# autonomousvision/unimatch

Hardware: AMD Instinct MI355X
Metric: image_pairs_per_sec (higher is better)
Workload: dtype f16x2

## Files before the change

include/unimatch_hip.h:

```cpp
#ifndef UNIMATCH_HIP_H
#define UNIMATCH_HIP_H

#include <stddef.h>
#include <stdint.h>

#ifdef __cplusplus
extern "C" {
#endif

#define UM_VERSION 220

#define UM_MODE_EXACT 0
#define UM_MODE_FAST 1

#define UM_ERR_BAD_ARG (-1)
#define UM_ERR_BAD_GEOMETRY (-2)
#define UM_ERR_WORKSPACE (-3)
#define UM_ERR_UNSUPPORTED (-4)
#define UM_ERR_COLLECTIVE (-5)

int um_version(void);
const char* um_last_error_string(void);

#define UM_RANGE_PLANES 1u
#define UM_RANGE_ATTN_TOKENS 2u
#define UM_RANGE_ATTN_QUERY 4u
#define UM_RANGE_ATTN_OUTPUT 8u
#define UM_RANGE_FFN_TOKENS 16u
#define UM_RANGE_FFN_HIDDEN 32u
#define UM_RANGE_KV_TOKENS 64u
#define UM_RANGE_LINEAR 128u
int um_range_flags(unsigned* flags_out, int reset);

#define UM_K_WINDOW_ATTN 0
#define UM_K_GLOBAL_SOFTMAX 1
#define UM_K_SPLIT_PLANES 2
#define UM_K_LOCAL_CORR 3
#define UM_K_COST_VOLUME 4
#define UM_K_PROP_LOCAL 5
#define UM_K_DEPTH_CORR 6
#define UM_K_LINEAR 7
#define UM_K_INSTANCE_NORM 8
#define UM_K_CONVEX_UPSAMPLE 9
#define UM_K_FFN 10
#define UM_K_CONV 11
#define UM_K_COUNT 12
#define UM_V_WATTN_TILE 0
#define UM_V_WATTN_KSPLIT 1
#define UM_V_FFN_TILE 2
#define UM_V_FFN_HSPLIT 3
#define UM_V_GSV4 4
#define UM_V_GSV3 5
#define UM_V_K4_MFMA 6
#define UM_V_K4_VALU 7
#define UM_V_K3_MFMA 8
#define UM_V_K3_VALU 9
#define UM_V_CONV_PATCH 10
#define UM_V_CONV_ROWS 11
#define UM_V_CONV_GENERIC 12
#define UM_V_WATTN_W8 13
#define UM_V_CONV_PATCH_NORM 14
#define UM_V_COUNT 15
int um_census_enable(int on);
long um_census_count(int variant);
int um_window_attn_tile_census(int enable, unsigned long long* counts4);
double um_probe_mfma_flops(int iters);
int um_probe_mfma(float* sink, int iters, void* stream);
int um_probe_copy(const void* src, void* dst, size_t bytes, void* stream);
int um_probe_chase(const unsigned* ring, unsigned* out, int hops, void* stream);
int um_timing_enable(int kernel_mask);
int um_timing_collect(int kernel_id, double* total_ms, int* launches);

size_t um_window_attn_workspace_bytes(int streams, int tokens, int channels, int mode);
int um_window_attn_fwd(const float* q, const float* k, const float* v, float* out,
                       int streams, int h, int w, int channels,
                       int win_h, int win_w, int shift_h, int shift_w,
                       int mode, void* workspace, size_t workspace_bytes, void* stream);

int um_window_attn_planes_fwd(const void* q_planes, const void* k_planes, const void* v_planes, float* out,
                              int streams, int h, int w, int channels, int ldq, int ldkv,
                              long q_plane_stride, long kv_plane_stride,
                              int win_h, int win_w, int shift_h, int shift_w, int kv_rotate, int mode, void* stream);

int um_window_attn_merge_fwd(const void* q_planes, const void* k_planes, const void* v_planes, const void* wm_planes,
                             const float* gamma, const float* beta, const float* residual, float eps, int wshift, float* out,
                             int streams, int h, int w, int channels, int ldq, int ldkv, long q_plane_stride,
                             long kv_plane_stride, int win_h, int win_w, int shift_h, int shift_w, int kv_rotate, int mode,
                             void* stream);

size_t um_window_attn_ksplit_workspace_bytes(int streams, int h, int w, int win_h, int win_w);
int um_window_attn_plan(int streams, int h, int w, int win_h, int win_w, int* full_tiles, int* split_tiles, int* parts);
int um_window_attn_qproj_merge_fwd(const float* x, const void* wq_planes, const void* k_planes, const void* v_planes,
                                   const void* wm_planes, const float* gamma, const float* beta, const float* residual, float eps,
                                   int wshift, float* out, int streams, int h, int w, int channels, int ldkv,
                                   long kv_plane_stride, int win_h, int win_w, int shift_h, int shift_w, int kv_rotate, int mode,
                                   void* workspace, size_t workspace_bytes, void* stream);

#define UM_EPI_PLANES 0
#define UM_EPI_LN 1
#define UM_EPI_GELU_PLANES 2
size_t um_planes_bytes(long rows, int cols, int mode);
int um_weight_planes(const float* w, void* planes, int n, int k, int wshift, int mode, void* stream);
int um_linear_fwd(const float* a0, const float* a1, const void* a_planes, const void* w_planes,
                  int m, int n, int k, int wshift, int epilogue, void* out,
                  const float* gamma, const float* beta, const float* residual, float eps,
                  int mode, void* stream);

int um_linear_bias_fwd(const float* a0, const void* a_planes, const void* w_planes, const float* bias, int m, int n, int k,
                       int wshift, float out_mul, float bias_mul, void* out_planes, float* out_f32, int mode, void* stream);

int um_ffn_fwd(const float* x, const float* y, const void* w1_planes, const void* w2_planes, int m, int hidden,
               int wshift, const float* gamma, const float* beta, float eps, float* out, int mode, void* stream);
size_t um_ffn_split_workspace_bytes(int m, int hidden);
int um_ffn_ws_fwd(const float* x, const float* y, const void* w1_planes, const void* w2_planes, int m, int hidden,
                  int wshift, const float* gamma, const float* beta, float eps, float* out, int mode, void* workspace,
                  size_t workspace_bytes, void* stream);

int um_kv4_fwd(const float* x, const void* wc_planes, int m, int wshift, void* out_planes, int mode, void* stream);
int um_ffn_kv_fwd(const float* x, const float* y, const void* w1_planes, const void* w2_planes, int m, int hidden, int wshift,
                  const float* gamma, const float* beta, float eps, float* out, const void* wc_planes, void* kv_planes, int mode,
                  void* workspace, size_t workspace_bytes, void* stream);

int um_conv2d_fwd(const void* a_planes, const void* w_planes, const float* bias, float* out, float* stats_out, int batch,
                  int hi, int wi, int cin, int cout, int kh, int kw, int stride, int pad_h, int pad_w, int relu, int wshift,
                  int mode, void* stream);
int um_conv2d_ex(const void* a_planes, int a_ld, int a_coff, long a_rows, const void* w_planes, const float* bias, float* out,
                 int out_ld, int out_coff, void* out_planes, int outp_ld, int outp_coff, long outp_rows, float* stats_out,
                 int batch, int hi, int wi, int cin, int cout, int kh, int kw, int stride, int pad_h, int pad_w, int act,
                 int wshift, int mode, void* stream);
int um_conv2d_gru_fwd(int gate, const void* a_planes, int a_ld, int a_coff, long a_rows, const void* w_planes, const float* bias,
                      float* hidden, const float* z, int z_ld, float* z_out, int z_out_ld, void* out_planes, int outp_ld,
                      int outp_coff, long outp_rows, int batch, int hi, int wi, int cin, int channels, int kh, int kw, int pad_h,
                      int pad_w, int wshift, int mode, void* stream);
int um_conv2d_gru_add_fwd(int gate, const void* a_planes, int a_ld, int a_coff, long a_rows, const void* w_planes, const float* bias,
                          const float* addend, int addend_ld, float* hidden, const float* z, int z_ld, float* z_out, int z_out_ld,
                          void* out_planes, int outp_ld, int outp_coff, long outp_rows, int batch, int hi, int wi, int cin,
                          int channels, int kh, int kw, int pad_h, int pad_w, int wshift, int mode, void* stream);
int um_conv2d_addend_fwd(const void* a_planes, const void* w_planes, const float* bias, const float* addend, int addend_ld,
                         int addend_period, float* out, int batch, int hi, int wi, int cin, int cout, int kh, int kw, int stride,
                         int pad_h, int pad_w, int wshift, int mode, void* stream);
int um_conv_stats_parts(int hi, int wi, int cout, int kh, int kw, int stride, int pad_h, int pad_w);
size_t um_conv_stats_bytes(int batch, int parts, int channels);

size_t um_stem_planes_bytes(int batch, int h, int w);
size_t um_conv7_planes_bytes(int batch, int h, int w, int stride);
int um_conv7_fwd(const float* image, int channels, int normalize, const float* mean3, const float* std3, void* image_planes,
                 const void* w_planes, const float* bias, float* out, int out_ld, int out_coff, void* out_planes, int outp_ld,
                 int outp_coff, long outp_rows, float* stats_out, int batch, int h, int w, int cout, int stride, int act,
                 int wshift, void* stream);
int um_stem_conv_fwd(const float* image, int normalize, const float* mean3, const float* std3, void* image_planes,
                     const void* w_planes, float* out, float* stats_out, int batch, int h, int w, int cout, int wshift,
                     void* stream);

int um_stem_conv_pair_fwd(const float* image0, int batch0, const float* image1, int batch1, int normalize, const float* mean3,
                          const float* std3, void* image_planes, const void* w_planes, float* out, float* stats_out, int h, int w,
                          int cout, int wshift, void* stream);

size_t um_nhwc_norm_workspace_bytes(int batch, int pixels, int channels);
int um_nhwc_instance_norm(const float* x, const float* shortcut, const void* shortcut_planes, void* planes_out, float* f32_out,
                          int batch, int pixels, int channels, float eps, int normalize, int relu, const float* conv_stats,
                          int conv_stats_parts, void* workspace, size_t workspace_bytes, int mode, void* stream);

int um_nhwc_concat_planes(const float* map, const float* tokens, void* planes_out, int batch, int pixels, int map_channels, int channels,
                          int mode, void* stream);

size_t um_nhwc_norm_sc_workspace_bytes(int batch, int pixels, int channels);
int um_nhwc_instance_norm_sc(const float* x, const float* shortcut, const void* shortcut_planes, void* planes_out, float* f32_out,
                             int batch, int pixels, int channels, float eps, int normalize, int relu, const float* conv_stats,
                             int conv_stats_parts, void* workspace, size_t workspace_bytes, int mode, void* stream,
                             const float* sc_conv_stats, int sc_conv_stats_parts);

int um_nhwc_stats_finalize(const float* conv_stats, int conv_stats_parts, float* stats_out, int batch, int pixels, int channels,
                           float eps, void* stream);
int um_conv2d_norm_supported(int hi, int wi, int cin, int cout, int kh, int kw, int stride, int pad_h, int pad_w, int mode);
int um_conv2d_norm_fwd(const float* x, const float* norm_stats, int norm_relu, const void* w_planes, const float* bias, float* out,
                       float* stats_out, int batch, int hi, int wi, int cin, int cout, int kh, int kw, int stride, int pad_h,
                       int pad_w, int relu, int wshift, int mode, void* stream);

int um_conv2d_entry_supported(int hi, int wi, int cin, int cout, int kh, int kw, int stride, int pad_h, int pad_w, int mode);
int um_conv2d_entry_fwd(const float* u, const float* ustats, const void* s_planes, const void* w_planes, const void* w2_planes,
                        const float* bias2, float* out_t, float* out_d, float* stats_t, float* stats_d, int batch, int hi, int wi,
                        int cin, int cout, int kh, int kw, int stride, int pad_h, int pad_w, int wshift, int mode, void* stream);

int um_nhwc_gate(int mode, const float* src, int src_ld, const float* zr, float* hbuf, void* planes_out, int ld, int coff,
                 long plane_rows, long rows, int channels, void* stream);

int um_nchw_to_nhwc(const float* x, void* planes_out, float* f32_out, int batch, int channels, int pixels, int mode,
                    void* stream);

size_t um_global_corr_workspace_bytes(int batch, int tokens, int channels, int mode);
int um_global_corr_softmax_flow(const float* f0, const float* f1, float* flow,
                                int batch, int h, int w, int channels, int bidir,
                                int mode, void* workspace, size_t workspace_bytes, void* stream);

int um_global_corr_softmax_stereo(const float* f0, const float* f1, float* disp,
                                  int batch, int h, int w, int channels,
                                  int mode, void* workspace, size_t workspace_bytes, void* stream);

int um_prop_global_attn(const float* q, const float* k, const float* value, float* out,
                        int batch, int h, int w, int channels, int value_channels,
                        int mode, void* workspace, size_t workspace_bytes, void* stream);
float um_global_corr_plane_scale(int channels);
int um_prop_global_attn_planes(const void* q_planes, const void* k_planes, const float* value, float* out, int batch, int h,
                               int w, int channels, int value_channels, int mode, void* workspace, size_t workspace_bytes,
                               void* stream);

size_t um_global_match_stats_workspace_bytes(int batch, int tokens, int channels, int mode);
int um_global_match_stats(const float* f0, const float* f1, float* stats, int* best, float* mean,
                          int batch, int h, int w, int channels, int bidir, int stereo,
                          int mode, void* workspace, size_t workspace_bytes, void* stream);
int um_match_mutual(const int* best_fwd, const int* best_bwd, unsigned char* mutual, int batch, int h, int w, int radius,
                    void* stream);


int um_local_corr_softmax(const float* f0, const float* f1, float* out,
                          int batch, int h, int w, int channels, int radius, int one_d, void* stream);

int um_local_corr_with_flow(const float* f0, const float* f1, const float* flow, float* cost,
                            int batch, int h, int w, int channels, int radius, void* stream);
int um_local_corr_with_flow_dilated(const float* f0, const float* f1, const float* flow, float* cost,
                                    int batch, int h, int w, int channels, int radius, int dilation, void* stream);
int um_local_corr_with_flow_planes(const float* f0, const float* f1, const float* flow, void* planes_out, int ld, long plane_rows,
                                   int batch, int h, int w, int channels, int radius, void* stream);

size_t um_local_corr_feat_planes_bytes(int batch, int h, int w, int channels);
int um_local_corr_feat_planes(const float* f0, const float* f1, void* feat_planes, int batch, int h, int w, int channels,
                              void* stream);
int um_local_corr_with_flow_feat_supported(int h, int w, int channels, int radius);
int um_local_corr_softmax_mfma(const float* f0, const float* f1, float* out, int batch, int h, int w, int channels, int radius,
                               void* workspace, size_t workspace_bytes, void* stream);
int um_local_corr_with_flow_feat(const float* f0, const float* f1, const void* feat_planes, const float* flow, float* cost,
                                 void* planes_out, int ld, long plane_rows, int batch, int h, int w, int channels, int radius,
                                 int flags, unsigned* stats ,
                                 void* stream);

int um_prop_local_attn(const float* q, const float* k, const float* value, float* out,
                       int batch, int h, int w, int channels, int value_channels, int radius,
                       void* stream);

int um_depth_corr_softmax(const float* f0, const float* f1, const float* cam, const float* candidates,
                          float* out, int batch, int h, int w, int channels, int num_candidates,
                          int from_argmax, void* stream);

int um_convex_upsample(const float* flow, const float* mask, float* up, int batch, int channels, int h, int w,
                       int factor, int is_depth, int mask_nhwc, void* stream);

int um_flow_warp(const float* feature_tokens, const float* flow, float* out_tokens, int batch, int h, int w, int channels,
                 void* stream);

int um_fwd_bwd_occlusion(const float* fwd, const float* bwd, float* occ_fwd, float* occ_bwd, int batch, int h, int w, float alpha,
                         float beta, void* stream);
size_t um_flow_to_rgb_workspace_bytes(int batch, int h, int w);
int um_flow_to_rgb(const float* flow, unsigned char* rgb, int batch, int h, int w, void* workspace, size_t ws_bytes, void* stream);

int um_flow_chain(const float* flow, const float* occ, const float* pos_in, const unsigned char* alive_in, float* tracks,
                  unsigned char* visible, int pairs, int h, int w, int n, int grid_stride, void* stream);

#define UM_FLOW_METRICS_K 16
#define UM_DISP_METRICS_K 8
#define UM_DEPTH_METRICS_K 8
size_t um_flow_metrics_workspace_bytes(int batch, int h, int w);
int um_flow_metrics(const float* pred, const float* gt, const float* valid, const float* noc_valid, double* rows, int batch, int hp,
                    int wp, int h, int w, int top, int left, void* workspace, size_t ws_bytes, void* stream);
size_t um_disp_metrics_workspace_bytes(int batch, int h, int w);
int um_disp_metrics(const float* pred, const float* gt, double* rows, int batch, int hp, int wp, int h, int w, int top, int left,
                    float max_disp, void* workspace, size_t ws_bytes, void* stream);
size_t um_depth_metrics_workspace_bytes(int batch, int h, int w);
int um_depth_metrics(const float* pred, const float* gt, const float* valid, double* rows, int batch, int hp, int wp, int h, int w,
                     int top, int left, float lo, float hi, void* workspace, size_t ws_bytes, void* stream);

#define UM_PREPOST_MAX_DIM 262140
#define UM_IMG_F32_NCHW 0
#define UM_IMG_U8_NHWC 1
#define UM_SIZE_PAD 0
#define UM_SIZE_RESIZE 1
#define UM_PRED_FLOW 0
#define UM_PRED_DISPARITY 1
#define UM_PRED_DEPTH 2
int um_image_prepare(const void* src, int src_layout, float* dst, int batch, int h, int w, int transpose, const float* mean,
                     const float* std, int mode, int hp, int wp, int top, int left, void* stream);
int um_pred_restore(const float* pred, float* out, int batch, int channels, int hp, int wp, int mode, int top, int left, int h, int w,
                    int kind, int transpose, void* stream);
int um_image_prepare_flip(const void* src, int src_layout, float* dst, int batch, int h, int w, int transpose, const float* mean,
                          const float* std, int mode, int hp, int wp, int top, int left, int hflip, void* stream);
int um_pred_restore_flip(const float* pred, float* out, int batch, int channels, int hp, int wp, int mode, int top, int left, int h,
                         int w, int kind, int transpose, int hflip, void* stream);

#define UM_NORM_MINMAX_255 0
#define UM_NORM_MIN_P95_256 1
size_t um_scalar_to_rgb_workspace_bytes(int batch, int h, int w);
int um_scalar_to_rgb(const float* x, unsigned char* rgb, int batch, int h, int w, int inverse, int norm, const unsigned char* lut,
                     float* stats_out, void* workspace, size_t ws_bytes, void* stream);

int um_flow_upsample2x(const float* flow, float* out, int batch, int channels, int h, int w, float mult, void* stream);
int um_depth_cam_pack(const float* intrinsics, const float* pose, float* cam, int batch, float stride_div, int bidir, void* stream);
int um_rigid_flow(const float* inv_depth, const float* cam, float* flow, int batch, int h, int w, void* stream);
int um_relative_pose_pairs(const float* poses, float* rel, int frames, void* stream);

int um_disp_consistency(const float* disp_left, const float* disp_right, float* occ_left, float* occ_right, int batch, int h, int w,
                        float alpha, float beta, void* stream);
int um_depth_consistency(const float* depth_ref, const float* depth_src, const float* cam_fwd, const float* cam_inv, float* occ,
                         float* err_px, float* err_rel, int batch, int h, int w, float px_thr, float rel_thr, void* stream);
size_t um_points_workspace_bytes(int batch, int h, int w, int stride);
int um_points_pack(const float* depth, const float* cam_world, const float* keep, const unsigned char* colors, float* xyz,
                   unsigned char* rgb, int* count, int batch, int h, int w, int stride, float min_depth, float max_depth, void* workspace,
                   size_t ws_bytes, void* stream);

int um_instance_norm_fwd(const float* x, const float* shortcut, float* y, long planes, int hw, float eps,
                         int relu, void* stream);

#define UM_COMM_ID_BYTES 128
int um_comm_unique_id(void* id_out );
int um_comm_init_rank(void** comm_out, const void* id , int rank, int world);
int um_comm_init_file(void** comm_out, const char* path, int rank, int world, int timeout_seconds);
int um_comm_init_file_nonce(void** comm_out, const char* path, int rank, int world, int timeout_seconds, int nonce);
int um_comm_world(void* comm);
int um_comm_destroy(void* comm);
int um_allgather_preds(void* comm, const float* send, float* recv, size_t count_per_rank, void* stream);

int um_swin_attn_fwd(const float* q, const float* k, const float* v, float* out, int streams, int h, int w, int channels,
                     int win_h, int win_w, int shift_h, int shift_w, int mode, void* workspace, size_t workspace_bytes,
                     void* stream);
int um_attn1d_fwd(const float* q, const float* k, const float* v, float* out, int streams, int h, int w, int channels,
                  int win_w, int shift_w, int mode, void* workspace, size_t workspace_bytes, void* stream);
int um_local_corr_softmax_1d(const float* f0, const float* f1, float* out, int batch, int h, int w, int channels, int radius,
                             void* stream);
size_t um_workspace_bytes_swin_attn_fwd(int streams, int h, int w, int channels, int mode);
size_t um_workspace_bytes_attn1d_fwd(int streams, int h, int w, int channels, int mode);
size_t um_workspace_bytes_global_corr_softmax_flow(int batch, int h, int w, int channels, int mode);
size_t um_workspace_bytes_global_corr_softmax_stereo(int batch, int h, int w, int channels, int mode);
size_t um_workspace_bytes_prop_global_attn(int batch, int h, int w, int channels, int mode);
size_t um_workspace_bytes_local_corr_softmax(int batch, int h, int w, int channels, int mode);
size_t um_workspace_bytes_local_corr_softmax_1d(int batch, int h, int w, int channels, int mode);
size_t um_workspace_bytes_local_corr_with_flow(int batch, int h, int w, int channels, int mode);
size_t um_workspace_bytes_prop_local_attn(int batch, int h, int w, int channels, int mode);
size_t um_workspace_bytes_depth_corr_softmax(int batch, int h, int w, int channels, int mode);
size_t um_workspace_bytes_allgather_preds(int batch, int h, int w, int channels, int mode);

#ifdef UM_DIAGNOSTIC_BUILD
int um_debug_mfma_peak(float* sink, int iters, int random_operands, void* stream);
int um_debug_mfma_ticks(unsigned long long* ticks, float* sink, int iters, int random_operands, int waves, int chain, void* stream);
int um_debug_mfma_lds(unsigned long long* ticks, float* sink, int tiles, int mode, void* stream);
#endif

#ifdef __cplusplus
}
#endif
#endif
```

unimatch_amd/_abi.py:

```python
import ctypes
import os

_HERE = os.path.dirname(os.path.abspath(__file__))
LIB_PATH = os.environ.get('UM_LIB') or os.path.join(_HERE, 'libunimatch_hip.so')

MODE_EXACT = 0
MODE_FAST = 1

CENSUS = {'wattn_tile': 0, 'wattn_ksplit': 1, 'ffn_tile': 2, 'ffn_hsplit': 3, 'gsv4': 4, 'gsv3': 5, 'k4_mfma': 6, 'k4_valu': 7,
          'k3_mfma': 8, 'k3_valu': 9, 'conv_patch': 10, 'conv_rows': 11, 'conv_generic': 12, 'wattn_w8': 13, 'conv_patch_norm': 14}

_c_int, _c_size_t, _c_void_p = ctypes.c_int, ctypes.c_size_t, ctypes.c_void_p

SIGNATURES = {
    'um_version': (_c_int, []),
    'um_last_error_string': (ctypes.c_char_p, []),
    'um_range_flags': (_c_int, [ctypes.POINTER(ctypes.c_uint), _c_int]),
    'um_timing_enable': (_c_int, [_c_int]),
    'um_timing_collect': (_c_int, [_c_int, ctypes.POINTER(ctypes.c_double), ctypes.POINTER(_c_int)]),
    'um_window_attn_workspace_bytes': (_c_size_t, [_c_int] * 4),
    'um_window_attn_fwd': (_c_int, [_c_void_p] * 4 + [_c_int] * 9 + [_c_void_p, _c_size_t, _c_void_p]),
    'um_window_attn_planes_fwd': (_c_int, [_c_void_p] * 4 + [_c_int] * 6 + [ctypes.c_long] * 2 + [_c_int] * 6 + [_c_void_p]),
    'um_window_attn_merge_fwd': (_c_int, [_c_void_p] * 7 + [ctypes.c_float, _c_int, _c_void_p] + [_c_int] * 6 + [ctypes.c_long] * 2 +
                                 [_c_int] * 6 + [_c_void_p]),
    'um_window_attn_qproj_merge_fwd': (_c_int, [_c_void_p] * 8 + [ctypes.c_float, _c_int, _c_void_p] + [_c_int] * 5 + [ctypes.c_long] +
                                       [_c_int] * 6 + [_c_void_p, _c_size_t, _c_void_p]),
    'um_window_attn_ksplit_workspace_bytes': (_c_size_t, [_c_int] * 5),
    'um_window_attn_plan': (_c_int, [_c_int] * 5 + [ctypes.POINTER(_c_int)] * 3),
    'um_planes_bytes': (_c_size_t, [ctypes.c_long, _c_int, _c_int]),
    'um_weight_planes': (_c_int, [_c_void_p] * 2 + [_c_int] * 4 + [_c_void_p]),
    'um_linear_fwd': (_c_int, [_c_void_p] * 4 + [_c_int] * 5 + [_c_void_p] * 4 + [ctypes.c_float, _c_int, _c_void_p]),
    'um_linear_bias_fwd': (_c_int, [_c_void_p] * 4 + [_c_int] * 4 + [ctypes.c_float] * 2 + [_c_void_p] * 2 + [_c_int, _c_void_p]),
    'um_ffn_fwd': (_c_int, [_c_void_p] * 4 + [_c_int] * 3 + [_c_void_p] * 2 + [ctypes.c_float, _c_void_p, _c_int, _c_void_p]),
    'um_ffn_ws_fwd': (_c_int, [_c_void_p] * 4 + [_c_int] * 3 + [_c_void_p] * 2 + [ctypes.c_float, _c_void_p, _c_int, _c_void_p, _c_size_t,
                                _c_void_p]),
    'um_ffn_split_workspace_bytes': (_c_size_t, [_c_int] * 2),
    'um_ffn_kv_fwd': (_c_int, [_c_void_p] * 4 + [_c_int] * 3 + [_c_void_p] * 2 + [ctypes.c_float, _c_void_p, _c_void_p, _c_void_p, _c_int, _c_void_p,
                                _c_size_t, _c_void_p]),
    'um_kv4_fwd': (_c_int, [_c_void_p, _c_void_p, _c_int, _c_int, _c_void_p, _c_int, _c_void_p]),
    'um_conv2d_fwd': (_c_int, [_c_void_p] * 5 + [_c_int] * 13 + [_c_void_p]),
    'um_conv2d_addend_fwd': (_c_int, [_c_void_p] * 4 + [_c_int, _c_int, _c_void_p] + [_c_int] * 12 + [_c_void_p]),
    'um_conv2d_ex': (_c_int, [_c_void_p, _c_int, _c_int, ctypes.c_long, _c_void_p, _c_void_p, _c_void_p, _c_int, _c_int, _c_void_p,
                              _c_int, _c_int, ctypes.c_long, _c_void_p] + [_c_int] * 13 + [_c_void_p]),
    'um_nhwc_gate': (_c_int, [_c_int, _c_void_p, _c_int, _c_void_p, _c_void_p, _c_void_p, _c_int, _c_int, ctypes.c_long, ctypes.c_long,
                              _c_int, _c_void_p]),
    'um_local_corr_with_flow_planes': (_c_int, [_c_void_p] * 4 + [_c_int, ctypes.c_long] + [_c_int] * 5 + [_c_void_p]),
    'um_conv2d_gru_fwd': (_c_int, [_c_int, _c_void_p, _c_int, _c_int, ctypes.c_long, _c_void_p, _c_void_p, _c_void_p, _c_void_p, _c_int,
                                   _c_void_p, _c_int, _c_void_p, _c_int, _c_int, ctypes.c_long] + [_c_int] * 11 + [_c_void_p]),
    'um_conv2d_gru_add_fwd': (_c_int, [_c_int, _c_void_p, _c_int, _c_int, ctypes.c_long, _c_void_p, _c_void_p, _c_void_p, _c_int, _c_void_p, _c_void_p,
                                        _c_int, _c_void_p, _c_int, _c_void_p, _c_int, _c_int, ctypes.c_long] + [_c_int] * 11 + [_c_void_p]),
    'um_conv2d_norm_supported': (_c_int, [_c_int] * 10),
    'um_conv2d_norm_fwd': (_c_int, [_c_void_p, _c_void_p, _c_int] + [_c_void_p] * 4 + [_c_int] * 13 + [_c_void_p]),
    'um_conv2d_entry_supported': (_c_int, [_c_int] * 10),
    'um_conv2d_entry_fwd': (_c_int, [_c_void_p] * 10 + [_c_int] * 12 + [_c_void_p]),
    'um_nhwc_norm_sc_workspace_bytes': (_c_size_t, [_c_int] * 3),
    'um_nhwc_instance_norm_sc': (_c_int, [_c_void_p] * 5 + [_c_int] * 3 + [ctypes.c_float, _c_int, _c_int, _c_void_p, _c_int, _c_void_p,
                                          _c_size_t, _c_int, _c_void_p, _c_void_p, _c_int]),
    'um_nhwc_stats_finalize': (_c_int, [_c_void_p, _c_int, _c_void_p] + [_c_int] * 3 + [ctypes.c_float, _c_void_p]),
    'um_conv_stats_bytes': (_c_size_t, [_c_int] * 3),
    'um_conv_stats_parts': (_c_int, [_c_int] * 8),
    'um_stem_planes_bytes': (_c_size_t, [_c_int] * 3),
    'um_conv7_planes_bytes': (_c_size_t, [_c_int] * 4),
    'um_conv7_fwd': (_c_int, [_c_void_p, _c_int, _c_int] + [_c_void_p] * 6 + [_c_int, _c_int, _c_void_p, _c_int, _c_int, ctypes.c_long,
                              _c_void_p] + [_c_int] * 7 + [_c_void_p]),
    'um_stem_conv_fwd': (_c_int, [_c_void_p, _c_int] + [_c_void_p] * 6 + [_c_int] * 5 + [_c_void_p]),
    'um_stem_conv_pair_fwd': (_c_int, [_c_void_p, _c_int, _c_void_p, _c_int, _c_int] + [_c_void_p] * 6 + [_c_int] * 4 + [_c_void_p]),
    'um_nhwc_concat_planes': (_c_int, [_c_void_p] * 3 + [_c_int] * 5 + [_c_void_p]),
    'um_nhwc_norm_workspace_bytes': (_c_size_t, [_c_int] * 3),
    'um_nhwc_instance_norm': (_c_int, [_c_void_p] * 5 + [_c_int] * 3 + [ctypes.c_float, _c_int, _c_int, _c_void_p, _c_int, _c_void_p,
                                       _c_size_t, _c_int, _c_void_p]),
    'um_nchw_to_nhwc': (_c_int, [_c_void_p] * 3 + [_c_int] * 4 + [_c_void_p]),
    'um_flow_warp': (_c_int, [_c_void_p] * 3 + [_c_int] * 4 + [_c_void_p]),
    'um_fwd_bwd_occlusion': (_c_int, [_c_void_p] * 4 + [_c_int] * 3 + [ctypes.c_float] * 2 + [_c_void_p]),
    'um_flow_to_rgb_workspace_bytes': (_c_size_t, [_c_int] * 3),
    'um_flow_to_rgb': (_c_int, [_c_void_p] * 2 + [_c_int] * 3 + [_c_void_p, _c_size_t, _c_void_p]),
    'um_flow_chain': (_c_int, [_c_void_p] * 6 + [_c_int] * 5 + [_c_void_p]),
    'um_flow_metrics_workspace_bytes': (_c_size_t, [_c_int] * 3),
    'um_flow_metrics': (_c_int, [_c_void_p] * 5 + [_c_int] * 7 + [_c_void_p, _c_size_t, _c_void_p]),
    'um_disp_metrics_workspace_bytes': (_c_size_t, [_c_int] * 3),
    'um_disp_metrics': (_c_int, [_c_void_p] * 3 + [_c_int] * 7 + [ctypes.c_float, _c_void_p, _c_size_t, _c_void_p]),
    'um_depth_metrics_workspace_bytes': (_c_size_t, [_c_int] * 3),
    'um_depth_metrics': (_c_int, [_c_void_p] * 4 + [_c_int] * 7 + [ctypes.c_float] * 2 + [_c_void_p, _c_size_t, _c_void_p]),
    'um_image_prepare': (_c_int, [_c_void_p, _c_int, _c_void_p] + [_c_int] * 4 + [ctypes.POINTER(ctypes.c_float)] * 2 + [_c_int] * 5 +
                         [_c_void_p]),
    'um_pred_restore': (_c_int, [_c_void_p] * 2 + [_c_int] * 11 + [_c_void_p]),
    'um_image_prepare_flip': (_c_int, [_c_void_p, _c_int, _c_void_p] + [_c_int] * 4 + [ctypes.POINTER(ctypes.c_float)] * 2 + [_c_int] * 6 +
                              [_c_void_p]),
    'um_pred_restore_flip': (_c_int, [_c_void_p] * 2 + [_c_int] * 12 + [_c_void_p]),
    'um_scalar_to_rgb_workspace_bytes': (_c_size_t, [_c_int] * 3),
    'um_scalar_to_rgb': (_c_int, [_c_void_p] * 2 + [_c_int] * 5 + [_c_void_p] * 3 + [_c_size_t, _c_void_p]),
    'um_convex_upsample': (_c_int, [_c_void_p] * 3 + [_c_int] * 7 + [_c_void_p]),
    'um_flow_upsample2x': (_c_int, [_c_void_p] * 2 + [_c_int] * 4 + [ctypes.c_float, _c_void_p]),
    'um_depth_cam_pack': (_c_int, [_c_void_p] * 3 + [_c_int, ctypes.c_float, _c_int, _c_void_p]),
    'um_rigid_flow': (_c_int, [_c_void_p] * 3 + [_c_int] * 3 + [_c_void_p]),
    'um_relative_pose_pairs': (_c_int, [_c_void_p] * 2 + [_c_int, _c_void_p]),
    'um_disp_consistency': (_c_int, [_c_void_p] * 4 + [_c_int] * 3 + [ctypes.c_float] * 2 + [_c_void_p]),
    'um_depth_consistency': (_c_int, [_c_void_p] * 7 + [_c_int] * 3 + [ctypes.c_float] * 2 + [_c_void_p]),
    'um_points_workspace_bytes': (_c_size_t, [_c_int] * 4),
    'um_points_pack': (_c_int, [_c_void_p] * 7 + [_c_int] * 4 + [ctypes.c_float] * 2 + [_c_void_p, _c_size_t, _c_void_p]),
    'um_instance_norm_fwd': (_c_int, [_c_void_p] * 3 + [ctypes.c_long, _c_int, ctypes.c_float, _c_int, _c_void_p]),
    'um_global_corr_workspace_bytes': (_c_size_t, [_c_int] * 4),
    'um_global_corr_softmax_flow': (_c_int, [_c_void_p] * 3 + [_c_int] * 6 + [_c_void_p, _c_size_t, _c_void_p]),
    'um_global_corr_softmax_stereo': (_c_int, [_c_void_p] * 3 + [_c_int] * 5 + [_c_void_p, _c_size_t, _c_void_p]),
    'um_prop_global_attn': (_c_int, [_c_void_p] * 4 + [_c_int] * 6 + [_c_void_p, _c_size_t, _c_void_p]),
    'um_global_corr_plane_scale': (ctypes.c_float, [_c_int]),
    'um_prop_global_attn_planes': (_c_int, [_c_void_p] * 4 + [_c_int] * 6 + [_c_void_p, _c_size_t, _c_void_p]),
    'um_global_match_stats_workspace_bytes': (_c_size_t, [_c_int] * 4),
    'um_global_match_stats': (_c_int, [_c_void_p] * 5 + [_c_int] * 7 + [_c_void_p, _c_size_t, _c_void_p]),
    'um_match_mutual': (_c_int, [_c_void_p] * 3 + [_c_int] * 4 + [_c_void_p]),
    'um_local_corr_softmax': (_c_int, [_c_void_p] * 3 + [_c_int] * 6 + [_c_void_p]),
    'um_local_corr_with_flow': (_c_int, [_c_void_p] * 4 + [_c_int] * 5 + [_c_void_p]),
    'um_local_corr_with_flow_dilated': (_c_int, [_c_void_p] * 4 + [_c_int] * 6 + [_c_void_p]),
    'um_local_corr_feat_planes_bytes': (ctypes.c_size_t, [_c_int] * 4),
    'um_local_corr_feat_planes': (_c_int, [_c_void_p] * 3 + [_c_int] * 4 + [_c_void_p]),
    'um_local_corr_with_flow_feat_supported': (_c_int, [_c_int] * 4),
    'um_local_corr_softmax_mfma': (_c_int, [_c_void_p] * 3 + [_c_int] * 5 + [_c_void_p, ctypes.c_size_t, _c_void_p]),
    'um_local_corr_with_flow_feat': (_c_int, [_c_void_p] * 6 + [_c_int, ctypes.c_long] + [_c_int] * 6 + [_c_void_p, _c_void_p]),
    'um_prop_local_attn': (_c_int, [_c_void_p] * 4 + [_c_int] * 6 + [_c_void_p]),
    'um_depth_corr_softmax': (_c_int, [_c_void_p] * 5 + [_c_int] * 6 + [_c_void_p]),
    'um_census_enable': (_c_int, [_c_int]),
    'um_census_count': (ctypes.c_long, [_c_int]),
    'um_window_attn_tile_census': (_c_int, [_c_int, ctypes.POINTER(ctypes.c_ulonglong)]),
    'um_probe_mfma_flops': (ctypes.c_double, [_c_int]),
    'um_probe_mfma': (_c_int, [_c_void_p, _c_int, _c_void_p]),
    'um_probe_copy': (_c_int, [_c_void_p, _c_void_p, _c_size_t, _c_void_p]),
    'um_probe_chase': (_c_int, [_c_void_p, _c_void_p, _c_int, _c_void_p]),
    'um_swin_attn_fwd': (_c_int, [_c_void_p] * 4 + [_c_int] * 9 + [_c_void_p, _c_size_t, _c_void_p]),
    'um_attn1d_fwd': (_c_int, [_c_void_p] * 4 + [_c_int] * 7 + [_c_void_p, _c_size_t, _c_void_p]),
    'um_local_corr_softmax_1d': (_c_int, [_c_void_p] * 3 + [_c_int] * 5 + [_c_void_p]),
    **{f'um_workspace_bytes_{op}': (_c_size_t, [_c_int] * 5) for op in (
        'swin_attn_fwd', 'attn1d_fwd', 'global_corr_softmax_flow', 'global_corr_softmax_stereo', 'prop_global_attn',
        'local_corr_softmax', 'local_corr_softmax_1d', 'local_corr_with_flow', 'prop_local_attn', 'depth_corr_softmax',
        'allgather_preds')},
    'um_comm_unique_id': (_c_int, [_c_void_p]),
    'um_comm_init_rank': (_c_int, [ctypes.POINTER(_c_void_p), _c_void_p, _c_int, _c_int]),
    'um_comm_init_file': (_c_int, [ctypes.POINTER(_c_void_p), ctypes.c_char_p, _c_int, _c_int, _c_int]),
    'um_comm_init_file_nonce': (_c_int, [ctypes.POINTER(_c_void_p), ctypes.c_char_p, _c_int, _c_int, _c_int, _c_int]),
    'um_comm_world': (_c_int, [_c_void_p]),
    'um_comm_destroy': (_c_int, [_c_void_p]),
    'um_allgather_preds': (_c_int, [_c_void_p, _c_void_p, _c_void_p, _c_size_t, _c_void_p]),
}
COMM_ID_BYTES = 128
DIAG_SIGNATURES = {
    'um_debug_mfma_peak': (_c_int, [_c_void_p, _c_int, _c_int, _c_void_p]),
    'um_debug_mfma_lds': (_c_int, [_c_void_p, _c_void_p, _c_int, _c_int, _c_void_p]),
    'um_debug_mfma_ticks': (_c_int, [_c_void_p, _c_void_p, _c_int, _c_int, _c_int, _c_int, _c_void_p]),
}

RANGE_ROLES = {1: 'a tensor converted to operand planes (q / k / v / features)', 2: 'attention source tokens', 4: 'projected queries',
               8: 'attention output (input of the merge Linear)', 16: 'FFN input [x | y]', 32: 'FFN hidden activations',
               64: 'tokens / projected keys and values of the k | v projection', 128: 'inputs / plane outputs of a Linear'}

_lib = None


class HipExtensionError(RuntimeError):
    pass


def load():
    global _lib
    if _lib is not None:
        return _lib
    if not os.path.exists(LIB_PATH):
        raise HipExtensionError(
            f'{LIB_PATH} is missing: build it with `python -m unimatch_amd.build` '
            '(hipcc --offload-arch=gfx950).  There is no CPU / PyTorch fallback for the hot path.')
    try:
        lib = ctypes.CDLL(LIB_PATH)
    except OSError as exc:
        raise HipExtensionError(f'cannot load {LIB_PATH}: {exc}') from exc
    for name, (res, args) in SIGNATURES.items():
        try:
            fn = getattr(lib, name)
        except AttributeError as exc:
            raise HipExtensionError(f'{LIB_PATH} does not export {name}') from exc
        fn.restype = res
        fn.argtypes = args
    for name, (res, args) in DIAG_SIGNATURES.items():
        fn = getattr(lib, name, None)
        if fn is not None:
            fn.restype = res
            fn.argtypes = args
    _lib = lib
    return lib


def load_diagnostic():
    lib = load()
    if not hasattr(lib, 'um_debug_mfma_peak'):
        raise HipExtensionError('the shipped library carries no um_debug_* symbol: build a diagnostic variant '
                                '(`python -m unimatch_amd.build --variant diag`) and set UM_LIB=unimatch_amd/_variants/libdiag.so')
    return lib


def census(lib=None):
    lib = lib or load()
    return {k: int(lib.um_census_count(v)) for k, v in CENSUS.items()}


def attn_tile_census(enable):
    out = (ctypes.c_ulonglong * 4)()
    check(load().um_window_attn_tile_census(1 if enable else 0, out), 'um_window_attn_tile_census')
    return dict(zip(('full', 'probed', 'probed_then_computed', 'workgroups'), (int(v) for v in out)))


def check(code, what):
    if code == 0:
        return
    msg = load().um_last_error_string().decode('utf-8', 'replace')
    if code < 0:
        raise ValueError(f'{what}: {msg} (code {code})')
    raise RuntimeError(f'{what}: HIP error {code}')


class OperandRangeError(FloatingPointError):
    """An activation reached fp16's largest finite value (65504) on its way into an exact-mode MFMA operand."""


def range_flags(reset=False):
    out = ctypes.c_uint(0)
    check(load().um_range_flags(ctypes.byref(out), 1 if reset else 0), 'um_range_flags')
    return out.value


def check_operand_range(where=''):
    flags = range_flags(reset=True)
    if flags:
        roles = '; '.join(v for k, v in RANGE_ROLES.items() if flags & k)
        raise OperandRangeError(
            f'{where}exact mode splits fp32 values into fp16 hi | lo operands, and an element of magnitude >= 65504 reached: {roles} '
            '(the hi plane is inf there and NaN follows downstream; the fp32 reference has no such limit).  Scale the inputs / '
            "weights by a power of two, or run precision='fast' (bf16 operands: fp32's exponent range).")
```

unimatch_amd/build.py:

```python
import os
import re
import shutil
import subprocess
import sys

HERE = os.path.dirname(os.path.abspath(__file__))
CSRC = os.path.join(HERE, 'csrc')
LIB = os.path.join(HERE, 'libunimatch_hip.so')
SOURCES = ['capi.hip', 'global_match.hip', 'window_attn.hip', 'local_ops.hip', 'linear.hip', 'ffn.hip', 'conv.hip', 'nhwc_ops.hip', 'norm_ops.hip', 'upsample.hip',
           'rccl_gather.hip', 'local_corr_mfma.hip', 'aliases.hip', 'probe.hip', 'video.hip', 'metrics.hip', 'prepost.hip', 'visualize.hip', 'geometry.hip', 'match_stats.hip']
DIAG_SOURCES = ['microbench.hip']
HEADERS = ['common.h', 'planes.h', 'timing.h', os.path.join('..', '..', 'include', 'unimatch_hip.h')]
EXTRA_FLAGS = {'ffn.hip': ['-fno-slp-vectorize'], 'global_match.hip': ['-fno-slp-vectorize', '-mllvm', '-amdgpu-mfma-vgpr-form', '-Wno-inline-asm'], 'window_attn.hip': ['-fno-slp-vectorize'],
               'linear.hip': ['-fno-slp-vectorize'],
               'video.hip': ['-ffp-contract=off'],
               'metrics.hip': ['-ffp-contract=off', '-fhip-fp32-correctly-rounded-divide-sqrt'],
               'prepost.hip': ['-ffp-contract=off', '-fhip-fp32-correctly-rounded-divide-sqrt'],
               'visualize.hip': ['-ffp-contract=off', '-fhip-fp32-correctly-rounded-divide-sqrt'],
               'geometry.hip': ['-ffp-contract=off', '-fhip-fp32-correctly-rounded-divide-sqrt'],
               'match_stats.hip': ['-fno-slp-vectorize', '-fhip-fp32-correctly-rounded-divide-sqrt', '-Wno-inline-asm']}
RESOURCE_GUARDS = {'conv.hip': {'conv_entry_kernel': 2},
                   'geometry.hip': {'disp_consistency_kernel': 4, 'depth_consistency_kernel': 4, 'points_count_kernel': 4,
                                    'points_scan_kernel': 4, 'points_scatter_kernel': 4},
                   'match_stats.hip': {'match_stats_kernel': 2, 'match_mutual_kernel': 4}}
FLAGS = ['--offload-arch=gfx950', '-O3', '-std=c++17', '-fPIC', '-fno-gpu-rdc', '-Wno-unused-result']


def find_hipcc():
    for cand in (os.environ.get('HIPCC'), shutil.which('hipcc'), '/opt/rocm/bin/hipcc'):
        if cand and os.path.exists(cand):
            return cand
    raise RuntimeError('hipcc not found: the HIP extension cannot be built')


def parse_resource_report(text):
    out, cur = {}, None
    for line in text.splitlines():
        m = re.search(r'remark: .*?Function Name: (\S+)', line)
        if m:
            cur = out.setdefault(m.group(1), {})
            continue
        m = re.search(r'remark: .*?\s{2,}([A-Za-z ]+?)(?: \[[^\]]*\])?: (\d+)', line)
        if m and cur is not None:
            cur[m.group(1).strip()] = int(m.group(2))
    return out


def check_resources(src, report):
    for key, min_occ in RESOURCE_GUARDS.get(src, {}).items():
        hits = {k: v for k, v in report.items() if key in k}
        if not hits:
            raise RuntimeError(f'{src}: no resource report for {key}: the guard of unimatch_amd/build.py has nothing to check')
        for name, r in hits.items():
            if r.get('ScratchSize', -1) != 0 or r.get('Occupancy', 0) < min_occ:
                raise RuntimeError(f'{src}: {name} needs scratch {r.get("ScratchSize")} B/lane at occupancy {r.get("Occupancy")} '
                                   f'({r.get("VGPRs")} VGPRs): it was written for no scratch at {min_occ} waves per SIMD')


def _stale(target, deps):
    if not os.path.exists(target):
        return True
    t = os.path.getmtime(target)
    return any(os.path.getmtime(d) > t for d in deps)


def build(force=False, verbose=False):
    hipcc = find_hipcc()
    objdir = os.path.join(HERE, '_obj')
    os.makedirs(objdir, exist_ok=True)
    hdrs = [os.path.normpath(os.path.join(CSRC, h)) for h in HEADERS] + [os.path.abspath(__file__)]
    objs = []
    for src in SOURCES:
        s = os.path.join(CSRC, src)
        o = os.path.join(objdir, src.replace('.hip', '.o'))
        if force or _stale(o, [s] + hdrs) or (src in RESOURCE_GUARDS and not os.path.exists(o[:-2] + '.resources.txt')):
            cmd = [hipcc] + FLAGS + EXTRA_FLAGS.get(src, []) + ['-c', s, '-o', o]
            if verbose:
                print(' '.join(cmd))
            if src in RESOURCE_GUARDS:
                done = subprocess.run(cmd + ['-Rpass-analysis=kernel-resource-usage', '-fno-caret-diagnostics'], cwd=CSRC, stderr=subprocess.PIPE, text=True)
                remarks = [ln for ln in done.stderr.splitlines() if 'kernel-resource-usage' in ln]
                sys.stderr.write('\n'.join(ln for ln in done.stderr.splitlines() if 'kernel-resource-usage' not in ln))
                if done.returncode != 0:
                    raise subprocess.CalledProcessError(done.returncode, cmd)
                try:
                    check_resources(src, parse_resource_report('\n'.join(remarks)))
                except RuntimeError:
                    os.remove(o)
                    raise
                with open(o[:-2] + '.resources.txt', 'w') as f:
                    f.write('\n'.join(remarks) + '\n')
            else:
                subprocess.run(cmd, check=True, cwd=CSRC)
        objs.append(o)
    if force or _stale(LIB, objs):
        cmd = [hipcc, '--offload-arch=gfx950', '-shared', '-fPIC', '-o', LIB] + objs + ['-ldl']
        if verbose:
            print(' '.join(cmd))
        subprocess.run(cmd, check=True)
    return LIB


def build_variant(name, defines, verbose=False, only=None):
    hipcc = find_hipcc()
    objdir = os.path.join(HERE, '_variants', '_obj_' + name)
    os.makedirs(objdir, exist_ok=True)
    objs = []
    defines = list(defines) + ['-DUM_DIAGNOSTIC_BUILD']
    if only:
        build(verbose=verbose)
    for src in SOURCES + DIAG_SOURCES:
        if only and src not in only and src not in DIAG_SOURCES:
            objs.append(os.path.join(HERE, '_obj', src.replace('.hip', '.o')))
            continue
        o = os.path.join(objdir, src.replace('.hip', '.o'))
        cmd = [hipcc] + FLAGS + EXTRA_FLAGS.get(src, []) + list(defines) + ['-c', os.path.join(CSRC, src), '-o', o]
        if verbose:
            print(' '.join(cmd))
        subprocess.run(cmd, check=True, cwd=CSRC)
        objs.append(o)
    lib = os.path.join(HERE, '_variants', f'lib{name}.so')
    subprocess.run([hipcc, '--offload-arch=gfx950', '-shared', '-fPIC', '-o', lib] + objs + ['-ldl'], check=True)
    shutil.rmtree(objdir, ignore_errors=True)
    return lib


if __name__ == '__main__':
    if '--variant' in sys.argv:
        i = sys.argv.index('--variant')
        only = sys.argv[sys.argv.index('--only') + 1].split(',') if '--only' in sys.argv else None
        print(build_variant(sys.argv[i + 1], [a for a in sys.argv[i + 2:] if a.startswith('-D')], verbose=True, only=only))
    else:
        print(build(force='--force' in sys.argv, verbose=True))
```

unimatch_amd/csrc/ffn.hip:

```cpp
#include <type_traits>
#include <stdlib.h>
#ifndef UM_FFN_H1
#define UM_FFN_H1 0
#endif
#include "common.h"
#include "planes.h"

#ifdef UM_FFN_TRACE
__device__ unsigned long long* g_um_ffn_trace = nullptr;
#define UM_FSTAMP(slot) do { if (tracing && i < 24) trace_buf[(i) * 8 + (slot)] = __builtin_amdgcn_s_memtime(); } while (0)
#else
#define UM_FSTAMP(slot) do { } while (0)
#endif

struct Kv4Args {
    const float* x;
    const unsigned short* w;
    long w_plane_stride;
    unsigned short* out;
    long out_plane_stride;
    int M;
    float out_scale;
    unsigned* range_flag;
};

struct FfnArgs {
    const float* x;
    const float* y;
    const unsigned short* w1;
    long w1_plane_stride;
    const unsigned short* w2;
    long w2_plane_stride;
    const float* gamma;
    const float* beta;
    float* out;
    int M, hid;
    float out_scale;
    float eps;
    int split;
    float* hs_part;
    unsigned* hs_flag;
    Kv4Args kv;
    unsigned* range_flag;
};

__device__ __forceinline__ void ffn_dma16_at(const void* base, unsigned byte_off, unsigned lds_addr) {
    lds_addr = __builtin_amdgcn_readfirstlane(lds_addr);
    unsigned keep;
    asm volatile("s_mov_b32 %0, m0\n\ts_mov_b32 m0, %3\n\ts_nop 0\n\tglobal_load_lds_dwordx4 %1, %2\n\ts_mov_b32 m0, %0"
                 : "=&s"(keep)
                 : "v"(byte_off), "s"(base), "s"(lds_addr)
                 : "memory");
}
__device__ __forceinline__ void ffn_dma16(const void* base, unsigned byte_off, const unsigned char* lds_dst) {
    const unsigned dst = __builtin_amdgcn_readfirstlane(
        (unsigned)(unsigned long)(const __attribute__((address_space(3))) unsigned char*)lds_dst);
    unsigned keep;
    asm volatile("s_mov_b32 %0, m0\n\ts_mov_b32 m0, %3\n\ts_nop 0\n\tglobal_load_lds_dwordx4 %1, %2\n\ts_mov_b32 m0, %0"
                 : "=&s"(keep)
                 : "v"(byte_off), "s"(base), "s"(dst)
                 : "memory");
}

#ifndef UM_FFN_ORDER
#define UM_FFN_ORDER 1
#endif
#ifndef UM_FFN_PRIO
#define UM_FFN_PRIO 0
#endif
#ifndef UM_FFN_DMA_ASYM
#define UM_FFN_DMA_ASYM 0
#endif
#ifndef UM_FFN_NT
#define UM_FFN_NT 0
#endif
#if UM_FFN_NT >= 1
#define UM_FFN_LD(p) __builtin_nontemporal_load(p)
#else
#define UM_FFN_LD(p) (*(p))
#endif
#if UM_FFN_NT >= 2
#define UM_FFN_ST(p, v) __builtin_nontemporal_store(v, p)
#else
#define UM_FFN_ST(p, v) (*(p) = (v))
#endif
#ifndef UM_FFN_ROWSTORE
#define UM_FFN_ROWSTORE 1
#endif
#ifndef UM_FFN_ABL
#define UM_FFN_ABL 0
#endif
struct Gelu2 {
    float x[2], r[2];
};
#define UM_GELU_STAGES 4
__device__ __forceinline__ void ffn_gelu_stage(Gelu2& g, int stage) {
#pragma unroll
    for (int i = 0; i < 2; ++i) {
        if (UM_FFN_ABL & 1) {
            if (stage == UM_GELU_STAGES - 1) g.x[i] = g.x[i] * 0.5f;
            continue;
        }
        const float u = __builtin_fabsf(g.x[i]);
        switch (stage) {
        case 0:
            g.r[i] = __builtin_fmaf(-2.572117637100746e-06f, u, 3.6567180359270424e-05f);
            g.r[i] = __builtin_fmaf(g.r[i], u, -1.7448408470954746e-04f);
            g.r[i] = __builtin_fmaf(g.r[i], u, -1.6111040895339102e-04f);
            break;
        case 1:
            g.r[i] = __builtin_fmaf(g.r[i], u, 7.089670747518539e-03f);
            g.r[i] = __builtin_fmaf(g.r[i], u, -5.2510716021060944e-02f);
            g.r[i] = __builtin_fmaf(g.r[i], u, -4.592045545578003e-01f);
            break;
        case 2:
            g.r[i] = __builtin_fmaf(g.r[i], u, -1.151105523109436f);
            g.r[i] = g.r[i] * u;
            g.r[i] = fast_exp2(g.r[i]);
            break;
        default: {
            const float hx = g.x[i] * 0.5f;
            const float sum = hx + __builtin_fabsf(hx);
            g.x[i] = __builtin_fmaf(-__builtin_fabsf(hx), g.r[i], sum);
            break;
        }
        }
    }
}

template <int NS>
struct FfnLds {
    static constexpr int W1P = 32 * 512;
    static constexpr int W1S = NS * W1P;
    static constexpr int W2P = 128 * 64;
    static constexpr int W2S = NS * W2P;
    static constexpr int W1_OFF = 0, W2_OFF = 2 * W1S, XB_OFF = W2_OFF + 2 * W2S;
    static constexpr int XB = 2048;
    static constexpr int RING = XB_OFF + 2 * 8 * XB;
    static constexpr int TOTAL = RING > 65536 ? RING : 65536;
};


template <int NS>
struct Kv4Lds {
    static constexpr int RING = 2 * FfnLds<NS>::W1S;
    static constexpr int SCRP = 2048;
    static constexpr int SCRW = 2 * NS * SCRP;
    static constexpr int SCR_BYTES = 8 * SCRW;
};

template <typename T, int NS, bool CHUNK0_ISSUED>
__device__ __forceinline__ void kv4_project(unsigned char* ring, unsigned char* scr, const Kv4Args& k, const i16x8 (&yf)[NS][8],
                                            int m0, int wave, int lane, const int (&aoff)[8], float neg1) {
    using L = FfnLds<NS>;
    const int pair = wave & 3, role = wave >> 2;
    const int half = lane >> 5, tl = lane & 31;
    auto dma = [&](int c, int slot) {
#pragma unroll
        for (int i = 0; i < 2; ++i) {
            const int blk = 8 * i + wave;
            const int r = 2 * blk + half, cc = tl ^ r;
            const unsigned off = (unsigned)((((long)(32 * c + r)) * 256 + 8 * cc) * 2);
#pragma unroll
            for (int pl = 0; pl < NS; ++pl)
                ffn_dma16(k.w + pl * k.w_plane_stride, off, ring + slot * L::W1S + pl * L::W1P + blk * 1024);
        }
    };
    unsigned char* myscr = scr + wave * Kv4Lds<NS>::SCRW;
    const int sw = (tl >> 2) & 3;
    auto store_chunk = [&](int c) {
        const unsigned char* sp = myscr + (c & 1) * (NS * Kv4Lds<NS>::SCRP);
        const int j = 2 * role + (c >> 2);
#pragma unroll
        for (int pl = 0; pl < NS; ++pl)
#pragma unroll
            for (int it = 0; it < 2; ++it) {
                const int row = 16 * it + (lane >> 2), q = lane & 3;
                const u32x4 d = *reinterpret_cast<const u32x4*>(sp + pl * Kv4Lds<NS>::SCRP + row * 64 + ((q ^ ((row >> 2) & 3)) << 4));
                const long tok = (long)m0 + 32 * pair + row;
                if (tok < k.M)
                    *reinterpret_cast<u32x4*>(k.out + pl * k.out_plane_stride + ((long)j * k.M + tok) * 128 + 32 * (c & 3) + 8 * q) = d;
            }
    };
    if (!CHUNK0_ISSUED) dma(0, 0);
    float kmx = 0.f;
#pragma unroll 1
    for (int c = 0; c < 8; ++c) {
        const int slot = c & 1;
        asm volatile("s_waitcnt vmcnt(0)" ::: "memory");
        __syncthreads();
        if (c + 1 < 8) dma(c + 1, slot ^ 1);
        if (c > 0) store_chunk(c - 1);
        const unsigned char* w1s = ring + slot * L::W1S;
        f32x16 acc;
#pragma unroll
        for (int r = 0; r < 16; ++r) acc[r] = 0.f;
        {
            i16x8 fh[3], fl[3];
            __builtin_amdgcn_s_setprio(1);
#pragma unroll
            for (int ks = 0; ks < 2; ++ks) {
                fh[ks] = *reinterpret_cast<const i16x8*>(w1s + aoff[ks]);
                if (NS == 2) fl[ks] = *reinterpret_cast<const i16x8*>(w1s + L::W1P + aoff[ks]);
            }
#pragma unroll
            for (int ks = 0; ks < 8; ++ks) {
                if (ks + 2 < 8) {
                    fh[(ks + 2) % 3] = *reinterpret_cast<const i16x8*>(w1s + aoff[ks + 2]);
                    if (NS == 2) fl[(ks + 2) % 3] = *reinterpret_cast<const i16x8*>(w1s + L::W1P + aoff[ks + 2]);
                }
                if (NS == 2) {
                    acc = T::mfma(fl[ks % 3], yf[0][ks], acc);
                    acc = T::mfma(fh[ks % 3], yf[NS - 1][ks], acc);
                }
                acc = T::mfma(fh[ks % 3], yf[0][ks], acc);
            }
            constexpr int RD = NS, MF = (NS == 2) ? 3 : 1;
            __builtin_amdgcn_sched_group_barrier(0x100, 2 * RD, 0);
#pragma unroll
            for (int ks = 0; ks < 6; ++ks) {
                __builtin_amdgcn_sched_group_barrier(0x008, MF, 0);
                __builtin_amdgcn_sched_group_barrier(0x100, RD, 0);
            }
            __builtin_amdgcn_sched_group_barrier(0x008, 2 * MF, 0);
            __builtin_amdgcn_s_setprio(0);
        }
        unsigned char* dp = myscr + slot * (NS * Kv4Lds<NS>::SCRP) + tl * 64 + 8 * half;
#pragma unroll
        for (int g = 0; g < 4; ++g) {
            const float v0 = acc[4 * g] * k.out_scale, v1 = acc[4 * g + 1] * k.out_scale, v2 = acc[4 * g + 2] * k.out_scale,
                        v3 = acc[4 * g + 3] * k.out_scale;
            kmx = fmaxf(fmaxf(kmx, fmaxf(__builtin_fabsf(v0), __builtin_fabsf(v1))), fmaxf(__builtin_fabsf(v2), __builtin_fabsf(v3)));
            const unsigned h0 = T::pack2(v0, v1), h1 = T::pack2(v2, v3);
            *reinterpret_cast<u32x2*>(dp + ((g ^ sw) << 4)) = u32x2{h0, h1};
            if (NS == 2) {
                const unsigned l0 = T::lo2(v0, v1, h0, neg1), l1 = T::lo2(v2, v3, h1, neg1);
                *reinterpret_cast<u32x2*>(dp + Kv4Lds<NS>::SCRP + ((g ^ sw) << 4)) = u32x2{l0, l1};
            }
        }
    }
    store_chunk(7);
    um_range_note<T>(k.range_flag, kmx, UM_RANGE_KV_TOKENS);
}

template <typename T, int NS>
__global__ __launch_bounds__(512, 2) void kv4_kernel(Kv4Args k) {
    extern __shared__ __attribute__((aligned(16))) unsigned char lds[];
    const int tid = threadIdx.x, lane = tid & 63;
    const float neg1 = um_opaque_neg1();
    const int wave = __builtin_amdgcn_readfirstlane(tid >> 6);
    const int pair = wave & 3, role = wave >> 2;
    const int half = lane >> 5, tl = lane & 31;
    const int m0 = (int)blockIdx.x * 128;
    const int tok = m0 + 32 * pair + tl;
    i16x8 yf[NS][8];
    {
        const float* src = k.x + (long)min(tok, k.M - 1) * 128 + 8 * half;
        float xmx = 0.f;
#pragma unroll
        for (int ks = 0; ks < 8; ++ks) {
            const f32x4 v0 = *reinterpret_cast<const f32x4*>(src + 16 * ks);
            const f32x4 v1 = *reinterpret_cast<const f32x4*>(src + 16 * ks + 4);
#pragma unroll
            for (int j = 0; j < 4; ++j) xmx = fmaxf(xmx, fmaxf(__builtin_fabsf(v0[j]), __builtin_fabsf(v1[j])));
            const u32x4 h = {T::pack2(v0[0], v0[1]), T::pack2(v0[2], v0[3]), T::pack2(v1[0], v1[1]), T::pack2(v1[2], v1[3])};
            yf[0][ks] = __builtin_bit_cast(i16x8, h);
            if (NS == 2) {
                const u32x4 l = {T::lo2(v0[0], v0[1], h[0], neg1), T::lo2(v0[2], v0[3], h[1], neg1),
                                 T::lo2(v1[0], v1[1], h[2], neg1), T::lo2(v1[2], v1[3], h[3], neg1)};
                yf[NS - 1][ks] = __builtin_bit_cast(i16x8, l);
            }
        }
        um_range_note<T>(k.range_flag, xmx, UM_RANGE_KV_TOKENS);
    }
    const int arow = tl ^ (16 * role);
    int aoff[8];
#pragma unroll
    for (int ks = 0; ks < 8; ++ks) aoff[ks] = arow * 512 + (((16 * role + 2 * ks + half) ^ arow) << 4);
    kv4_project<T, NS, false>(lds, lds + Kv4Lds<NS>::RING, k, yf, m0, wave, lane, aoff, neg1);
}

template <typename T, int NS, bool HSPLIT = false, bool KV4 = false>
__global__ __launch_bounds__(512, 2) void ffn_kernel(FfnArgs a) {
    using L = FfnLds<NS>;
    extern __shared__ __attribute__((aligned(16))) unsigned char lds[];

    const int tid = threadIdx.x, lane = tid & 63;
    const float neg1 = um_opaque_neg1();
    const int wave = __builtin_amdgcn_readfirstlane(tid >> 6);
    const int pair = wave & 3, role = wave >> 2;
    const int half = lane >> 5, tl = lane & 31;
    const int nsplit = HSPLIT ? a.split : 1;
    const int tile_id = HSPLIT ? (int)blockIdx.x / nsplit : (int)blockIdx.x;
    const int part = HSPLIT ? (int)blockIdx.x - tile_id * nsplit : 0;
    const int m0 = tile_id * 128;
    const int tok = m0 + 32 * pair + tl;
    const int nslice = (a.hid >> 5) / nsplit;
    const int sbase = part * nslice;

    auto dma_w1 = [&](int j, int slot) {
#pragma unroll
        for (int i = 0; i < 2; ++i) {
            const int blk = 8 * i + wave;
            const int r = 2 * blk + half, c = tl ^ r;
            const unsigned off = (unsigned)((((long)(32 * (sbase + j) + r)) * 256 + 8 * c) * 2);
#pragma unroll
            for (int pl = 0; pl < NS; ++pl)
                ffn_dma16(a.w1 + pl * a.w1_plane_stride, off, lds + L::W1_OFF + slot * L::W1S + pl * L::W1P + blk * 1024);
        }
    };
    auto dma_w2 = [&](int j, int slot) {
        const int r = 16 * wave + (lane >> 2), c = (lane & 3) ^ ((r >> 2) & 3);
        const unsigned off = (unsigned)((((long)r) * a.hid + 32 * (sbase + j) + 8 * c) * 2);
#pragma unroll
        for (int pl = 0; pl < NS; ++pl)
            ffn_dma16(a.w2 + pl * a.w2_plane_stride, off, lds + L::W2_OFF + slot * L::W2S + pl * L::W2P + wave * 1024);
    };

#ifdef UM_FFN_TRACE
    const bool tracing = g_um_ffn_trace != nullptr && (blockIdx.x % 37) == 0 && lane == 0 && pair == 0;
    unsigned long long* trace_buf = g_um_ffn_trace + ((size_t)(blockIdx.x / 37) * 2 + role) * (24 * 8 + 8);
    if (tracing) trace_buf[24 * 8] = __builtin_amdgcn_s_memtime();
#endif
    const unsigned lds_wave = __builtin_amdgcn_readfirstlane(
        (unsigned)(unsigned long)(const __attribute__((address_space(3))) unsigned char*)lds) + (unsigned)wave * 1024u;
    auto dma_piece = [&](int k, int jw1, int jw2, int slot) {
        if (k < 4) {
            const int i = k >> 1, pl = k & 1;
            if (pl >= NS) return;
            const int blk = 8 * i + wave;
            const int r = 2 * blk + half, c = tl ^ r;
            const unsigned off = (unsigned)((((long)(32 * (sbase + jw1) + r)) * 256 + 8 * c) * 2);
            ffn_dma16_at(a.w1 + pl * a.w1_plane_stride, off, lds_wave + (unsigned)(L::W1_OFF + slot * L::W1S + pl * L::W1P + 8 * i * 1024));
        } else {
            const int pl = k - 4;
            if (pl >= NS) return;
            const int r = 16 * wave + (lane >> 2), c = (lane & 3) ^ ((r >> 2) & 3);
            const unsigned off = (unsigned)((((long)r) * a.hid + 32 * (sbase + jw2) + 8 * c) * 2);
            ffn_dma16_at(a.w2 + pl * a.w2_plane_stride, off, lds_wave + (unsigned)(L::W2_OFF + slot * L::W2S + pl * L::W2P));
        }
    };

    auto dma_piece_asym = [&](int k, int jw1, int jw2, int slot) {
        const int pl = k & 1;
        if (pl >= NS) return;
        if (k < 8) {
            const int blk = 4 * (k >> 1) + pair;
            const int r = 2 * blk + half, c = tl ^ r;
            const unsigned off = (unsigned)((((long)(32 * (sbase + jw1) + r)) * 256 + 8 * c) * 2);
            ffn_dma16(a.w1 + pl * a.w1_plane_stride, off, lds + L::W1_OFF + slot * L::W1S + pl * L::W1P + blk * 1024);
        } else {
            const int blk = 2 * pair + ((k - 8) >> 1);
            const int r = 16 * blk + (lane >> 2), c = (lane & 3) ^ ((r >> 2) & 3);
            const unsigned off = (unsigned)((((long)r) * a.hid + 32 * (sbase + jw2) + 8 * c) * 2);
            ffn_dma16(a.w2 + pl * a.w2_plane_stride, off, lds + L::W2_OFF + slot * L::W2S + pl * L::W2P + blk * 1024);
        }
    };

    dma_w1(0, 0);

    i16x8 xf[NS][8];
    {
        const float* src = (role ? a.y : a.x) + (long)min(tok, a.M - 1) * 128 + 8 * half;
        float xmx = 0.f;
#pragma unroll
        for (int ks = 0; ks < 8; ++ks) {
            const f32x4 v0 = UM_FFN_LD(reinterpret_cast<const f32x4*>(src + 16 * ks));
            const f32x4 v1 = UM_FFN_LD(reinterpret_cast<const f32x4*>(src + 16 * ks + 4));
#pragma unroll
            for (int j = 0; j < 4; ++j) xmx = fmaxf(xmx, fmaxf(__builtin_fabsf(v0[j]), __builtin_fabsf(v1[j])));
            const u32x4 h = {T::pack2(v0[0], v0[1]), T::pack2(v0[2], v0[3]), T::pack2(v1[0], v1[1]), T::pack2(v1[2], v1[3])};
            xf[0][ks] = __builtin_bit_cast(i16x8, h);
            if (NS == 2) {
                const u32x4 l = {T::lo2(v0[0], v0[1], h[0], neg1), T::lo2(v0[2], v0[3], h[1], neg1),
                                 T::lo2(v1[0], v1[1], h[2], neg1), T::lo2(v1[2], v1[3], h[3], neg1)};
                xf[NS - 1][ks] = __builtin_bit_cast(i16x8, l);
            }
        }
        um_range_note<T>(a.range_flag, xmx, UM_RANGE_FFN_TOKENS);
    }

    f32x16 o[4];
#pragma unroll
    for (int ot = 0; ot < 4; ++ot)
#pragma unroll
        for (int r = 0; r < 16; ++r) o[ot][r] = 0.f;

    const int arow = tl ^ (16 * role);
    int aoff[8];
#pragma unroll
    for (int ks = 0; ks < 8; ++ks) aoff[ks] = arow * 512 + (((16 * role + 2 * ks + half) ^ arow) << 4);
    int boff[4];
#pragma unroll
    for (int ot = 0; ot < 4; ++ot) {
        const int r = 32 * ot + tl;
        boff[ot] = L::W2_OFF + r * 64 + (((2 * role + half) ^ ((r >> 2) & 3)) << 4);
    }
    unsigned char* xb_out = lds + L::XB_OFF + wave * L::XB + lane * 16;
    const unsigned char* xb_in = lds + L::XB_OFF + (wave ^ 4) * L::XB + lane * 16;

    auto phase_a = [&](const unsigned char* w1s, f32x16& sc) {
#pragma unroll
        for (int r = 0; r < 16; ++r) sc[r] = 0.f;
        if (UM_FFN_ABL & 4) return;
        i16x8 fh[3], fl[3];
#pragma unroll
        for (int ks = 0; ks < 2; ++ks) {
            fh[ks] = *reinterpret_cast<const i16x8*>(w1s + aoff[ks]);
            if (NS == 2) fl[ks] = *reinterpret_cast<const i16x8*>(w1s + L::W1P + aoff[ks]);
        }
#pragma unroll
        for (int ks = 0; ks < 8; ++ks) {
            if (ks + 2 < 8) {
                fh[(ks + 2) % 3] = *reinterpret_cast<const i16x8*>(w1s + aoff[ks + 2]);
                if (NS == 2) fl[(ks + 2) % 3] = *reinterpret_cast<const i16x8*>(w1s + L::W1P + aoff[ks + 2]);
            }
            if (NS == 2) {
                sc = T::mfma(fl[ks % 3], xf[0][ks], sc);
                sc = T::mfma(fh[ks % 3], xf[NS - 1][ks], sc);
            }
            sc = T::mfma(fh[ks % 3], xf[0][ks], sc);
        }
    };
    auto send = [&](const f32x16& sc, int parity) {
        if (UM_FFN_ABL & 16) return;
        unsigned char* p = xb_out + parity * (8 * L::XB);
        *reinterpret_cast<f32x4*>(p) = f32x4{sc[8], sc[9], sc[10], sc[11]};
        *reinterpret_cast<f32x4*>(p + 1024) = f32x4{sc[12], sc[13], sc[14], sc[15]};
    };

    asm volatile("s_waitcnt vmcnt(0)" ::: "memory");
    __syncthreads();
    if (nslice > 1) dma_w1(1, 1);

    f32x16 sc;
    __builtin_amdgcn_s_setprio(1);
    phase_a(lds + L::W1_OFF, sc);
    {
        constexpr int RD = NS, MF = (NS == 2) ? 3 : 1;
        __builtin_amdgcn_sched_group_barrier(0x100, 2 * RD, 0);
#pragma unroll
        for (int ks = 0; ks < 6; ++ks) {
            __builtin_amdgcn_sched_group_barrier(0x008, MF, 0);
            __builtin_amdgcn_sched_group_barrier(0x100, RD, 0);
        }
        __builtin_amdgcn_sched_group_barrier(0x008, 2 * MF, 0);
    }
    __builtin_amdgcn_s_setprio(0);
    send(sc, 0);

    struct Frag {
        unsigned wh[4], wl[4];
    };
    float hmx = 0.f;
    auto frag_stage = [&](Frag& f, const Gelu2* g, i16x8* pf, int stage) {
        switch (stage) {
        case 0:
#pragma unroll
            for (int q = 0; q < 4; ++q) {
                hmx = fmaxf(hmx, fmaxf(__builtin_fabsf(g[q].x[0]), __builtin_fabsf(g[q].x[1])));
                f.wh[q] = T::pack2(g[q].x[0], g[q].x[1]);
            }
            break;
        case 1:
            if (NS == 2 && !UM_FFN_H1) {
#pragma unroll
                for (int q = 0; q < 2; ++q) f.wl[q] = T::lo2(g[q].x[0], g[q].x[1], f.wh[q], neg1);
            }
            break;
        case 2:
            if (NS == 2 && !UM_FFN_H1) {
#pragma unroll
                for (int q = 2; q < 4; ++q) f.wl[q] = T::lo2(g[q].x[0], g[q].x[1], f.wh[q], neg1);
            }
            break;
        default: {
            const auto sx = __builtin_amdgcn_permlane32_swap(f.wh[0], f.wh[2], false, false);
            const auto sy = __builtin_amdgcn_permlane32_swap(f.wh[1], f.wh[3], false, false);
            const u32x4 fh = {sx[0], sy[0], sx[1], sy[1]};
            pf[0] = __builtin_bit_cast(i16x8, fh);
            if (NS == 2 && !UM_FFN_H1) {
                const auto tx = __builtin_amdgcn_permlane32_swap(f.wl[0], f.wl[2], false, false);
                const auto ty = __builtin_amdgcn_permlane32_swap(f.wl[1], f.wl[3], false, false);
                const u32x4 fl = {tx[0], ty[0], tx[1], ty[1]};
                pf[NS - 1] = __builtin_bit_cast(i16x8, fl);
            }
            break;
        }
        }
    };

    i16x8 pf[NS];
    auto iteration = [&](auto has_a_tag, auto has_b_tag, int i) {
        constexpr bool HAS_A = decltype(has_a_tag)::value && !(UM_FFN_ABL & 4);
        constexpr bool HAS_B = decltype(has_b_tag)::value && !(UM_FFN_ABL & 8);
        constexpr int MF = (NS == 2) ? 3 : 1;
        constexpr int MFB = (NS == 2 && UM_FFN_H1) ? 2 : MF;
        constexpr int NMFMA = (HAS_A ? 8 * MF : 0) + (HAS_B ? 4 * MFB : 0);
        constexpr int NGELU = 4 * UM_GELU_STAGES, NSTAGE = NGELU + 4;
        const int slot = i & 1;
        const unsigned char* w1s = lds + L::W1_OFF + (slot ^ 1) * L::W1S;
        const unsigned char* w2s = lds + (slot ^ 1) * L::W2S;
        UM_FSTAMP(0);
        asm volatile("s_waitcnt vmcnt(0)" ::: "memory");
        UM_FSTAMP(1);
        __syncthreads();
        UM_FSTAMP(2);
        if (!(UM_FFN_ABL & 2)) {
            if (i + 2 < nslice) dma_w1(i + 2, slot);
            dma_w2(i, slot);
        }
        f32x4 r0 = {0.f, 0.f, 0.f, 0.f}, r1 = r0;
        if (!(UM_FFN_ABL & 16)) {
            const unsigned char* p = xb_in + slot * (8 * L::XB);
            r0 = *reinterpret_cast<const f32x4*>(p);
            r1 = *reinterpret_cast<const f32x4*>(p + 1024);
        }
        Gelu2 g[4];
#pragma unroll
        for (int q = 0; q < 2; ++q) {
#pragma unroll
            for (int i = 0; i < 2; ++i) {
                g[q].x[i] = (sc[2 * q + i] + r0[2 * q + i]) * a.out_scale;
                g[2 + q].x[i] = (sc[4 + 2 * q + i] + r1[2 * q + i]) * a.out_scale;
            }
        }
        Frag fr;
        i16x8 pfn[NS];
        int done = 0;
        auto valu_share = [&](int slot_idx) {
            const int upto = (slot_idx + 1) * NSTAGE / (NMFMA > 0 ? NMFMA : 1);
            for (; done < upto; ++done) {
                if (done < NGELU) ffn_gelu_stage(g[done / UM_GELU_STAGES], done % UM_GELU_STAGES);
                else frag_stage(fr, g, pfn, done - NGELU);
            }
        };
        f32x16 scn, scm;
#pragma unroll
        for (int r = 0; r < 16; ++r) scn[r] = scm[r] = 0.f;
        UM_FSTAMP(3);
        __builtin_amdgcn_s_setprio(1);
        int mslot = 0;
        i16x8 fh[3], fl[3];
        if (HAS_A) {
#pragma unroll
            for (int ks = 0; ks < 2; ++ks) {
                fh[ks] = *reinterpret_cast<const i16x8*>(w1s + aoff[ks]);
                if (NS == 2) fl[ks] = *reinterpret_cast<const i16x8*>(w1s + L::W1P + aoff[ks]);
            }
        }
        if (HAS_B) {
            i16x8 vh[4], vl[4];
#pragma unroll
            for (int ot = 0; ot < 4; ++ot) {
                vh[ot] = *reinterpret_cast<const i16x8*>(w2s + boff[ot]);
                if (NS == 2) vl[ot] = *reinterpret_cast<const i16x8*>(w2s + L::W2P + boff[ot]);
            }
#pragma unroll
            for (int m = 0; m < MFB; ++m)
#pragma unroll
                for (int ot = 0; ot < 4; ++ot) {
                    const i16x8 wa = (NS == 2 && m == 0) ? vl[ot] : vh[ot];
                    const i16x8 hb = (NS == 2 && MFB == 3 && m == 1) ? pf[NS - 1] : pf[0];
                    o[ot] = T::mfma(wa, hb, o[ot]);
                    valu_share(mslot++);
                    __builtin_amdgcn_sched_group_barrier(0x008, 1, 1);
                    __builtin_amdgcn_sched_group_barrier(0x402, 16, 1);
                    __builtin_amdgcn_sched_barrier(0);
                }
        }
        if (HAS_A) {
#pragma unroll
            for (int ks = 0; ks < 8; ++ks) {
                if (ks + 2 < 8) {
                    fh[(ks + 2) % 3] = *reinterpret_cast<const i16x8*>(w1s + aoff[ks + 2]);
                    if (NS == 2) fl[(ks + 2) % 3] = *reinterpret_cast<const i16x8*>(w1s + L::W1P + aoff[ks + 2]);
                }
#pragma unroll
                for (int m = 0; m < MF; ++m) {
                    const i16x8 wa = (NS == 2 && m == 0) ? fl[ks % 3] : fh[ks % 3];
                    const i16x8 xb = (NS == 2 && m == 1) ? xf[NS - 1][ks] : xf[0][ks];
                    if ((ks * MF + m) & 1) scm = T::mfma(wa, xb, scm);
                    else scn = T::mfma(wa, xb, scn);
                    valu_share(mslot++);
                    if (m == 0 && ks + 2 < 8) __builtin_amdgcn_sched_group_barrier(0x100, NS, 1);
                    __builtin_amdgcn_sched_group_barrier(0x008, 1, 1);
                    __builtin_amdgcn_sched_group_barrier(0x402, 16, 1);
                    __builtin_amdgcn_sched_barrier(0);
                }
            }
        }
        __builtin_amdgcn_s_setprio(0);
        UM_FSTAMP(4);
        for (; done < NSTAGE; ++done) {
            if (done < NGELU) ffn_gelu_stage(g[done / UM_GELU_STAGES], done % UM_GELU_STAGES);
            else frag_stage(fr, g, pfn, done - NGELU);
        }
        __builtin_amdgcn_sched_barrier(0);
        if (decltype(has_a_tag)::value) {
#pragma unroll
            for (int r = 0; r < 16; ++r) scn[r] += scm[r];
            send(scn, slot ^ 1);
#pragma unroll
            for (int r = 0; r < 8; ++r) sc[r] = scn[r];
        }
#pragma unroll
        for (int pl = 0; pl < NS; ++pl) pf[pl] = pfn[pl];
        UM_FSTAMP(5);
    };

    auto iteration1 = [&](auto has_a_tag, auto has_b_tag, auto dma1_tag, auto slot_tag, int i) {
        constexpr bool HAS_A = decltype(has_a_tag)::value && !(UM_FFN_ABL & 4);
        constexpr bool HAS_B = decltype(has_b_tag)::value && !(UM_FFN_ABL & 8);
        constexpr bool DMA1 = decltype(dma1_tag)::value;
        constexpr int MF = (NS == 2) ? 3 : 1;
        constexpr int MFB = (NS == 2 && UM_FFN_H1) ? 2 : MF;
        constexpr int NA = HAS_A ? 8 * MF : 0, NB = HAS_B ? 4 * MFB : 0, NMFMA = NA + NB;
        constexpr int NGELU = 4 * UM_GELU_STAGES, NSTAGE = NGELU + 4;
        const int slot = slot_tag;
        const unsigned char* w1s = lds + L::W1_OFF + (slot ^ 1) * L::W1S;
        const unsigned char* w2s = lds + (slot ^ 1) * L::W2S;
        UM_FSTAMP(0);
        asm volatile("s_waitcnt vmcnt(0)" ::: "memory");
        UM_FSTAMP(1);
        __syncthreads();
        UM_FSTAMP(2);
        f32x4 r0 = {0.f, 0.f, 0.f, 0.f}, r1 = r0;
        if (!(UM_FFN_ABL & 16)) {
            const unsigned char* p = xb_in + slot * (8 * L::XB);
            r0 = *reinterpret_cast<const f32x4*>(p);
            r1 = *reinterpret_cast<const f32x4*>(p + 1024);
        }
        i16x8 fh[3], fl[3];
        if (HAS_A) {
#pragma unroll
            for (int ks = 0; ks < 2; ++ks) {
                fh[ks] = *reinterpret_cast<const i16x8*>(w1s + aoff[ks]);
                if (NS == 2) fl[ks] = *reinterpret_cast<const i16x8*>(w1s + L::W1P + aoff[ks]);
            }
        }
        Gelu2 g[4];
#pragma unroll
        for (int q = 0; q < 2; ++q) {
#pragma unroll
            for (int e = 0; e < 2; ++e) {
                g[q].x[e] = (sc[2 * q + e] + r0[2 * q + e]) * a.out_scale;
                g[2 + q].x[e] = (sc[4 + 2 * q + e] + r1[2 * q + e]) * a.out_scale;
            }
        }
        Frag fr;
        i16x8 pfn[NS];
        int done = 0;
        auto valu_share = [&](int slot_idx) {
            const int upto = (slot_idx + 1) * NSTAGE / (NMFMA > 0 ? NMFMA : 1);
            for (; done < upto; ++done) {
                if (done < NGELU) ffn_gelu_stage(g[done / UM_GELU_STAGES], done % UM_GELU_STAGES);
                else frag_stage(fr, g, pfn, done - NGELU);
            }
        };
        int piece = UM_FFN_DMA_ASYM ? (DMA1 ? 0 : 8) : (DMA1 ? 0 : 4);
        constexpr int NPIECE = UM_FFN_DMA_ASYM ? 12 : 6;
        auto dma_share = [&](int slot_idx) {
            if (UM_FFN_ABL & 2) return;
            if (slot_idx >= 1 && piece < NPIECE) {
                if (UM_FFN_DMA_ASYM) {
                    if (role == 0) dma_piece_asym(piece, i + 2, i, slot);
                    piece += (NS == 1) ? 2 : 1;
                } else {
                    dma_piece(piece, i + 2, i, slot);
                    ++piece;
                    if (NS == 1 && (piece == 1 || piece == 3)) ++piece;
                }
            }
        };
        f32x16 scn, scm;
#pragma unroll
        for (int r = 0; r < 16; ++r) scn[r] = scm[r] = 0.f;
        UM_FSTAMP(3);
        __builtin_amdgcn_s_setprio(1);
        auto prio = [&](int ms) {
            int fav = -1;
            if (UM_FFN_PRIO == 1 && (ms == 0 || ms == NMFMA / 2)) fav = ms == 0 ? 0 : 1;
            if (UM_FFN_PRIO == 2 && ms % 6 == 0) fav = (ms / 6) & 1;
            if (UM_FFN_PRIO == 4 && ms % 3 == 0) fav = (ms / 3) & 1;
            if (UM_FFN_PRIO == 5 && ms % 12 == 0) fav = (ms / 12) & 1;
            if (UM_FFN_PRIO == 3 && ms == 0) fav = 1;
            if (fav < 0) return;
            if (role == fav) __builtin_amdgcn_s_setprio(2);
            else __builtin_amdgcn_s_setprio(1);
        };
        int mslot = 0;
        i16x8 vh[4], vl[4];
        if (HAS_A) {
#pragma unroll
            for (int ks = 0; ks < 8; ++ks) {
                if (ks + 2 < 8) {
                    fh[(ks + 2) % 3] = *reinterpret_cast<const i16x8*>(w1s + aoff[ks + 2]);
                    if (NS == 2) fl[(ks + 2) % 3] = *reinterpret_cast<const i16x8*>(w1s + L::W1P + aoff[ks + 2]);
                }
#pragma unroll
                for (int m = 0; m < MF; ++m) {
                    const i16x8 wa = (NS == 2 && m == 0) ? fl[ks % 3] : fh[ks % 3];
                    const i16x8 xb = (NS == 2 && m == 1) ? xf[NS - 1][ks] : xf[0][ks];
                    prio(mslot);
                    if ((ks * MF + m) & 1) scm = T::mfma(wa, xb, scm);
                    else scn = T::mfma(wa, xb, scn);
                    const int left = NA - 1 - (ks * MF + m);
                    const bool vread = HAS_B && left < 4;
                    if (vread) {
                        vh[3 - left] = *reinterpret_cast<const i16x8*>(w2s + boff[3 - left]);
                        if (NS == 2) vl[3 - left] = *reinterpret_cast<const i16x8*>(w2s + L::W2P + boff[3 - left]);
                    }
                    dma_share(mslot);
                    valu_share(mslot++);
                    if ((m == 0 && ks + 2 < 8) || vread) __builtin_amdgcn_sched_group_barrier(0x100, NS, 1);
                    __builtin_amdgcn_sched_group_barrier(0x008, 1, 1);
                    __builtin_amdgcn_sched_group_barrier(0x402, 16, 1);
                    __builtin_amdgcn_sched_barrier(0);
                }
            }
        }
        if (HAS_B) {
            if (!HAS_A) {
#pragma unroll
                for (int ot = 0; ot < 4; ++ot) {
                    vh[ot] = *reinterpret_cast<const i16x8*>(w2s + boff[ot]);
                    if (NS == 2) vl[ot] = *reinterpret_cast<const i16x8*>(w2s + L::W2P + boff[ot]);
                }
            }
#pragma unroll
            for (int m = 0; m < MFB; ++m)
#pragma unroll
                for (int ot = 0; ot < 4; ++ot) {
                    const i16x8 wa = (NS == 2 && m == 0) ? vl[ot] : vh[ot];
                    const i16x8 hb = (NS == 2 && MFB == 3 && m == 1) ? pf[NS - 1] : pf[0];
                    prio(mslot);
                    o[ot] = T::mfma(wa, hb, o[ot]);
                    const int bslot = m * 4 + ot;
                    dma_share(mslot);
                    if (decltype(has_a_tag)::value) {
                        constexpr int H0 = NB >= 6 ? 2 : NB - 3;
                        static_assert(NB == 0 || H0 >= 0, "phase B too short for the hand-over");
                        if (bslot == H0) {
#pragma unroll
                            for (int r = 0; r < 8; ++r) scn[r] += scm[r];
                        }
                        if (bslot == H0 + 1) {
#pragma unroll
                            for (int r = 8; r < 16; ++r) scn[r] += scm[r];
                        }
                        if (bslot == H0 + 2) send(scn, slot ^ 1);
                    }
                    valu_share(mslot++);
                    __builtin_amdgcn_sched_group_barrier(0x008, 1, 1);
                    __builtin_amdgcn_sched_group_barrier(0x602, 24, 1);
                    __builtin_amdgcn_sched_barrier(0);
                }
        }
        __builtin_amdgcn_s_setprio(0);
        UM_FSTAMP(4);
        for (; done < NSTAGE; ++done) {
            if (done < NGELU) ffn_gelu_stage(g[done / UM_GELU_STAGES], done % UM_GELU_STAGES);
            else frag_stage(fr, g, pfn, done - NGELU);
        }
        if (!(UM_FFN_ABL & 2)) {
            while (piece < NPIECE) {
                if (UM_FFN_DMA_ASYM) {
                    if (role == 0) dma_piece_asym(piece, i + 2, i, slot);
                    piece += (NS == 1) ? 2 : 1;
                } else {
                    dma_piece(piece, i + 2, i, slot);
                    ++piece;
                    if (NS == 1 && (piece == 1 || piece == 3)) ++piece;
                }
            }
        }
        __builtin_amdgcn_sched_barrier(0);
        if (decltype(has_a_tag)::value) {
            if (!HAS_B) {
#pragma unroll
                for (int r = 0; r < 16; ++r) scn[r] += scm[r];
                send(scn, slot ^ 1);
            }
#pragma unroll
            for (int r = 0; r < 8; ++r) sc[r] = scn[r];
        }
#pragma unroll
        for (int pl = 0; pl < NS; ++pl) pf[pl] = pfn[pl];
        UM_FSTAMP(5);
    };

    if (UM_FFN_ORDER == 1) {
        using Y = std::true_type;
        using N = std::false_type;
        using S0 = std::integral_constant<int, 0>;
        using S1 = std::integral_constant<int, 1>;
        if ((nslice & 1) == 0 && nslice >= 4) {
            iteration1(Y{}, N{}, Y{}, S0{}, 0);
            int i = 1;
            for (; i + 4 < nslice; i += 2) {
                iteration1(Y{}, Y{}, Y{}, S1{}, i);
                iteration1(Y{}, Y{}, Y{}, S0{}, i + 1);
            }
            iteration1(Y{}, Y{}, Y{}, S1{}, nslice - 3);
            iteration1(Y{}, Y{}, N{}, S0{}, nslice - 2);
            iteration1(N{}, Y{}, N{}, S1{}, nslice - 1);
        } else {
            if (2 < nslice) iteration1(Y{}, N{}, Y{}, 0, 0);
            else iteration1(Y{}, N{}, N{}, 0, 0);
            int i = 1;
            for (; i + 2 < nslice; ++i) iteration1(Y{}, Y{}, Y{}, i & 1, i);
            for (; i + 1 < nslice; ++i) iteration1(Y{}, Y{}, N{}, i & 1, i);
            iteration1(N{}, Y{}, N{}, (nslice - 1) & 1, nslice - 1);
        }
    } else {
        iteration(std::true_type{}, std::false_type{}, 0);
        for (int i = 1; i + 1 < nslice; ++i) iteration(std::true_type{}, std::true_type{}, i);
        iteration(std::false_type{}, std::true_type{}, nslice - 1);
    }
    f32x4 rr[16];
    {
        const unsigned char* w2s = lds + ((nslice - 1) & 1) * L::W2S;
        asm volatile("s_waitcnt vmcnt(0)" ::: "memory");
        __syncthreads();
        if (role == 0) {
            const float* res = a.x + (long)min(tok, a.M - 1) * 128 + 4 * half;
#pragma unroll
            for (int q = 0; q < 16; ++q)
                rr[q] = (UM_FFN_ABL & 32) ? f32x4{0.f, 0.f, 0.f, 0.f} : UM_FFN_LD(reinterpret_cast<const f32x4*>(res + 8 * q));
        }
        if (!(UM_FFN_ABL & 8)) {
#pragma unroll
            for (int ot = 0; ot < 4; ++ot) {
                const i16x8 vh = *reinterpret_cast<const i16x8*>(w2s + boff[ot]);
                if (NS == 2) {
                    const i16x8 vl = *reinterpret_cast<const i16x8*>(w2s + L::W2P + boff[ot]);
                    o[ot] = T::mfma(vl, pf[0], o[ot]);
                    if (!UM_FFN_H1) o[ot] = T::mfma(vh, pf[NS - 1], o[ot]);
                }
                o[ot] = T::mfma(vh, pf[0], o[ot]);
            }
        }
    }

#ifdef UM_FFN_TRACE
    if (tracing) trace_buf[24 * 8 + 1] = __builtin_amdgcn_s_memtime();
#endif
    um_range_note<T>(a.range_flag, hmx, UM_RANGE_FFN_HIDDEN);
    __syncthreads();
    static_assert(!(KV4 && HSPLIT), "the k | v epilogue runs on whole tiles only");
    if constexpr (KV4) {
#pragma unroll
        for (int i = 0; i < 2; ++i) {
            const int blk = 8 * i + wave;
            const int r = 2 * blk + half, cc = tl ^ r;
            const unsigned off = (unsigned)((((long)r) * 256 + 8 * cc) * 2);
#pragma unroll
            for (int pl = 0; pl < NS; ++pl)
                ffn_dma16(a.kv.w + pl * a.kv.w_plane_stride, off, lds + pl * L::W1P + blk * 1024);
        }
    }
    unsigned char* ob = lds + (KV4 ? 65536 : 0) + pair * 16384 + lane * 16;
    if (role == 1) {
#pragma unroll
        for (int ot = 0; ot < 4; ++ot)
#pragma unroll
            for (int g = 0; g < 4; ++g)
                *reinterpret_cast<f32x4*>(ob + (4 * ot + g) * 1024) =
                    f32x4{o[ot][4 * g], o[ot][4 * g + 1], o[ot][4 * g + 2], o[ot][4 * g + 3]};
    }
    __syncthreads();
    if (!HSPLIT && !KV4 && role == 1) return;
    if (role == 0) {
#pragma unroll
        for (int ot = 0; ot < 4; ++ot)
#pragma unroll
            for (int g = 0; g < 4; ++g) {
                const f32x4 r = *reinterpret_cast<const f32x4*>(ob + (4 * ot + g) * 1024);
#pragma unroll
                for (int i = 0; i < 4; ++i) o[ot][4 * g + i] = (o[ot][4 * g + i] + r[i]) * a.out_scale;
            }
    }
    if constexpr (HSPLIT) {
        const int t4 = 64 * pair + lane;
        constexpr int HS_SLOT = 16 * 256 * 4;
        if (role == 0) {
            float* mine = a.hs_part + ((long)tile_id * nsplit + part) * HS_SLOT + 4 * t4;
#pragma unroll
            for (int ot = 0; ot < 4; ++ot)
#pragma unroll
                for (int g = 0; g < 4; ++g) {
                    const f32x4 v = {o[ot][4 * g], o[ot][4 * g + 1], o[ot][4 * g + 2], o[ot][4 * g + 3]};
                    st_agent_16B(mine + (ot * 4 + g) * 1024, v);
                }
        }
        asm volatile("s_waitcnt vmcnt(0)" ::: "memory");
        __syncthreads();
        unsigned* ticket = reinterpret_cast<unsigned*>(lds);
        if (tid == 0) *ticket = __hip_atomic_fetch_add(a.hs_flag + tile_id, 1u, __ATOMIC_RELAXED, __HIP_MEMORY_SCOPE_AGENT);
        __syncthreads();
        const unsigned my_ticket = *ticket;
        __syncthreads();
        if (my_ticket != (unsigned)(nsplit - 1)) return;
        asm volatile("buffer_inv sc1" ::: "memory");
        if (tid == 0) __hip_atomic_store(a.hs_flag + tile_id, 0u, __ATOMIC_RELAXED, __HIP_MEMORY_SCOPE_AGENT);
        if (role == 1) return;
        for (int p = 0; p < nsplit; ++p) {
            const float* pr = a.hs_part + ((long)tile_id * nsplit + p) * HS_SLOT + 4 * t4;
#pragma unroll
            for (int ot = 0; ot < 4; ++ot) {
                f32x4 w[4];
                const float* q = pr + ot * 4 * 1024;
                ld_agent_16Bx4(q, q + 1024, q + 2048, q + 3072, w[0], w[1], w[2], w[3]);
#pragma unroll
                for (int g = 0; g < 4; ++g)
#pragma unroll
                    for (int i = 0; i < 4; ++i) o[ot][4 * g + i] = (p == 0 ? 0.f : o[ot][4 * g + i]) + w[g][i];
            }
        }
    }
    float s1 = 0.f;
#pragma unroll
    for (int ot = 0; ot < 4; ++ot)
#pragma unroll
        for (int r = 0; r < 16; ++r) s1 += o[ot][r];
    float u, v2;
    half_wave_pair(s1, u, v2);
    const float mean = (u + v2) * (1.0f / 128.0f);
    float s2 = 0.f;
#pragma unroll
    for (int ot = 0; ot < 4; ++ot)
#pragma unroll
        for (int r = 0; r < 16; ++r) {
            const float d = o[ot][r] - mean;
            s2 = __builtin_fmaf(d, d, s2);
        }
    half_wave_pair(s2, u, v2);
    const float rstd = 1.0f / sqrtf((u + v2) * (1.0f / 128.0f) + a.eps);
#if UM_FFN_ROWSTORE
    if (role == 0) {
        unsigned char* stg = lds + (KV4 ? 65536 : 0) + pair * 16384;
#pragma unroll
        for (int ot = 0; ot < 4; ++ot)
#pragma unroll
            for (int g = 0; g < 4; ++g) {
                const int n = 32 * ot + 8 * g;
                const f32x4 gm = *reinterpret_cast<const f32x4*>(a.gamma + n + 4 * half);
                const f32x4 bt = *reinterpret_cast<const f32x4*>(a.beta + n + 4 * half);
                f32x4 yv;
#pragma unroll
                for (int i = 0; i < 4; ++i) yv[i] = (o[ot][4 * g + i] - mean) * rstd * gm[i] + bt[i] + rr[4 * ot + g][i];
                *reinterpret_cast<f32x4*>(stg + tl * 512 + (((8 * ot + 2 * g + half) ^ tl) << 4)) = yv;
                if constexpr (KV4) {
#pragma unroll
                    for (int i = 0; i < 4; ++i) o[ot][4 * g + i] = yv[i];
                }
            }
        __builtin_amdgcn_wave_barrier();
        const int cc = lane & 31;
#pragma unroll
        for (int j = 0; j < 16; ++j) {
            const int r = 2 * j + half;
            const f32x4 v = *reinterpret_cast<const f32x4*>(stg + r * 512 + ((cc ^ r) << 4));
            const int trow = m0 + 32 * pair + r;
            if (trow < a.M) UM_FFN_ST(reinterpret_cast<f32x4*>(a.out + (long)trow * 128 + 4 * cc), v);
        }
    }
#else
    if (KV4 ? role == 0 : tok < a.M) {
        const int tokc = min(tok, a.M - 1);
        float* dst = a.out + (long)tokc * 128 + 4 * half;
#pragma unroll
        for (int ot = 0; ot < 4; ++ot)
#pragma unroll
            for (int g = 0; g < 4; ++g) {
                const int n = 32 * ot + 8 * g;
                const f32x4 gm = *reinterpret_cast<const f32x4*>(a.gamma + n + 4 * half);
                const f32x4 bt = *reinterpret_cast<const f32x4*>(a.beta + n + 4 * half);
                f32x4 yv;
#pragma unroll
                for (int i = 0; i < 4; ++i) yv[i] = (o[ot][4 * g + i] - mean) * rstd * gm[i] + bt[i] + rr[4 * ot + g][i];
                if (tok < a.M) UM_FFN_ST(reinterpret_cast<f32x4*>(dst + n), yv);
                if constexpr (KV4) {
#pragma unroll
                    for (int i = 0; i < 4; ++i) o[ot][4 * g + i] = yv[i];
                }
            }
    }
#endif
#ifdef UM_FFN_TRACE
    if (tracing) trace_buf[24 * 8 + 2] = __builtin_amdgcn_s_memtime();
#endif
    if constexpr (KV4) {
        i16x8 yf[NS][8];
        unsigned char* xch = lds + 65536 + pair * 16384 + lane * 16;
        if (role == 0) {
#pragma unroll
            for (int ot = 0; ot < 4; ++ot)
#pragma unroll
                for (int kk = 0; kk < 2; ++kk) {
                    unsigned wh[4], wl[4];
#pragma unroll
                    for (int j = 0; j < 4; ++j) {
                        const float p0 = o[ot][8 * kk + 2 * j], p1 = o[ot][8 * kk + 2 * j + 1];
                        wh[j] = T::pack2(p0, p1);
                        if (NS == 2) wl[j] = T::lo2(p0, p1, wh[j], neg1);
                    }
                    {
                        const auto xx = __builtin_amdgcn_permlane32_swap(wh[0], wh[2], false, false);
                        const auto yy = __builtin_amdgcn_permlane32_swap(wh[1], wh[3], false, false);
                        const u32x4 f = {xx[0], yy[0], xx[1], yy[1]};
                        yf[0][2 * ot + kk] = __builtin_bit_cast(i16x8, f);
                    }
                    if (NS == 2) {
                        const auto xx = __builtin_amdgcn_permlane32_swap(wl[0], wl[2], false, false);
                        const auto yy = __builtin_amdgcn_permlane32_swap(wl[1], wl[3], false, false);
                        const u32x4 f = {xx[0], yy[0], xx[1], yy[1]};
                        yf[NS - 1][2 * ot + kk] = __builtin_bit_cast(i16x8, f);
                    }
                }
#pragma unroll
            for (int pl = 0; pl < NS; ++pl)
#pragma unroll
                for (int ks = 0; ks < 8; ++ks) *reinterpret_cast<i16x8*>(xch + (pl * 8 + ks) * 1024) = yf[pl][ks];
        }
        __syncthreads();
        if (role == 1) {
#pragma unroll
            for (int pl = 0; pl < NS; ++pl)
#pragma unroll
                for (int ks = 0; ks < 8; ++ks) yf[pl][ks] = *reinterpret_cast<const i16x8*>(xch + (pl * 8 + ks) * 1024);
        }
        kv4_project<T, NS, true>(lds, lds + 65536, a.kv, yf, m0, wave, lane, aoff, neg1);
#ifdef UM_FFN_TRACE
        if (tracing) trace_buf[24 * 8 + 3] = __builtin_amdgcn_s_memtime();
#endif
    }
}

extern void um_set_error(const char* fmt, ...);
#ifdef UM_FFN_TRACE
extern "C" int um_debug_set_ffn_trace(void* ptr) {
    return (int)hipMemcpyToSymbol(HIP_SYMBOL(g_um_ffn_trace), &ptr, sizeof(ptr));
}
#endif

template <typename T, int NS, bool HSPLIT, bool KV4 = false>
static hipError_t launch_ffn_impl(const FfnArgs& a, hipStream_t stream) {
    constexpr int LDS = FfnLds<NS>::TOTAL > 131072 ? FfnLds<NS>::TOTAL : (KV4 ? 131072 : FfnLds<NS>::TOTAL);
    static bool configured = false;
    if (!configured) {
        hipError_t e = hipFuncSetAttribute(reinterpret_cast<const void*>(&ffn_kernel<T, NS, HSPLIT, KV4>),
                                           hipFuncAttributeMaxDynamicSharedMemorySize, LDS);
        if (e != hipSuccess) return e;
        configured = true;
    }
    ScopedKernelTimer timer(UM_K_FFN, stream);
    um_census_hit(HSPLIT ? UM_V_FFN_HSPLIT : UM_V_FFN_TILE);
    hipLaunchKernelGGL((ffn_kernel<T, NS, HSPLIT, KV4>), dim3(((a.M + 127) / 128) * a.split), dim3(512), LDS, stream, a);
    return hipGetLastError();
}

template <typename T, int NS>
static hipError_t launch_ffn(const FfnArgs& a, hipStream_t stream) {
    if (a.kv.w) return launch_ffn_impl<T, NS, false, true>(a, stream);
    return a.split > 1 ? launch_ffn_impl<T, NS, true>(a, stream) : launch_ffn_impl<T, NS, false>(a, stream);
}

static int ffn_num_cus() { return um_num_cus(); }

static int ffn_hidden_split(int m, int hidden) {
    static const bool off = um_debug_env("UM_FFN_NO_HSPLIT") != nullptr;
    if (off) return 1;
    const int tiles = (m + 127) / 128, nslice = hidden / 32, cus = ffn_num_cus();
    int split = 1;
    while (split < 4 && tiles * (2 * split) <= cus && nslice % (2 * split) == 0 && nslice / (2 * split) >= 4) split *= 2;
    return split;
}

static size_t ffn_hs_bytes(int m, int split) {
    const size_t tiles = (size_t)((m + 127) / 128);
    return ((tiles * sizeof(unsigned) + 255) & ~(size_t)255) + tiles * split * (64 * 256 * sizeof(float));
}

extern "C" size_t um_ffn_split_workspace_bytes(int m, int hidden) {
    if (m <= 0 || hidden < 64 || hidden % 32 != 0) return 0;
    const int split = ffn_hidden_split(m, hidden);
    return split > 1 ? ffn_hs_bytes(m, split) : 0;
}

extern "C" int um_ffn_ws_fwd(const float* x, const float* y, const void* w1_planes, const void* w2_planes, int m, int hidden,
                             int wshift, const float* gamma, const float* beta, float eps, float* out, int mode, void* workspace,
                             size_t workspace_bytes, void* stream_);

extern "C" int um_ffn_fwd(const float* x, const float* y, const void* w1_planes, const void* w2_planes, int m, int hidden,
                          int wshift, const float* gamma, const float* beta, float eps, float* out, int mode,
                          void* stream_) {
    return um_ffn_ws_fwd(x, y, w1_planes, w2_planes, m, hidden, wshift, gamma, beta, eps, out, mode, nullptr, 0, stream_);
}

extern "C" int um_kv4_fwd(const float* x, const void* wc_planes, int m, int wshift, void* out_planes, int mode, void* stream_);
static int ffn_impl(const float* x, const float* y, const void* w1_planes, const void* w2_planes, int m, int hidden,
                    int wshift, const float* gamma, const float* beta, float eps, float* out, int mode, void* workspace,
                    size_t workspace_bytes, const void* wc_planes, void* kv_planes, void* stream_);

extern "C" int um_ffn_ws_fwd(const float* x, const float* y, const void* w1_planes, const void* w2_planes, int m, int hidden,
                             int wshift, const float* gamma, const float* beta, float eps, float* out, int mode, void* workspace,
                             size_t workspace_bytes, void* stream_) {
    return ffn_impl(x, y, w1_planes, w2_planes, m, hidden, wshift, gamma, beta, eps, out, mode, workspace, workspace_bytes, nullptr,
                    nullptr, stream_);
}

extern "C" int um_ffn_kv_fwd(const float* x, const float* y, const void* w1_planes, const void* w2_planes, int m, int hidden,
                             int wshift, const float* gamma, const float* beta, float eps, float* out, const void* wc_planes,
                             void* kv_planes, int mode, void* workspace, size_t workspace_bytes, void* stream_) {
    if (!wc_planes || !kv_planes) {
        um_set_error("um_ffn_kv_fwd: null k | v weight planes or output planes");
        return -1;
    }
    return ffn_impl(x, y, w1_planes, w2_planes, m, hidden, wshift, gamma, beta, eps, out, mode, workspace, workspace_bytes, wc_planes,
                    kv_planes, stream_);
}

static int ffn_impl(const float* x, const float* y, const void* w1_planes, const void* w2_planes, int m, int hidden,
                    int wshift, const float* gamma, const float* beta, float eps, float* out, int mode, void* workspace,
                    size_t workspace_bytes, const void* wc_planes, void* kv_planes, void* stream_) {
    if (!x || !y || !w1_planes || !w2_planes || !gamma || !beta || !out || m <= 0 || hidden < 64 || hidden % 32 != 0 ||
        (mode != 0 && mode != 1) || wshift < 0 || wshift > 14) {
        um_set_error("um_ffn_fwd: bad argument (m=%d hidden=%d wshift=%d mode=%d; hidden must be a multiple of 32, >= 64)",
                     m, hidden, wshift, mode);
        return -1;
    }
    if ((long)hidden * 256 * 2 >= (1L << 32)) {
        um_set_error("um_ffn_fwd: weight planes beyond 4 GiB are not addressable by this kernel");
        return -4;
    }
    FfnArgs a;
    a.x = x;
    a.y = y;
    a.w1 = (const unsigned short*)w1_planes;
    a.w1_plane_stride = (long)hidden * 256;
    a.w2 = (const unsigned short*)w2_planes;
    a.w2_plane_stride = (long)128 * hidden;
    a.gamma = gamma;
    a.beta = beta;
    a.out = out;
    a.M = m;
    a.hid = hidden;
    a.out_scale = ldexpf(1.f, -wshift);
    a.eps = eps;
    a.split = 1;
    a.hs_part = nullptr;
    a.hs_flag = nullptr;
    a.kv = Kv4Args{};
    a.range_flag = a.kv.range_flag = (mode == 0) ? um_range_flag_dev() : nullptr;
    if (workspace) {
        const int split = ffn_hidden_split(m, hidden);
        if (split > 1 && workspace_bytes >= ffn_hs_bytes(m, split)) {
            const size_t slots = (size_t)((m + 127) / 128);
            a.split = split;
            a.hs_flag = (unsigned*)workspace;
            a.hs_part = (float*)((unsigned char*)workspace + ((slots * sizeof(unsigned) + 255) & ~(size_t)255));
        }
    }
    static const bool no_fuse = um_debug_env("UM_FFN_NO_KV4") != nullptr;
    const bool fuse = wc_planes && a.split == 1 && !no_fuse;
    if (fuse) {
        a.kv.x = nullptr;
        a.kv.w = (const unsigned short*)wc_planes;
        a.kv.w_plane_stride = 256L * 256;
        a.kv.out = (unsigned short*)kv_planes;
        a.kv.out_plane_stride = 4L * m * 128;
        a.kv.M = m;
        a.kv.out_scale = a.out_scale;
    }
    const hipError_t e = mode == 0 ? launch_ffn<Fp16, 2>(a, (hipStream_t)stream_) : launch_ffn<Bf16, 1>(a, (hipStream_t)stream_);
    if (e != hipSuccess) {
        um_set_error("um_ffn_fwd: launch failed: %s", hipGetErrorString(e));
        return (int)e;
    }
    if (wc_planes && !fuse) return um_kv4_fwd(out, wc_planes, m, wshift, kv_planes, mode, stream_);
    return 0;
}

extern "C" int um_kv4_fwd(const float* x, const void* wc_planes, int m, int wshift, void* out_planes, int mode, void* stream_) {
    if (!x || !wc_planes || !out_planes || m <= 0 || (mode != 0 && mode != 1) || wshift < 0 || wshift > 14) {
        um_set_error("um_kv4_fwd: bad argument (m=%d wshift=%d mode=%d)", m, wshift, mode);
        return -1;
    }
    Kv4Args k;
    k.x = x;
    k.w = (const unsigned short*)wc_planes;
    k.w_plane_stride = 256L * 256;
    k.out = (unsigned short*)out_planes;
    k.out_plane_stride = 4L * m * 128;
    k.M = m;
    k.out_scale = ldexpf(1.f, -wshift);
    k.range_flag = (mode == 0) ? um_range_flag_dev() : nullptr;
    hipStream_t stream = (hipStream_t)stream_;
    hipError_t e = hipSuccess;
    ScopedKernelTimer timer(UM_K_LINEAR, stream);
    if (mode == 0) {
        constexpr int LDS = Kv4Lds<2>::RING + Kv4Lds<2>::SCR_BYTES;
        static bool configured = false;
        if (!configured) {
            e = hipFuncSetAttribute(reinterpret_cast<const void*>(&kv4_kernel<Fp16, 2>), hipFuncAttributeMaxDynamicSharedMemorySize, LDS);
            if (e != hipSuccess) return (int)e;
            configured = true;
        }
        hipLaunchKernelGGL((kv4_kernel<Fp16, 2>), dim3((m + 127) / 128), dim3(512), LDS, stream, k);
    } else {
        constexpr int LDS = Kv4Lds<1>::RING + Kv4Lds<1>::SCR_BYTES;
        static bool configured = false;
        if (!configured) {
            e = hipFuncSetAttribute(reinterpret_cast<const void*>(&kv4_kernel<Bf16, 1>), hipFuncAttributeMaxDynamicSharedMemorySize, LDS);
            if (e != hipSuccess) return (int)e;
            configured = true;
        }
        hipLaunchKernelGGL((kv4_kernel<Bf16, 1>), dim3((m + 127) / 128), dim3(512), LDS, stream, k);
    }
    e = hipGetLastError();
    if (e != hipSuccess) {
        um_set_error("um_kv4_fwd: launch failed: %s", hipGetErrorString(e));
        return (int)e;
    }
    return 0;
}
```

unimatch_amd/ops.py:

```python
import contextlib
import ctypes
import threading
import weakref
from collections import namedtuple

import torch

from . import _abi

PRECISIONS = {'exact': _abi.MODE_EXACT, 'fast': _abi.MODE_FAST}


class KernelTimer:

    def __init__(self):
        self.records = []

    def summary(self):
        torch.cuda.synchronize()
        out = {}
        for name, s, e, meta in self.records:
            d = out.setdefault(name, {'calls': 0, 'ms': 0.0, 'meta': meta})
            d['calls'] += 1
            d['ms'] += s.elapsed_time(e)
        return out


def _ptr(t):
    return t.data_ptr()


def _stream():
    return torch.cuda.current_stream().cuda_stream


def _check_tokens(name, t, n=None, tokens=None):
    if not (t.is_cuda and t.dtype == torch.float32 and t.dim() == 3 and t.is_contiguous()):
        raise ValueError(f'{name}: expected a contiguous CUDA float32 [N, L, C] tensor, got '
                         f'{tuple(t.shape)} {t.dtype} {t.device} contiguous={t.is_contiguous()}')
    if n is not None and t.shape[0] != n or tokens is not None and t.shape[1] != tokens:
        raise ValueError(f'{name}: shape {tuple(t.shape)} does not match N={n}, L={tokens}')


def _check_map(name, t, n, h, w):
    if not (t.is_cuda and t.dtype == torch.float32 and t.dim() == 4 and t.is_contiguous()
            and t.shape[0] == n and t.shape[2] == h and t.shape[3] == w):
        raise ValueError(f'{name}: expected a contiguous CUDA float32 [{n}, V, {h}, {w}] tensor, got '
                         f'{tuple(t.shape)} {t.dtype}')


def pack_kv4_weights(weights):
    w4 = torch.cat([w.detach().float() for w in weights], 0)
    perm = torch.arange(32, device=w4.device) ^ 16
    cross = w4[256:].view(8, 32, 128)[:, perm].reshape(256, 128)
    return torch.cat([w4[:256], cross], 1).contiguous()


WorkspaceKey = namedtuple('WorkspaceKey', 'kind geometry device owner')


class _Scope(threading.local):
    token = None
    lane = 0


class WorkspaceRegistry:

    GEOMETRIES = 8

    def __init__(self, stream=None, capturing=None):
        self._entries = {}
        self._scope = _Scope()
        self._stream_handle = stream or _stream
        self._capturing = capturing or torch.cuda.is_current_stream_capturing

    @contextlib.contextmanager
    def graph_scope(self, token):
        prev, self._scope.token = self._scope.token, token
        owned = {}
        try:
            yield owned
        finally:
            self._scope.token = prev
            for k in [k for k in self._entries if isinstance(k.owner, tuple) and k.owner[0] is token]:
                owned[k] = self._entries.pop(k)

    @contextlib.contextmanager
    def part_scope(self, lane):
        prev, self._scope.lane = self._scope.lane, lane
        try:
            yield
        finally:
            self._scope.lane = prev

    def workspace_scope(self):
        return self._scope.token, self._scope.lane

    def workspace_entries(self):
        return list(self._entries.items())

    def _workspace(self, kind, geometry, nbytes, device, keep):
        scope = self._scope
        owner = self._stream_handle() if scope.token is None else (scope.token, scope.lane)
        buf = self._entries.get((kind, geometry, device, owner))
        if buf is None:
            if self._capturing():
                return torch.zeros(nbytes, dtype=torch.uint8, device=device)
            group = [k for k in self._entries if (k.kind, k.device, k.owner) == (kind, device, owner)]
            for k in group[:max(0, len(group) + 1 - keep)]:
                del self._entries[k]
            buf = self._entries[WorkspaceKey(kind, geometry, device, owner)] = torch.zeros(nbytes, dtype=torch.uint8, device=device)
        return buf

    def release_cached_planes(self):
        for k in [k for k in self._entries if isinstance(k.kind, tuple)]:
            del self._entries[k]


class HipOps(WorkspaceRegistry):

    fused_tail = True
    fused_ffn = True
    fused_merge = True
    fused_qproj = True
    block_kv = True
    refine_hoist = True
    fused_kv = True
    fused_conv = True
    norm_on_load = True
    fused_entry = True
    fused_glue = True
    CONV_MODE = 0
    WSHIFT = 10

    def __init__(self, precision='exact'):
        if precision not in PRECISIONS:
            raise ValueError(f'precision must be one of {sorted(PRECISIONS)}')
        self.lib = _abi.load()
        if not torch.cuda.is_available():
            raise _abi.HipExtensionError('no GPU visible: the UniMatch hot path only runs on the HIP extension')
        self.precision = precision
        self.mode = PRECISIONS[precision]
        self.timer = None
        self.nplanes = 2 if precision == 'exact' else 1
        self._wcache = {}
        self.cache_generation = 0
        WorkspaceRegistry.__init__(self)

    def _ws(self, nbytes, device):
        return torch.empty(max(int(nbytes), 256), dtype=torch.uint8, device=device)

    def _launch(self, name, fn, meta=None):
        if self.timer is None:
            return fn()
        s, e = torch.cuda.Event(enable_timing=True), torch.cuda.Event(enable_timing=True)
        s.record()
        r = fn()
        e.record()
        self.timer.records.append((name, s, e, meta))
        return r

    def window_attention(self, q, k, v, h, w, win_h, win_w, shift_h=0, shift_w=0):
        s, l, c = q.shape
        _check_tokens('q', q, tokens=h * w)
        _check_tokens('k', k, s, l)
        _check_tokens('v', v, s, l)
        out = torch.empty_like(q)
        nbytes = self.lib.um_window_attn_workspace_bytes(s, l, c, self.mode)
        ws = self._ws(nbytes, q.device)
        n = win_h * win_w
        meta = {'flops': 4.0 * s * l * n * c, 'bytes': 4.0 * 4 * s * l * c}
        code = self._launch('window_attn', lambda: self.lib.um_window_attn_fwd(
            _ptr(q), _ptr(k), _ptr(v), _ptr(out), s, h, w, c, win_h, win_w, shift_h, shift_w,
            self.mode, _ptr(ws), ws.numel(), _stream()), meta)
        _abi.check(code, 'um_window_attn_fwd')
        return out

    def _cache_get(self, tag, tensors):
        key = (tag,) + tuple((id(t), t._version, t.data_ptr(), str(t.device), t.dtype) for t in tensors)
        hit = self._wcache.get(key)
        if hit is not None and all(r() is t for r, t in zip(hit[0], tensors)):
            return key, hit[1]
        return key, None

    def invalidate_weights(self):
        self._wcache.clear()
        self._entries.clear()
        self.cache_generation += 1

    def _cache_put(self, key, tensors, value):
        if len(self._wcache) > 256:
            self._wcache = {k: v for k, v in self._wcache.items() if all(r() is not None for r in v[0])}
            if len(self._wcache) > 256:
                self._wcache.clear()
        self._wcache[key] = (tuple(weakref.ref(t) for t in tensors), value)
        self.cache_generation += 1
        return value

    def weight_planes(self, weights):
        key, hit = self._cache_get('lin', weights)
        if hit is not None:
            return hit
        w = (weights[0] if len(weights) == 1 else torch.cat(list(weights), 0)).detach().float().contiguous()
        n, k = w.shape
        self._check_weight_range(w, self.WSHIFT if self.mode == 0 else 0, 'Linear weight')
        planes = torch.empty(self.lib.um_planes_bytes(n, k, self.mode), dtype=torch.uint8, device=w.device)
        _abi.check(self.lib.um_weight_planes(_ptr(w), _ptr(planes), n, k, self.WSHIFT, self.mode, _stream()),
                   'um_weight_planes')
        return self._cache_put(key, weights, (planes, n, k))

    @staticmethod
    def _check_weight_range(w, shift, what):
        limit = 65504.0 / float(1 << shift)
        amax = float(w.abs().max()) if w.numel() else 0.0
        if not amax < limit:
            raise ValueError(f'{what}: max |w| = {amax:.4g} does not fit the fp16 operand planes (|w| < {limit:.4g} at the '
                             f'2^{shift} pre-scale; see include/unimatch_hip.h, "Operand range")')

    def _check_rows(self, name, t, k):
        if not (t.is_cuda and t.dtype == torch.float32 and t.dim() == 2 and t.is_contiguous() and t.shape[1] == k):
            raise ValueError(f'{name}: expected a contiguous CUDA float32 [M, {k}] tensor, got {tuple(t.shape)} {t.dtype}')

    def linear_planes(self, a, weights, a1=None, gelu=False, a_planes_k=None):
        wp, n, k = self.weight_planes(weights)
        if a_planes_k is not None:
            m = a.numel() // (2 * self.nplanes * a_planes_k)
            args = (None, None, _ptr(a))
        else:
            m = a.shape[0]
            self._check_rows('a', a, k // 2 if a1 is not None else k)
            if a1 is not None:
                self._check_rows('a1', a1, k // 2)
            args = (_ptr(a), _ptr(a1) if a1 is not None else None, None)
        out = torch.empty(self.lib.um_planes_bytes(m, n, self.mode), dtype=torch.uint8, device=a.device)
        meta = {'flops': 2.0 * m * n * k}
        code = self._launch('linear', lambda: self.lib.um_linear_fwd(
            args[0], args[1], args[2], _ptr(wp), m, n, k, self.WSHIFT, 2 if gelu else 0, _ptr(out),
            None, None, None, 0.0, self.mode, _stream()), meta)
        _abi.check(code, 'um_linear_fwd')
        return out, m, n

    def linear_ln(self, a, weights, norm, residual=None, a_planes_k=None):
        wp, n, k = self.weight_planes(weights)
        if a_planes_k is not None:
            m = a.numel() // (2 * self.nplanes * a_planes_k)
            args = (None, None, _ptr(a))
        else:
            m = a.shape[0]
            self._check_rows('a', a, k)
            args = (_ptr(a), None, None)
        if residual is not None:
            self._check_rows('residual', residual, n)
        out = torch.empty((m, n), dtype=torch.float32, device=a.device)
        code = self._launch('linear', lambda: self.lib.um_linear_fwd(
            args[0], args[1], args[2], _ptr(wp), m, n, k, self.WSHIFT, 1, _ptr(out),
            _ptr(norm.weight), _ptr(norm.bias), _ptr(residual) if residual is not None else None,
            float(norm.eps), self.mode, _stream()), {'flops': 2.0 * m * n * k})
        _abi.check(code, 'um_linear_fwd')
        return out

    def ffn_ln(self, x, y, w1, w2, norm):
        w1p, hid, k1 = self.weight_planes((w1,))
        w2p, n2, k2 = self.weight_planes((w2,))
        if (k1, n2, k2) != (256, 128, hid):
            raise ValueError(f'ffn_ln: expected W1 [hidden, 256] and W2 [128, hidden], got {tuple(w1.shape)} {tuple(w2.shape)}')
        self._check_rows('x', x, 128)
        self._check_rows('y', y, 128)
        m = x.shape[0]
        if y.shape[0] != m:
            raise ValueError('ffn_ln: x and y must have the same number of rows')
        out = torch.empty((m, 128), dtype=torch.float32, device=x.device)
        ws = self._split_workspace('ffn_hsplit', (m, hid), x.device)
        code = self._launch('ffn', lambda: self.lib.um_ffn_ws_fwd(
            _ptr(x), _ptr(y), _ptr(w1p), _ptr(w2p), m, hid, self.WSHIFT, _ptr(norm.weight), _ptr(norm.bias),
            float(norm.eps), _ptr(out), self.mode, _ptr(ws) if ws is not None else None, ws.numel() if ws is not None else 0,
            _stream()), {'flops': 2.0 * m * hid * (256 + 128)})
        _abi.check(code, 'um_ffn_ws_fwd')
        return out

    def ffn_ln_kv(self, x, y, w1, w2, norm, kv_weights):
        w1p, hid, k1 = self.weight_planes((w1,))
        w2p, n2, k2 = self.weight_planes((w2,))
        if (k1, n2, k2) != (256, 128, hid):
            raise ValueError(f'ffn_ln_kv: expected W1 [hidden, 256] and W2 [128, hidden], got {tuple(w1.shape)} {tuple(w2.shape)}')
        self._check_rows('x', x, 128)
        self._check_rows('y', y, 128)
        m = x.shape[0]
        if y.shape[0] != m:
            raise ValueError('ffn_ln_kv: x and y must have the same number of rows')
        wc = self.kv4_weight_planes(kv_weights)
        out = torch.empty((m, 128), dtype=torch.float32, device=x.device)
        kv = torch.empty(self.lib.um_planes_bytes(4 * m, 128, self.mode), dtype=torch.uint8, device=x.device)
        ws = self._split_workspace('ffn_hsplit', (m, hid), x.device)
        code = self._launch('ffn', lambda: self.lib.um_ffn_kv_fwd(
            _ptr(x), _ptr(y), _ptr(w1p), _ptr(w2p), m, hid, self.WSHIFT, _ptr(norm.weight), _ptr(norm.bias),
            float(norm.eps), _ptr(out), _ptr(wc), _ptr(kv), self.mode, _ptr(ws) if ws is not None else None,
            ws.numel() if ws is not None else 0, _stream()), {'flops': 2.0 * m * hid * (256 + 128) + 2.0 * m * 512 * 128})
        _abi.check(code, 'um_ffn_kv_fwd')
        return out, kv

    def window_attention_planes(self, q, k, v, streams, h, w, win_h, win_w, shift_h=0, shift_w=0, kv_rotate=0):
        (qt, qrows, qcols, qoff), (kt, krows, kcols, koff), (vt, vrows, vcols, voff) = q, k, v
        if (krows, kcols) != (vrows, vcols) or qrows != streams * h * w or krows != qrows:
            raise ValueError('inconsistent plane shapes')
        out = torch.empty((streams, h * w, 128), dtype=torch.float32, device=qt.device)
        n = win_h * win_w
        meta = {'flops': 4.0 * streams * h * w * n * 128}
        code = self._launch('window_attn', lambda: self.lib.um_window_attn_planes_fwd(
            _ptr(qt) + 2 * qoff, _ptr(kt) + 2 * koff, _ptr(vt) + 2 * voff, _ptr(out), streams, h, w, 128,
            qcols, kcols, qrows * qcols, krows * kcols, win_h, win_w, shift_h, shift_w, kv_rotate, self.mode, _stream()), meta)
        _abi.check(code, 'um_window_attn_planes_fwd')
        return out

    def window_attention_merge(self, q, k, v, streams, h, w, win_h, win_w, shift_h, shift_w, kv_rotate, merge_weight, norm,
                               residual=None):
        (qt, qrows, qcols, qoff), (kt, krows, kcols, koff), (vt, vrows, vcols, voff) = q, k, v
        if (krows, kcols) != (vrows, vcols) or qrows != streams * h * w or krows != qrows:
            raise ValueError('inconsistent plane shapes')
        wp, n, kk = self.weight_planes((merge_weight,))
        if (n, kk) != (128, 128):
            raise ValueError('window_attention_merge: the merge weight must be [128, 128]')
        if residual is not None:
            self._check_rows('residual', residual, 128)
        out = torch.empty((streams, h * w, 128), dtype=torch.float32, device=qt.device)
        meta = {'flops': 4.0 * streams * h * w * win_h * win_w * 128}
        code = self._launch('window_attn', lambda: self.lib.um_window_attn_merge_fwd(
            _ptr(qt) + 2 * qoff, _ptr(kt) + 2 * koff, _ptr(vt) + 2 * voff, _ptr(wp), _ptr(norm.weight), _ptr(norm.bias),
            _ptr(residual) if residual is not None else None, float(norm.eps), self.WSHIFT, _ptr(out), streams, h, w, 128,
            qcols, kcols, qrows * qcols, krows * kcols, win_h, win_w, shift_h, shift_w, kv_rotate, self.mode, _stream()), meta)
        _abi.check(code, 'um_window_attn_merge_fwd')
        return out

    def _split_workspace(self, kind, geometry, device):
        size = self.lib.um_window_attn_ksplit_workspace_bytes if kind == 'attn_ksplit' else self.lib.um_ffn_split_workspace_bytes
        nbytes = size(*geometry)
        return self._workspace(kind, geometry, nbytes, device, self.GEOMETRIES) if nbytes else None

    def window_attention_qproj_merge(self, x, q_weight, k, v, streams, h, w, win_h, win_w, shift_h, shift_w, kv_rotate,
                                     merge_weight, norm, residual=None):
        (kt, krows, kcols, koff), (vt, vrows, vcols, voff) = k[:4], v[:4]
        kps = k[4] if len(k) > 4 else krows * kcols
        if (v[4] if len(v) > 4 else vrows * vcols) != kps:
            raise ValueError('k and v must share their plane stride')
        self._check_rows('x', x, 128)
        if (krows, kcols) != (vrows, vcols) or x.shape[0] != streams * h * w or krows != x.shape[0]:
            raise ValueError('inconsistent plane shapes')
        wqp, nq, kq = self.weight_planes((q_weight,))
        wp, n, kk = self.weight_planes((merge_weight,))
        if (n, kk, nq, kq) != (128, 128, 128, 128):
            raise ValueError('window_attention_qproj_merge: the query and merge weights must be [128, 128]')
        if residual is not None:
            self._check_rows('residual', residual, 128)
        out = torch.empty((streams, h * w, 128), dtype=torch.float32, device=x.device)
        meta = {'flops': 4.0 * streams * h * w * win_h * win_w * 128}
        ks = self._split_workspace('attn_ksplit', (streams, h, w, win_h, win_w), x.device)
        code = self._launch('window_attn', lambda: self.lib.um_window_attn_qproj_merge_fwd(
            _ptr(x), _ptr(wqp), _ptr(kt) + 2 * koff, _ptr(vt) + 2 * voff, _ptr(wp), _ptr(norm.weight), _ptr(norm.bias),
            _ptr(residual) if residual is not None else None, float(norm.eps), self.WSHIFT, _ptr(out), streams, h, w, 128,
            kcols, kps, win_h, win_w, shift_h, shift_w, kv_rotate, self.mode,
            _ptr(ks) if ks is not None else None, ks.numel() if ks is not None else 0, _stream()), meta)
        _abi.check(code, 'um_window_attn_qproj_merge_fwd')
        return out

    def kv4_weight_planes(self, weights):
        key, hit = self._cache_get('kv4', weights)
        if hit is not None:
            return hit
        if len(weights) != 4 or any(tuple(w.shape) != (128, 128) for w in weights):
            raise ValueError('kv4_weight_planes: expected four [128, 128] weights (k_self, v_self, k_cross, v_cross)')
        wc = pack_kv4_weights(weights)
        self._check_weight_range(wc, self.WSHIFT if self.mode == 0 else 0, 'Linear weight')
        planes = torch.empty(self.lib.um_planes_bytes(256, 256, self.mode), dtype=torch.uint8, device=wc.device)
        _abi.check(self.lib.um_weight_planes(_ptr(wc), _ptr(planes), 256, 256, self.WSHIFT, self.mode, _stream()), 'um_weight_planes')
        return self._cache_put(key, weights, planes)

    @staticmethod
    def kv4_slices(kv, m):
        part = lambda j: (kv, m, 128, j * m * 128, 4 * m * 128)
        return (part(0), part(1)), (part(2), part(3))

    def kv4_planes(self, x, weights):
        self._check_rows('x', x, 128)
        wc = self.kv4_weight_planes(weights)
        m = x.shape[0]
        out = torch.empty(self.lib.um_planes_bytes(4 * m, 128, self.mode), dtype=torch.uint8, device=x.device)
        code = self._launch('linear', lambda: self.lib.um_kv4_fwd(_ptr(x), _ptr(wc), m, self.WSHIFT, _ptr(out), self.mode, _stream()),
                            {'flops': 2.0 * m * 512 * 128})
        _abi.check(code, 'um_kv4_fwd')
        return out

    def convex_upsample(self, flow, mask, factor, is_depth=False, mask_nhwc=False, out=None):
        b, v, h, w = flow.shape
        want = (b * h * w, 9 * factor * factor) if mask_nhwc else (b, 9 * factor * factor, h, w)
        if not (flow.is_cuda and flow.dtype == torch.float32 and mask.dtype == torch.float32 and tuple(mask.shape) == want):
            raise ValueError(f'convex_upsample: bad shapes flow {tuple(flow.shape)} mask {tuple(mask.shape)}')
        flow, mask = flow.contiguous(), mask.contiguous()
        up = out
        if up is None:
            up = torch.empty((b, v, factor * h, factor * w), dtype=torch.float32, device=flow.device)
        elif not (tuple(up.shape) == (b, v, factor * h, factor * w) and up.dtype == torch.float32 and up.device == flow.device
                  and up.is_contiguous()):
            raise ValueError(f'convex_upsample: out must be a contiguous float32 [{b}, {v}, {factor * h}, {factor * w}] tensor on '
                             f'{flow.device}, got {tuple(up.shape)} {up.dtype} {up.device}')
        code = self._launch('convex_upsample', lambda: self.lib.um_convex_upsample(
            _ptr(flow), _ptr(mask), _ptr(up), b, v, h, w, factor, int(bool(is_depth)), int(bool(mask_nhwc)), _stream()))
        _abi.check(code, 'um_convex_upsample')
        return up

    def flow_warp(self, tokens, flow, h, w):
        b, l, c = tokens.shape
        if not (tokens.is_cuda and tokens.dtype == torch.float32 and tokens.is_contiguous() and l == h * w
                and tuple(flow.shape) == (b, 2, h, w) and flow.dtype == torch.float32):
            raise ValueError(f'flow_warp: bad shapes tokens {tuple(tokens.shape)} flow {tuple(flow.shape)}')
        flow = flow.contiguous()
        out = torch.empty_like(tokens)
        code = self._launch('convex_upsample', lambda: self.lib.um_flow_warp(
            _ptr(tokens), _ptr(flow), _ptr(out), b, h, w, c, _stream()))
        _abi.check(code, 'um_flow_warp')
        return out

    def fwd_bwd_occlusion(self, fwd, bwd, alpha=0.01, beta=0.5):
        if not (fwd.is_cuda and fwd.dtype == torch.float32 and fwd.dim() == 4 and fwd.shape[1] == 2
                and bwd.shape == fwd.shape and bwd.dtype == torch.float32 and bwd.device == fwd.device):
            raise ValueError(f'fwd_bwd_occlusion: expected two CUDA float32 [B, 2, H, W] flows of one shape, got '
                             f'{tuple(fwd.shape)} {fwd.dtype} and {tuple(bwd.shape)} {bwd.dtype}')
        fwd, bwd = fwd.contiguous(), bwd.contiguous()
        b, _, h, w = fwd.shape
        occ_f = torch.empty((b, h, w), dtype=torch.float32, device=fwd.device)
        occ_b = torch.empty_like(occ_f)
        code = self._launch('fwd_bwd_occlusion', lambda: self.lib.um_fwd_bwd_occlusion(
            _ptr(fwd), _ptr(bwd), _ptr(occ_f), _ptr(occ_b), b, h, w, float(alpha), float(beta), _stream()))
        _abi.check(code, 'um_fwd_bwd_occlusion')
        return occ_f, occ_b

    def flow_to_rgb(self, flow):
        if not (flow.is_cuda and flow.dtype == torch.float32 and flow.dim() == 4 and flow.shape[1] == 2):
            raise ValueError(f'flow_to_rgb: expected a CUDA float32 [B, 2, H, W] flow, got {tuple(flow.shape)} {flow.dtype}')
        flow = flow.contiguous()
        b, _, h, w = flow.shape
        rgb = torch.empty((b, h, w, 3), dtype=torch.uint8, device=flow.device)
        ws = self._ws(self.lib.um_flow_to_rgb_workspace_bytes(b, h, w), flow.device)
        code = self._launch('flow_to_rgb', lambda: self.lib.um_flow_to_rgb(
            _ptr(flow), _ptr(rgb), b, h, w, _ptr(ws), ws.numel(), _stream()))
        _abi.check(code, 'um_flow_to_rgb')
        return rgb

    def flow_chain(self, flow, occ=None, points=None, alive=None, stride=1):
        if not (flow.is_cuda and flow.dtype == torch.float32 and flow.dim() == 4 and flow.shape[1] == 2):
            raise ValueError(f'flow_chain: flow: expected a CUDA float32 [P, 2, H, W] tensor, got {tuple(flow.shape)} {flow.dtype}')
        p, _, h, w = flow.shape
        if occ is not None and not (occ.dtype == torch.float32 and occ.device == flow.device and tuple(occ.shape) == (p, h, w)):
            raise ValueError(f'flow_chain: occ: expected float32 {(p, h, w)} on {flow.device}, got {tuple(occ.shape)} {occ.dtype} '
                             f'on {occ.device}')
        if points is not None:
            if not (points.dtype == torch.float32 and points.device == flow.device and points.dim() == 2 and points.shape[1] == 2):
                raise ValueError(f'flow_chain: points: expected float32 [N, 2] on {flow.device}, got {tuple(points.shape)} '
                                 f'{points.dtype} on {points.device}')
            n = points.shape[0]
            points = points.contiguous()
        else:
            if int(stride) < 1:
                raise ValueError(f'flow_chain: stride must be >= 1, got {stride}')
            n = -(-h // int(stride)) * -(-w // int(stride))
        if alive is not None:
            if not (alive.dtype == torch.bool and alive.device == flow.device and tuple(alive.shape) == (n,)):
                raise ValueError(f'flow_chain: alive: expected bool {(n,)} on {flow.device}, got {tuple(alive.shape)} {alive.dtype} '
                                 f'on {alive.device}')
            alive = alive.contiguous().view(torch.uint8)
        flow = flow.contiguous()
        occ = None if occ is None else occ.contiguous()
        tracks = torch.empty((p, n, 2), dtype=torch.float32, device=flow.device)
        visible = torch.empty((p, n), dtype=torch.uint8, device=flow.device)
        opt = lambda t: None if t is None else _ptr(t)
        code = self._launch('flow_chain', lambda: self.lib.um_flow_chain(
            _ptr(flow), opt(occ), opt(points), opt(alive), _ptr(tracks), _ptr(visible), p, h, w, n, int(stride), _stream()),
            {'bytes': 21.0 * p * n})
        _abi.check(code, 'um_flow_chain')
        return tracks, visible.view(torch.bool)

    @staticmethod
    def _check_sizing(name, mode, size, crop):
        if mode not in ('pad', 'resize'):
            raise ValueError(f"{name}: mode must be 'pad' or 'resize', got {mode!r}")
        (hp, wp), (top, left) = (int(s) for s in size), (int(c) for c in crop)
        if hp < 1 or wp < 1:
            raise ValueError(f'{name}: the inference size {hp}x{wp} is empty')
        return (1 if mode == 'resize' else 0), hp, wp, top, left

    def image_prepare(self, images, size, mode='pad', crop=(0, 0), transpose=False, mean=None, std=None, hflip=False, out=None):
        u8 = images.dtype == torch.uint8
        ok = images.is_cuda and images.dim() == 4 and (u8 or images.dtype == torch.float32) and images.shape[3 if u8 else 1] == 3
        if not ok:
            raise ValueError(f'image_prepare: expected a CUDA float32 [B, 3, H, W] or uint8 [B, H, W, 3] tensor, got '
                             f'{tuple(images.shape)} {images.dtype} {images.device}')
        if (mean is None) != (std is None) or (mean is not None and (len(mean) != 3 or len(std) != 3)):
            raise ValueError('image_prepare: mean and std are three floats each, given together')
        m, hp, wp, top, left = self._check_sizing('image_prepare', mode, size, crop)
        images = images.contiguous()
        b = images.shape[0]
        h, w = (images.shape[1:3] if u8 else images.shape[2:])
        ih, iw = (w, h) if transpose else (h, w)
        if m == 0 and (top < 0 or left < 0 or top + ih > hp or left + iw > wp):
            raise ValueError(f'image_prepare: the image {ih}x{iw} at ({top}, {left}) leaves the padded size {hp}x{wp}')
        if out is None:
            out = torch.empty((b, 3, hp, wp), dtype=torch.float32, device=images.device)
        elif not (out.is_cuda and out.device == images.device and out.dtype == torch.float32 and tuple(out.shape) == (b, 3, hp, wp)
                  and out.is_contiguous()):
            raise ValueError(f'image_prepare: out must be a contiguous CUDA float32 [{b}, 3, {hp}, {wp}] tensor on {images.device}, got '
                             f'{tuple(out.shape)} {out.dtype} {out.device}')
        fmean = (ctypes.c_float * 3)(*mean) if mean is not None else None
        fstd = (ctypes.c_float * 3)(*std) if std is not None else None
        code = self._launch('image_prepare', lambda: self.lib.um_image_prepare_flip(
            _ptr(images), 1 if u8 else 0, _ptr(out), b, h, w, int(bool(transpose)), fmean, fstd, m, hp, wp, top, left, int(bool(hflip)),
            _stream()))
        _abi.check(code, 'um_image_prepare_flip')
        return out

    def pred_restore(self, pred, size, mode='pad', crop=(0, 0), kind='flow', transpose=False, hflip=False, out=None):
        kinds = {'flow': 0, 'disparity': 1, 'depth': 2}
        if kind not in kinds:
            raise ValueError(f'pred_restore: kind must be one of {sorted(kinds)}, got {kind!r}')
        if not (pred.is_cuda and pred.dtype == torch.float32 and pred.dim() == 4 and pred.shape[1] == (2 if kind == 'flow' else 1)):
            raise ValueError(f"pred_restore: expected a CUDA float32 [B, {2 if kind == 'flow' else 1}, hp, wp] {kind}, got "
                             f'{tuple(pred.shape)} {pred.dtype} {pred.device}')
        m, h, w, top, left = self._check_sizing('pred_restore', mode, size, crop)
        pred = pred.contiguous()
        b, c, hp, wp = pred.shape
        ih, iw = (w, h) if transpose else (h, w)
        if m == 0 and (top < 0 or left < 0 or top + ih > hp or left + iw > wp):
            raise ValueError(f'pred_restore: the crop {ih}x{iw} at ({top}, {left}) leaves the prediction {hp}x{wp}')
        if out is None:
            out = torch.empty((b, c, h, w), dtype=torch.float32, device=pred.device)
        elif not (out.is_cuda and out.device == pred.device and out.dtype == torch.float32 and tuple(out.shape) == (b, c, h, w)
                  and out.is_contiguous()):
            raise ValueError(f'pred_restore: out must be a contiguous CUDA float32 [{b}, {c}, {h}, {w}] tensor on {pred.device}, got '
                             f'{tuple(out.shape)} {out.dtype} {out.device}')
        code = self._launch('pred_restore', lambda: self.lib.um_pred_restore_flip(
            _ptr(pred), _ptr(out), b, c, hp, wp, m, top, left, h, w, kinds[kind], int(bool(transpose)), int(bool(hflip)), _stream()))
        _abi.check(code, 'um_pred_restore_flip')
        return out

    NORMS = {'minmax_255': 0, 'min_p95_256': 1}

    def scalar_to_rgb(self, x, lut, inverse=False, norm='minmax_255', return_stats=False):
        if norm not in self.NORMS:
            raise ValueError(f'scalar_to_rgb: norm must be one of {sorted(self.NORMS)}, got {norm!r}')
        if not (x.is_cuda and x.dtype == torch.float32 and x.dim() == 3):
            raise ValueError(f'scalar_to_rgb: expected a CUDA float32 [B, H, W] tensor, got {tuple(x.shape)} {x.dtype} {x.device}')
        if not (lut.is_cuda and lut.device == x.device and lut.dtype == torch.uint8 and tuple(lut.shape) == (256, 3) and lut.is_contiguous()):
            raise ValueError(f'scalar_to_rgb: expected a contiguous uint8 [256, 3] table on {x.device}, got {tuple(lut.shape)} {lut.dtype} '
                             f'{lut.device}')
        x = x.contiguous()
        b, h, w = x.shape
        rgb = torch.empty((b, h, w, 3), dtype=torch.uint8, device=x.device)
        stats = torch.empty((b, 2), dtype=torch.float32, device=x.device) if return_stats else None
        ws = self._ws(self.lib.um_scalar_to_rgb_workspace_bytes(b, h, w), x.device)
        code = self._launch('scalar_to_rgb', lambda: self.lib.um_scalar_to_rgb(
            _ptr(x), _ptr(rgb), b, h, w, int(bool(inverse)), self.NORMS[norm], _ptr(lut), _ptr(stats) if return_stats else None,
            _ptr(ws), ws.numel(), _stream()))
        _abi.check(code, 'um_scalar_to_rgb')
        return (rgb, stats) if return_stats else rgb

    @staticmethod
    def _metric_args(name, pred, gt, channels, crop, masks):
        want = 4 if channels else 3
        ok = (pred.is_cuda and pred.dtype == torch.float32 and gt.dtype == torch.float32 and gt.device == pred.device
              and pred.dim() == want and gt.dim() == want and gt.shape[0] == pred.shape[0]
              and (not channels or (pred.shape[1] == channels and gt.shape[1] == channels)))
        if not ok:
            raise ValueError(f'{name}: expected CUDA float32 pred / gt of {want} dimensions and one batch, got {tuple(pred.shape)} '
                             f'{pred.dtype} and {tuple(gt.shape)} {gt.dtype}')
        b, (hp, wp), (h, w) = pred.shape[0], pred.shape[-2:], gt.shape[-2:]
        top, left = (int(crop[0]), int(crop[1])) if crop is not None else (0, 0)
        if top < 0 or left < 0 or top + h > hp or left + w > wp:
            raise ValueError(f'{name}: the crop {h}x{w} at ({top}, {left}) leaves the prediction {hp}x{wp}')
        out = []
        for m in masks:
            if m is not None:
                if not (m.is_cuda and m.device == pred.device and tuple(m.shape) == (b, h, w)):
                    raise ValueError(f'{name}: expected a CUDA mask [{b}, {h}, {w}], got {tuple(m.shape)} on {m.device}')
                m = m.float().contiguous()
            out.append(m)
        return pred.contiguous(), gt.contiguous(), out, (b, hp, wp, h, w, top, left)

    def flow_metrics(self, pred, gt, valid=None, noc_valid=None, crop=None):
        pred, gt, (valid, noc_valid), (b, hp, wp, h, w, top, left) = self._metric_args('flow_metrics', pred, gt, 2, crop, (valid, noc_valid))
        rows = torch.empty((b, 16), dtype=torch.float64, device=pred.device)
        ws = self._ws(self.lib.um_flow_metrics_workspace_bytes(b, h, w), pred.device)
        code = self._launch('flow_metrics', lambda: self.lib.um_flow_metrics(
            _ptr(pred), _ptr(gt), _ptr(valid) if valid is not None else None, _ptr(noc_valid) if noc_valid is not None else None,
            _ptr(rows), b, hp, wp, h, w, top, left, _ptr(ws), ws.numel(), _stream()))
        _abi.check(code, 'um_flow_metrics')
        return rows

    def disp_metrics(self, pred, gt, max_disp=0.0, crop=None):
        pred, gt, _, (b, hp, wp, h, w, top, left) = self._metric_args('disp_metrics', pred, gt, 0, crop, ())
        rows = torch.empty((b, 8), dtype=torch.float64, device=pred.device)
        ws = self._ws(self.lib.um_disp_metrics_workspace_bytes(b, h, w), pred.device)
        code = self._launch('disp_metrics', lambda: self.lib.um_disp_metrics(
            _ptr(pred), _ptr(gt), _ptr(rows), b, hp, wp, h, w, top, left, float(max_disp), _ptr(ws), ws.numel(), _stream()))
        _abi.check(code, 'um_disp_metrics')
# ... 668 lines not shown
```

Baseline: 961.2.

## Make FFN kernel persistent with a per-workgroup tile loop and overlapped next-tile loads

Restructures the FFN kernel so each workgroup loops over several 128-row tiles with stride gridDim.x, instead of launching one workgroup per tile. The grid is sized to about the CU count with balanced tiles per workgroup. The next tile's rows and first W1 chunk are prefetched while the current tile finishes, and in the KV4 path the ring slot is released early. This targets launch, tail and prologue costs, but adds register pressure, which the new resource guards try to bound, and more complex synchronisation.

```diff
diff --git a/include/unimatch_hip.h b/include/unimatch_hip.h
--- a/include/unimatch_hip.h
+++ b/include/unimatch_hip.h
@@ -120,6 +120,13 @@
 int um_ffn_kv_fwd(const float* x, const float* y, const void* w1_planes, const void* w2_planes, int m, int hidden, int wshift,
                   const float* gamma, const float* beta, float eps, float* out, const void* wc_planes, void* kv_planes, int mode,
                   void* workspace, size_t workspace_bytes, void* stream);
+int um_ffn_plan(int m, int* workgroups, int* tiles_per_wg_max);
+int um_ffn_ws_fwd_ex(const float* x, const float* y, const void* w1_planes, const void* w2_planes, int m, int hidden,
+                     int wshift, const float* gamma, const float* beta, float eps, float* out, int mode, void* workspace,
+                     size_t workspace_bytes, int grid_limit, void* stream);
+int um_ffn_kv_fwd_ex(const float* x, const float* y, const void* w1_planes, const void* w2_planes, int m, int hidden, int wshift,
+                     const float* gamma, const float* beta, float eps, float* out, const void* wc_planes, void* kv_planes, int mode,
+                     void* workspace, size_t workspace_bytes, int grid_limit, void* stream);
 
 int um_conv2d_fwd(const void* a_planes, const void* w_planes, const float* bias, float* out, float* stats_out, int batch,
                   int hi, int wi, int cin, int cout, int kh, int kw, int stride, int pad_h, int pad_w, int relu, int wshift,
diff --git a/unimatch_amd/_abi.py b/unimatch_amd/_abi.py
--- a/unimatch_amd/_abi.py
+++ b/unimatch_amd/_abi.py
@@ -38,6 +38,11 @@
     'um_ffn_kv_fwd': (_c_int, [_c_void_p] * 4 + [_c_int] * 3 + [_c_void_p] * 2 + [ctypes.c_float, _c_void_p, _c_void_p, _c_void_p, _c_int, _c_void_p,
                                 _c_size_t, _c_void_p]),
     'um_kv4_fwd': (_c_int, [_c_void_p, _c_void_p, _c_int, _c_int, _c_void_p, _c_int, _c_void_p]),
+    'um_ffn_plan': (_c_int, [_c_int] + [ctypes.POINTER(_c_int)] * 2),
+    'um_ffn_ws_fwd_ex': (_c_int, [_c_void_p] * 4 + [_c_int] * 3 + [_c_void_p] * 2 + [ctypes.c_float, _c_void_p, _c_int, _c_void_p, _c_size_t,
+                                   _c_int, _c_void_p]),
+    'um_ffn_kv_fwd_ex': (_c_int, [_c_void_p] * 4 + [_c_int] * 3 + [_c_void_p] * 2 + [ctypes.c_float, _c_void_p, _c_void_p, _c_void_p, _c_int,
+                                   _c_void_p, _c_size_t, _c_int, _c_void_p]),
     'um_conv2d_fwd': (_c_int, [_c_void_p] * 5 + [_c_int] * 13 + [_c_void_p]),
     'um_conv2d_addend_fwd': (_c_int, [_c_void_p] * 4 + [_c_int, _c_int, _c_void_p] + [_c_int] * 12 + [_c_void_p]),
     'um_conv2d_ex': (_c_int, [_c_void_p, _c_int, _c_int, ctypes.c_long, _c_void_p, _c_void_p, _c_void_p, _c_int, _c_int, _c_void_p,
diff --git a/unimatch_amd/build.py b/unimatch_amd/build.py
--- a/unimatch_amd/build.py
+++ b/unimatch_amd/build.py
@@ -20,6 +20,7 @@
                'geometry.hip': ['-ffp-contract=off', '-fhip-fp32-correctly-rounded-divide-sqrt'],
                'match_stats.hip': ['-fno-slp-vectorize', '-fhip-fp32-correctly-rounded-divide-sqrt', '-Wno-inline-asm']}
 RESOURCE_GUARDS = {'conv.hip': {'conv_entry_kernel': 2},
+                   'ffn.hip': {'ffn_kernel': 2, 'kv4_kernelI4Fp16': 3, 'kv4_kernelI4Bf16': 5},
                    'geometry.hip': {'disp_consistency_kernel': 4, 'depth_consistency_kernel': 4, 'points_count_kernel': 4,
                                     'points_scan_kernel': 4, 'points_scatter_kernel': 4},
                    'match_stats.hip': {'match_stats_kernel': 2, 'match_mutual_kernel': 4}}
diff --git a/unimatch_amd/csrc/ffn.hip b/unimatch_amd/csrc/ffn.hip
--- a/unimatch_amd/csrc/ffn.hip
+++ b/unimatch_amd/csrc/ffn.hip
@@ -8,7 +8,8 @@
 
 #ifdef UM_FFN_TRACE
 __device__ unsigned long long* g_um_ffn_trace = nullptr;
-#define UM_FSTAMP(slot) do { if (tracing && i < 24) trace_buf[(i) * 8 + (slot)] = __builtin_amdgcn_s_memtime(); } while (0)
+#define UM_FSTAMP(slot) do { if (tracing && trip == 0 && i < 24) trace_buf[(i) * 8 + (slot)] = __builtin_amdgcn_s_memtime(); \
+                             if (tracing && trip == 1 && i == 0 && (slot) == 0) trace_buf[24 * 8 + 4] = __builtin_amdgcn_s_memtime(); } while (0)
 #else
 #define UM_FSTAMP(slot) do { } while (0)
 #endif
@@ -149,9 +150,9 @@
     static constexpr int SCR_BYTES = 8 * SCRW;
 };
 
-template <typename T, int NS, bool CHUNK0_ISSUED>
+template <typename T, int NS, bool CHUNK0_ISSUED, class F>
 __device__ __forceinline__ void kv4_project(unsigned char* ring, unsigned char* scr, const Kv4Args& k, const i16x8 (&yf)[NS][8],
-                                            int m0, int wave, int lane, const int (&aoff)[8], float neg1) {
+                                            int m0, int wave, int lane, const int (&aoff)[8], float neg1, F ring_slot0_free) {
     using L = FfnLds<NS>;
     const int pair = wave & 3, role = wave >> 2;
     const int half = lane >> 5, tl = lane & 31;
@@ -190,6 +191,7 @@
         asm volatile("s_waitcnt vmcnt(0)" ::: "memory");
         __syncthreads();
         if (c + 1 < 8) dma(c + 1, slot ^ 1);
+        else ring_slot0_free();
         if (c > 0) store_chunk(c - 1);
         const unsigned char* w1s = ring + slot * L::W1S;
         f32x16 acc;
@@ -277,7 +279,13 @@
     int aoff[8];
 #pragma unroll
     for (int ks = 0; ks < 8; ++ks) aoff[ks] = arow * 512 + (((16 * role + 2 * ks + half) ^ arow) << 4);
-    kv4_project<T, NS, false>(lds, lds + Kv4Lds<NS>::RING, k, yf, m0, wave, lane, aoff, neg1);
+    kv4_project<T, NS, false>(lds, lds + Kv4Lds<NS>::RING, k, yf, m0, wave, lane, aoff, neg1, [] {});
+}
+
+template <class V, int N>
+__device__ __forceinline__ void um_fresh(V (&v)[N]) {
+#pragma unroll
+    for (int i = 0; i < N; ++i) asm volatile("" : "=v"(v[i]));
 }
 
 template <typename T, int NS, bool HSPLIT = false, bool KV4 = false>
@@ -285,16 +293,35 @@
     using L = FfnLds<NS>;
     extern __shared__ __attribute__((aligned(16))) unsigned char lds[];
 
-    const int tid = threadIdx.x, lane = tid & 63;
+    const int tid = threadIdx.x;
     const float neg1 = um_opaque_neg1();
     const int wave = __builtin_amdgcn_readfirstlane(tid >> 6);
     const int pair = wave & 3, role = wave >> 2;
-    const int half = lane >> 5, tl = lane & 31;
+    int lane = tid & 63, half, tl, arow;
+    int aoff[8], boff[4];
+    unsigned char* xb_out;
+    const unsigned char* xb_in;
+    auto lane_setup = [&]() {
+        asm volatile("" : "+v"(lane));
+        half = lane >> 5;
+        tl = lane & 31;
+        arow = tl ^ (16 * role);
+#pragma unroll
+        for (int ks = 0; ks < 8; ++ks) aoff[ks] = arow * 512 + (((16 * role + 2 * ks + half) ^ arow) << 4);
+#pragma unroll
+        for (int ot = 0; ot < 4; ++ot) {
+            const int r = 32 * ot + tl;
+            boff[ot] = L::W2_OFF + r * 64 + (((2 * role + half) ^ ((r >> 2) & 3)) << 4);
+        }
+        xb_out = lds + L::XB_OFF + wave * L::XB + lane * 16;
+        xb_in = lds + L::XB_OFF + (wave ^ 4) * L::XB + lane * 16;
+    };
+    lane_setup();
     const int nsplit = HSPLIT ? a.split : 1;
-    const int tile_id = HSPLIT ? (int)blockIdx.x / nsplit : (int)blockIdx.x;
+    int tile_id = HSPLIT ? (int)blockIdx.x / nsplit : (int)blockIdx.x;
     const int part = HSPLIT ? (int)blockIdx.x - tile_id * nsplit : 0;
-    const int m0 = tile_id * 128;
-    const int tok = m0 + 32 * pair + tl;
+    const int ntiles = (a.M + 127) >> 7;
+    int m0 = tile_id * 128;
     const int nslice = (a.hid >> 5) / nsplit;
     const int sbase = part * nslice;
 
@@ -321,6 +348,7 @@
     const bool tracing = g_um_ffn_trace != nullptr && (blockIdx.x % 37) == 0 && lane == 0 && pair == 0;
     unsigned long long* trace_buf = g_um_ffn_trace + ((size_t)(blockIdx.x / 37) * 2 + role) * (24 * 8 + 8);
     if (tracing) trace_buf[24 * 8] = __builtin_amdgcn_s_memtime();
+    int trip = 0;
 #endif
     const unsigned lds_wave = __builtin_amdgcn_readfirstlane(
         (unsigned)(unsigned long)(const __attribute__((address_space(3))) unsigned char*)lds) + (unsigned)wave * 1024u;
@@ -359,14 +387,22 @@
 
     dma_w1(0, 0);
 
+    f32x4 xraw[16];
+    auto load_rows = [&](int t) {
+        const float* src = (role ? a.y : a.x) + (long)min(t, a.M - 1) * 128 + 8 * half;
+#pragma unroll
+        for (int ks = 0; ks < 8; ++ks) {
+            xraw[2 * ks] = UM_FFN_LD(reinterpret_cast<const f32x4*>(src + 16 * ks));
+            xraw[2 * ks + 1] = UM_FFN_LD(reinterpret_cast<const f32x4*>(src + 16 * ks + 4));
+        }
+    };
+    load_rows(m0 + 32 * pair + tl);
     i16x8 xf[NS][8];
-    {
-        const float* src = (role ? a.y : a.x) + (long)min(tok, a.M - 1) * 128 + 8 * half;
+    auto split_rows = [&]() {
         float xmx = 0.f;
 #pragma unroll
         for (int ks = 0; ks < 8; ++ks) {
-            const f32x4 v0 = UM_FFN_LD(reinterpret_cast<const f32x4*>(src + 16 * ks));
-            const f32x4 v1 = UM_FFN_LD(reinterpret_cast<const f32x4*>(src + 16 * ks + 4));
+            const f32x4 v0 = xraw[2 * ks], v1 = xraw[2 * ks + 1];
 #pragma unroll
             for (int j = 0; j < 4; ++j) xmx = fmaxf(xmx, fmaxf(__builtin_fabsf(v0[j]), __builtin_fabsf(v1[j])));
             const u32x4 h = {T::pack2(v0[0], v0[1]), T::pack2(v0[2], v0[3]), T::pack2(v1[0], v1[1]), T::pack2(v1[2], v1[3])};
@@ -378,26 +414,9 @@
             }
         }
         um_range_note<T>(a.range_flag, xmx, UM_RANGE_FFN_TOKENS);
-    }
+    };
 
     f32x16 o[4];
-#pragma unroll
-    for (int ot = 0; ot < 4; ++ot)
-#pragma unroll
-        for (int r = 0; r < 16; ++r) o[ot][r] = 0.f;
-
-    const int arow = tl ^ (16 * role);
-    int aoff[8];
-#pragma unroll
-    for (int ks = 0; ks < 8; ++ks) aoff[ks] = arow * 512 + (((16 * role + 2 * ks + half) ^ arow) << 4);
-    int boff[4];
-#pragma unroll
-    for (int ot = 0; ot < 4; ++ot) {
-        const int r = 32 * ot + tl;
-        boff[ot] = L::W2_OFF + r * 64 + (((2 * role + half) ^ ((r >> 2) & 3)) << 4);
-    }
-    unsigned char* xb_out = lds + L::XB_OFF + wave * L::XB + lane * 16;
-    const unsigned char* xb_in = lds + L::XB_OFF + (wave ^ 4) * L::XB + lane * 16;
 
     auto phase_a = [&](const unsigned char* w1s, f32x16& sc) {
 #pragma unroll
@@ -429,25 +448,7 @@
         *reinterpret_cast<f32x4*>(p + 1024) = f32x4{sc[12], sc[13], sc[14], sc[15]};
     };
 
-    asm volatile("s_waitcnt vmcnt(0)" ::: "memory");
-    __syncthreads();
-    if (nslice > 1) dma_w1(1, 1);
-
     f32x16 sc;
-    __builtin_amdgcn_s_setprio(1);
-    phase_a(lds + L::W1_OFF, sc);
-    {
-        constexpr int RD = NS, MF = (NS == 2) ? 3 : 1;
-        __builtin_amdgcn_sched_group_barrier(0x100, 2 * RD, 0);
-#pragma unroll
-        for (int ks = 0; ks < 6; ++ks) {
-            __builtin_amdgcn_sched_group_barrier(0x008, MF, 0);
-            __builtin_amdgcn_sched_group_barrier(0x100, RD, 0);
-        }
-        __builtin_amdgcn_sched_group_barrier(0x008, 2 * MF, 0);
-    }
-    __builtin_amdgcn_s_setprio(0);
-    send(sc, 0);
 
     struct Frag {
         unsigned wh[4], wl[4];
@@ -790,251 +791,328 @@
         UM_FSTAMP(5);
     };
 
-    if (UM_FFN_ORDER == 1) {
-        using Y = std::true_type;
-        using N = std::false_type;
-        using S0 = std::integral_constant<int, 0>;
-        using S1 = std::integral_constant<int, 1>;
-        if ((nslice & 1) == 0 && nslice >= 4) {
-            iteration1(Y{}, N{}, Y{}, S0{}, 0);
-            int i = 1;
-            for (; i + 4 < nslice; i += 2) {
-                iteration1(Y{}, Y{}, Y{}, S1{}, i);
-                iteration1(Y{}, Y{}, Y{}, S0{}, i + 1);
-            }
-            iteration1(Y{}, Y{}, Y{}, S1{}, nslice - 3);
-            iteration1(Y{}, Y{}, N{}, S0{}, nslice - 2);
-            iteration1(N{}, Y{}, N{}, S1{}, nslice - 1);
-        } else {
-            if (2 < nslice) iteration1(Y{}, N{}, Y{}, 0, 0);
-            else iteration1(Y{}, N{}, N{}, 0, 0);
-            int i = 1;
-            for (; i + 2 < nslice; ++i) iteration1(Y{}, Y{}, Y{}, i & 1, i);
-            for (; i + 1 < nslice; ++i) iteration1(Y{}, Y{}, N{}, i & 1, i);
-            iteration1(N{}, Y{}, N{}, (nslice - 1) & 1, nslice - 1);
-        }
-    } else {
-        iteration(std::true_type{}, std::false_type{}, 0);
-        for (int i = 1; i + 1 < nslice; ++i) iteration(std::true_type{}, std::true_type{}, i);
-        iteration(std::false_type{}, std::true_type{}, nslice - 1);
-    }
-    f32x4 rr[16];
-    {
-        const unsigned char* w2s = lds + ((nslice - 1) & 1) * L::W2S;
+    int next_tile = 0;
+    bool has_next = false;
+    auto next_tile_w1 = [&]() {
+        lane_setup();
+        if constexpr (!KV4) {
+            __syncthreads();
+            dma_w1(0, 0);
+        }
+#ifdef UM_FFN_TRACE
+        ++trip;
+#endif
+        tile_id = next_tile;
+        m0 = tile_id * 128;
+    };
+#pragma unroll 1
+    for (;; next_tile_w1()) {
+        split_rows();
+#pragma unroll
+        for (int ot = 0; ot < 4; ++ot)
+#pragma unroll
+            for (int r = 0; r < 16; ++r) o[ot][r] = 0.f;
+        hmx = 0.f;
+        next_tile = tile_id + (int)gridDim.x;
+        has_next = !HSPLIT && next_tile < ntiles;
+
         asm volatile("s_waitcnt vmcnt(0)" ::: "memory");
         __syncthreads();
+        if (nslice > 1) dma_w1(1, 1);
+
+        __builtin_amdgcn_s_setprio(1);
+        phase_a(lds + L::W1_OFF, sc);
+        {
+            constexpr int RD = NS, MF = (NS == 2) ? 3 : 1;
+            __builtin_amdgcn_sched_group_barrier(0x100, 2 * RD, 0);
+#pragma unroll
+            for (int ks = 0; ks < 6; ++ks) {
+                __builtin_amdgcn_sched_group_barrier(0x008, MF, 0);
+                __builtin_amdgcn_sched_group_barrier(0x100, RD, 0);
+            }
+            __builtin_amdgcn_sched_group_barrier(0x008, 2 * MF, 0);
+        }
+        __builtin_amdgcn_s_setprio(0);
+        send(sc, 0);
+
+        if (UM_FFN_ORDER == 1) {
+            using Y = std::true_type;
+            using N = std::false_type;
+            using S0 = std::integral_constant<int, 0>;
+            using S1 = std::integral_constant<int, 1>;
+            if ((nslice & 1) == 0 && nslice >= 4) {
+                iteration1(Y{}, N{}, Y{}, S0{}, 0);
+                int i = 1;
+                for (; i + 4 < nslice; i += 2) {
+                    iteration1(Y{}, Y{}, Y{}, S1{}, i);
+                    iteration1(Y{}, Y{}, Y{}, S0{}, i + 1);
+                }
+                iteration1(Y{}, Y{}, Y{}, S1{}, nslice - 3);
+                iteration1(Y{}, Y{}, N{}, S0{}, nslice - 2);
+                iteration1(N{}, Y{}, N{}, S1{}, nslice - 1);
+            } else {
+                if (2 < nslice) iteration1(Y{}, N{}, Y{}, 0, 0);
+                else iteration1(Y{}, N{}, N{}, 0, 0);
+                int i = 1;
+                for (; i + 2 < nslice; ++i) iteration1(Y{}, Y{}, Y{}, i & 1, i);
+                for (; i + 1 < nslice; ++i) iteration1(Y{}, Y{}, N{}, i & 1, i);
+                iteration1(N{}, Y{}, N{}, (nslice - 1) & 1, nslice - 1);
+            }
+        } else {
+            iteration(std::true_type{}, std::false_type{}, 0);
+            for (int i = 1; i + 1 < nslice; ++i) iteration(std::true_type{}, std::true_type{}, i);
+            iteration(std::false_type{}, std::true_type{}, nslice - 1);
+        }
+        f32x4 rr[16];
+        um_fresh(rr);
+        {
+            const unsigned char* w2s = lds + ((nslice - 1) & 1) * L::W2S;
+            asm volatile("s_waitcnt vmcnt(0)" ::: "memory");
+            __syncthreads();
+            if (role == 0) {
+                const float* res = a.x + (long)min(m0 + 32 * pair + tl, a.M - 1) * 128 + 4 * half;
+#pragma unroll
+                for (int q = 0; q < 16; ++q)
+                    rr[q] = (UM_FFN_ABL & 32) ? f32x4{0.f, 0.f, 0.f, 0.f} : UM_FFN_LD(reinterpret_cast<const f32x4*>(res + 8 * q));
+            }
+            if (!(UM_FFN_ABL & 8)) {
+#pragma unroll
+                for (int ot = 0; ot < 4; ++ot) {
+                    const i16x8 vh = *reinterpret_cast<const i16x8*>(w2s + boff[ot]);
+                    if (NS == 2) {
+                        const i16x8 vl = *reinterpret_cast<const i16x8*>(w2s + L::W2P + boff[ot]);
+                        o[ot] = T::mfma(vl, pf[0], o[ot]);
+                        if (!UM_FFN_H1) o[ot] = T::mfma(vh, pf[NS - 1], o[ot]);
+                    }
+                    o[ot] = T::mfma(vh, pf[0], o[ot]);
+                }
+            }
+        }
+
+#ifdef UM_FFN_TRACE
+        if (tracing && trip == 0) trace_buf[24 * 8 + 1] = __builtin_amdgcn_s_memtime();
+#endif
+        um_range_note<T>(a.range_flag, hmx, UM_RANGE_FFN_HIDDEN);
+        __syncthreads();
+        static_assert(!(KV4 && HSPLIT), "the k | v epilogue runs on whole tiles only");
+        if constexpr (KV4) {
+#pragma unroll
+            for (int i = 0; i < 2; ++i) {
+                const int blk = 8 * i + wave;
+                const int r = 2 * blk + half, cc = tl ^ r;
+                const unsigned off = (unsigned)((((long)r) * 256 + 8 * cc) * 2);
+#pragma unroll
+                for (int pl = 0; pl < NS; ++pl)
+                    ffn_dma16(a.kv.w + pl * a.kv.w_plane_stride, off, lds + pl * L::W1P + blk * 1024);
+            }
+        }
+        unsigned char* ob = lds + (KV4 ? 65536 : 0) + pair * 16384 + lane * 16;
+        if (role == 1) {
+#pragma unroll
+            for (int ot = 0; ot < 4; ++ot)
+#pragma unroll
+                for (int g = 0; g < 4; ++g)
+                    *reinterpret_cast<f32x4*>(ob + (4 * ot + g) * 1024) =
+                        f32x4{o[ot][4 * g], o[ot][4 * g + 1], o[ot][4 * g + 2], o[ot][4 * g + 3]};
+        }
+        __syncthreads();
+        if (!HSPLIT && !KV4 && role == 1) {
+            um_fresh(xraw);
+            if (!has_next) return;
+            load_rows(next_tile * 128 + 32 * pair + tl);
+            continue;
+        }
         if (role == 0) {
-            const float* res = a.x + (long)min(tok, a.M - 1) * 128 + 4 * half;
-#pragma unroll
-            for (int q = 0; q < 16; ++q)
-                rr[q] = (UM_FFN_ABL & 32) ? f32x4{0.f, 0.f, 0.f, 0.f} : UM_FFN_LD(reinterpret_cast<const f32x4*>(res + 8 * q));
-        }
-        if (!(UM_FFN_ABL & 8)) {
-#pragma unroll
-            for (int ot = 0; ot < 4; ++ot) {
-                const i16x8 vh = *reinterpret_cast<const i16x8*>(w2s + boff[ot]);
-                if (NS == 2) {
-                    const i16x8 vl = *reinterpret_cast<const i16x8*>(w2s + L::W2P + boff[ot]);
-                    o[ot] = T::mfma(vl, pf[0], o[ot]);
-                    if (!UM_FFN_H1) o[ot] = T::mfma(vh, pf[NS - 1], o[ot]);
-                }
-                o[ot] = T::mfma(vh, pf[0], o[ot]);
-            }
-        }
-    }
-
+#pragma unroll
+            for (int ot = 0; ot < 4; ++ot)
+#pragma unroll
+                for (int g = 0; g < 4; ++g) {
+                    const f32x4 r = *reinterpret_cast<const f32x4*>(ob + (4 * ot + g) * 1024);
+#pragma unroll
+                    for (int i = 0; i < 4; ++i) o[ot][4 * g + i] = (o[ot][4 * g + i] + r[i]) * a.out_scale;
+                }
+        }
+        if constexpr (HSPLIT) {
+            const int t4 = 64 * pair + lane;
+            constexpr int HS_SLOT = 16 * 256 * 4;
+            if (role == 0) {
+                float* mine = a.hs_part + ((long)tile_id * nsplit + part) * HS_SLOT + 4 * t4;
+#pragma unroll
+                for (int ot = 0; ot < 4; ++ot)
+#pragma unroll
+                    for (int g = 0; g < 4; ++g) {
+                        const f32x4 v = {o[ot][4 * g], o[ot][4 * g + 1], o[ot][4 * g + 2], o[ot][4 * g + 3]};
+                        st_agent_16B(mine + (ot * 4 + g) * 1024, v);
+                    }
+            }
+            asm volatile("s_waitcnt vmcnt(0)" ::: "memory");
+            __syncthreads();
+            unsigned* ticket = reinterpret_cast<unsigned*>(lds);
+            if (tid == 0) *ticket = __hip_atomic_fetch_add(a.hs_flag + tile_id, 1u, __ATOMIC_RELAXED, __HIP_MEMORY_SCOPE_AGENT);
+            __syncthreads();
+            const unsigned my_ticket = *ticket;
+            __syncthreads();
+            if (my_ticket != (unsigned)(nsplit - 1)) return;
+            asm volatile("buffer_inv sc1" ::: "memory");
+            if (tid == 0) __hip_atomic_store(a.hs_flag + tile_id, 0u, __ATOMIC_RELAXED, __HIP_MEMORY_SCOPE_AGENT);
+            if (role == 1) return;
+            for (int p = 0; p < nsplit; ++p) {
+                const float* pr = a.hs_part + ((long)tile_id * nsplit + p) * HS_SLOT + 4 * t4;
+#pragma unroll
+                for (int ot = 0; ot < 4; ++ot) {
+                    f32x4 w[4];
+                    const float* q = pr + ot * 4 * 1024;
+                    ld_agent_16Bx4(q, q + 1024, q + 2048, q + 3072, w[0], w[1], w[2], w[3]);
+#pragma unroll
+                    for (int g = 0; g < 4; ++g)
+#pragma unroll
+                        for (int i = 0; i < 4; ++i) o[ot][4 * g + i] = (p == 0 ? 0.f : o[ot][4 * g + i]) + w[g][i];
+                }
+            }
+        }
+        if (role == 0) {
+            float s1 = 0.f;
+#pragma unroll
+            for (int ot = 0; ot < 4; ++ot)
+#pragma unroll
+                for (int r = 0; r < 16; ++r) s1 += o[ot][r];
+            float u, v2;
+            half_wave_pair(s1, u, v2);
+            const float mean = (u + v2) * (1.0f / 128.0f);
+            float s2 = 0.f;
+#pragma unroll
+            for (int ot = 0; ot < 4; ++ot)
+#pragma unroll
+                for (int r = 0; r < 16; ++r) {
+                    const float d = o[ot][r] - mean;
+                    s2 = __builtin_fmaf(d, d, s2);
+                }
+            half_wave_pair(s2, u, v2);
+            const float rstd = 1.0f / sqrtf((u + v2) * (1.0f / 128.0f) + a.eps);
+#if UM_FFN_ROWSTORE
+            {
+                unsigned char* stg = lds + (KV4 ? 65536 : 0) + pair * 16384;
+                f32x4 gmv[2][4], btv[2][4];
+                auto load_gb = [&](int ot) {
+#pragma unroll
+                    for (int g = 0; g < 4; ++g) {
+                        gmv[ot & 1][g] = *reinterpret_cast<const f32x4*>(a.gamma + 32 * ot + 8 * g + 4 * half);
+                        btv[ot & 1][g] = *reinterpret_cast<const f32x4*>(a.beta + 32 * ot + 8 * g + 4 * half);
+                    }
+                };
+                load_gb(0);
+#pragma unroll
+                for (int ot = 0; ot < 4; ++ot) {
+                    if (ot + 1 < 4) load_gb(ot + 1);
+                    __builtin_amdgcn_sched_barrier(0);
+#pragma unroll
+                    for (int g = 0; g < 4; ++g) {
+                        const f32x4 gm = gmv[ot & 1][g], bt = btv[ot & 1][g];
+                        f32x4 yv;
+#pragma unroll
+                        for (int i = 0; i < 4; ++i) yv[i] = (o[ot][4 * g + i] - mean) * rstd * gm[i] + bt[i] + rr[4 * ot + g][i];
+                        *reinterpret_cast<f32x4*>(stg + tl * 512 + (((8 * ot + 2 * g + half) ^ tl) << 4)) = yv;
+                        if constexpr (KV4) {
+#pragma unroll
+                            for (int i = 0; i < 4; ++i) o[ot][4 * g + i] = yv[i];
+                        }
+                    }
+                    __builtin_amdgcn_sched_barrier(0);
+                }
+                if constexpr (!HSPLIT) {
+                    um_fresh(xraw);
+                    if (has_next) load_rows(next_tile * 128 + 32 * pair + tl);
+                }
+                __builtin_amdgcn_wave_barrier();
+                const int cc = lane & 31;
+#pragma unroll
+                for (int j = 0; j < 16; ++j) {
+                    const int r = 2 * j + half;
+                    const f32x4 v = *reinterpret_cast<const f32x4*>(stg + r * 512 + ((cc ^ r) << 4));
+                    const int trow = m0 + 32 * pair + r;
+                    if (trow < a.M) UM_FFN_ST(reinterpret_cast<f32x4*>(a.out + (long)trow * 128 + 4 * cc), v);
+                }
+            }
+#else
+            const int tok = m0 + 32 * pair + tl;
+            if (KV4 || tok < a.M) {
+                const int tokc = min(tok, a.M - 1);
+                float* dst = a.out + (long)tokc * 128 + 4 * half;
+#pragma unroll
+                for (int ot = 0; ot < 4; ++ot)
+#pragma unroll
+                    for (int g = 0; g < 4; ++g) {
+                        const int n = 32 * ot + 8 * g;
+                        const f32x4 gm = *reinterpret_cast<const f32x4*>(a.gamma + n + 4 * half);
+                        const f32x4 bt = *reinterpret_cast<const f32x4*>(a.beta + n + 4 * half);
+                        f32x4 yv;
+#pragma unroll
+                        for (int i = 0; i < 4; ++i) yv[i] = (o[ot][4 * g + i] - mean) * rstd * gm[i] + bt[i] + rr[4 * ot + g][i];
+                        if (tok < a.M) UM_FFN_ST(reinterpret_cast<f32x4*>(dst + n), yv);
+                        if constexpr (KV4) {
+#pragma unroll
+                            for (int i = 0; i < 4; ++i) o[ot][4 * g + i] = yv[i];
+                        }
+                    }
+            }
+#endif
+        } else if constexpr (!HSPLIT) {
+            um_fresh(xraw);
+            if (has_next) load_rows(next_tile * 128 + 32 * pair + tl);
+        }
 #ifdef UM_FFN_TRACE
-    if (tracing) trace_buf[24 * 8 + 1] = __builtin_amdgcn_s_memtime();
-#endif
-    um_range_note<T>(a.range_flag, hmx, UM_RANGE_FFN_HIDDEN);
-    __syncthreads();
-    static_assert(!(KV4 && HSPLIT), "the k | v epilogue runs on whole tiles only");
-    if constexpr (KV4) {
-#pragma unroll
-        for (int i = 0; i < 2; ++i) {
-            const int blk = 8 * i + wave;
-            const int r = 2 * blk + half, cc = tl ^ r;
-            const unsigned off = (unsigned)((((long)r) * 256 + 8 * cc) * 2);
-#pragma unroll
-            for (int pl = 0; pl < NS; ++pl)
-                ffn_dma16(a.kv.w + pl * a.kv.w_plane_stride, off, lds + pl * L::W1P + blk * 1024);
-        }
-    }
-    unsigned char* ob = lds + (KV4 ? 65536 : 0) + pair * 16384 + lane * 16;
-    if (role == 1) {
-#pragma unroll
-        for (int ot = 0; ot < 4; ++ot)
-#pragma unroll
-            for (int g = 0; g < 4; ++g)
-                *reinterpret_cast<f32x4*>(ob + (4 * ot + g) * 1024) =
-                    f32x4{o[ot][4 * g], o[ot][4 * g + 1], o[ot][4 * g + 2], o[ot][4 * g + 3]};
-    }
-    __syncthreads();
-    if (!HSPLIT && !KV4 && role == 1) return;
-    if (role == 0) {
-#pragma unroll
-        for (int ot = 0; ot < 4; ++ot)
-#pragma unroll
-            for (int g = 0; g < 4; ++g) {
-                const f32x4 r = *reinterpret_cast<const f32x4*>(ob + (4 * ot + g) * 1024);
-#pragma unroll
-                for (int i = 0; i < 4; ++i) o[ot][4 * g + i] = (o[ot][4 * g + i] + r[i]) * a.out_scale;
-            }
-    }
-    if constexpr (HSPLIT) {
-        const int t4 = 64 * pair + lane;
-        constexpr int HS_SLOT = 16 * 256 * 4;
-        if (role == 0) {
-            float* mine = a.hs_part + ((long)tile_id * nsplit + part) * HS_SLOT + 4 * t4;
-#pragma unroll
-            for (int ot = 0; ot < 4; ++ot)
-#pragma unroll
-                for (int g = 0; g < 4; ++g) {
-                    const f32x4 v = {o[ot][4 * g], o[ot][4 * g + 1], o[ot][4 * g + 2], o[ot][4 * g + 3]};
-                    st_agent_16B(mine + (ot * 4 + g) * 1024, v);
-                }
-        }
-        asm volatile("s_waitcnt vmcnt(0)" ::: "memory");
-        __syncthreads();
-        unsigned* ticket = reinterpret_cast<unsigned*>(lds);
-        if (tid == 0) *ticket = __hip_atomic_fetch_add(a.hs_flag + tile_id, 1u, __ATOMIC_RELAXED, __HIP_MEMORY_SCOPE_AGENT);
-        __syncthreads();
-        const unsigned my_ticket = *ticket;
-        __syncthreads();
-        if (my_ticket != (unsigned)(nsplit - 1)) return;
-        asm volatile("buffer_inv sc1" ::: "memory");
-        if (tid == 0) __hip_atomic_store(a.hs_flag + tile_id, 0u, __ATOMIC_RELAXED, __HIP_MEMORY_SCOPE_AGENT);
-        if (role == 1) return;
-        for (int p = 0; p < nsplit; ++p) {
-            const float* pr = a.hs_part + ((long)tile_id * nsplit + p) * HS_SLOT + 4 * t4;
-#pragma unroll
-            for (int ot = 0; ot < 4; ++ot) {
-                f32x4 w[4];
-                const float* q = pr + ot * 4 * 1024;
-                ld_agent_16Bx4(q, q + 1024, q + 2048, q + 3072, w[0], w[1], w[2], w[3]);
-#pragma unroll
-                for (int g = 0; g < 4; ++g)
-#pragma unroll
-                    for (int i = 0; i < 4; ++i) o[ot][4 * g + i] = (p == 0 ? 0.f : o[ot][4 * g + i]) + w[g][i];
-            }
-        }
-    }
-    float s1 = 0.f;
-#pragma unroll
-    for (int ot = 0; ot < 4; ++ot)
-#pragma unroll
-        for (int r = 0; r < 16; ++r) s1 += o[ot][r];
-    float u, v2;
-    half_wave_pair(s1, u, v2);
-    const float mean = (u + v2) * (1.0f / 128.0f);
-    float s2 = 0.f;
-#pragma unroll
-    for (int ot = 0; ot < 4; ++ot)
-#pragma unroll
-        for (int r = 0; r < 16; ++r) {
-            const float d = o[ot][r] - mean;
-            s2 = __builtin_fmaf(d, d, s2);
-        }
-    half_wave_pair(s2, u, v2);
-    const float rstd = 1.0f / sqrtf((u + v2) * (1.0f / 128.0f) + a.eps);
-#if UM_FFN_ROWSTORE
-    if (role == 0) {
-        unsigned char* stg = lds + (KV4 ? 65536 : 0) + pair * 16384;
-#pragma unroll
-        for (int ot = 0; ot < 4; ++ot)
-#pragma unroll
-            for (int g = 0; g < 4; ++g) {
-                const int n = 32 * ot + 8 * g;
-                const f32x4 gm = *reinterpret_cast<const f32x4*>(a.gamma + n + 4 * half);
-                const f32x4 bt = *reinterpret_cast<const f32x4*>(a.beta + n + 4 * half);
-                f32x4 yv;
-#pragma unroll
-                for (int i = 0; i < 4; ++i) yv[i] = (o[ot][4 * g + i] - mean) * rstd * gm[i] + bt[i] + rr[4 * ot + g][i];
-                *reinterpret_cast<f32x4*>(stg + tl * 512 + (((8 * ot + 2 * g + half) ^ tl) << 4)) = yv;
-                if constexpr (KV4) {
-#pragma unroll
-                    for (int i = 0; i < 4; ++i) o[ot][4 * g + i] = yv[i];
-                }
-            }
-        __builtin_amdgcn_wave_barrier();
-        const int cc = lane & 31;
-#pragma unroll
-        for (int j = 0; j < 16; ++j) {
-            const int r = 2 * j + half;
-            const f32x4 v = *reinterpret_cast<const f32x4*>(stg + r * 512 + ((cc ^ r) << 4));
-            const int trow = m0 + 32 * pair + r;
-            if (trow < a.M) UM_FFN_ST(reinterpret_cast<f32x4*>(a.out + (long)trow * 128 + 4 * cc), v);
-        }
-    }
-#else
-    if (KV4 ? role == 0 : tok < a.M) {
-        const int tokc = min(tok, a.M - 1);
-        float* dst = a.out + (long)tokc * 128 + 4 * half;
-#pragma unroll
-        for (int ot = 0; ot < 4; ++ot)
-#pragma unroll
-            for (int g = 0; g < 4; ++g) {
-                const int n = 32 * ot + 8 * g;
-                const f32x4 gm = *reinterpret_cast<const f32x4*>(a.gamma + n + 4 * half);
-                const f32x4 bt = *reinterpret_cast<const f32x4*>(a.beta + n + 4 * half);
-                f32x4 yv;
-#pragma unroll
-                for (int i = 0; i < 4; ++i) yv[i] = (o[ot][4 * g + i] - mean) * rstd * gm[i] + bt[i] + rr[4 * ot + g][i];
-                if (tok < a.M) UM_FFN_ST(reinterpret_cast<f32x4*>(dst + n), yv);
-                if constexpr (KV4) {
-#pragma unroll
-                    for (int i = 0; i < 4; ++i) o[ot][4 * g + i] = yv[i];
-                }
-            }
-    }
-#endif
+        if (tracing && trip == 0) trace_buf[24 * 8 + 2] = __builtin_amdgcn_s_memtime();
+#endif
+        if constexpr (KV4) {
+            i16x8 yf[NS][8];
+#pragma unroll
+            for (int pl = 0; pl < NS; ++pl) um_fresh(yf[pl]);
+            unsigned char* xch = lds + 65536 + pair * 16384 + lane * 16;
+            if (role == 0) {
+#pragma unroll
+                for (int ot = 0; ot < 4; ++ot)
+#pragma unroll
+                    for (int kk = 0; kk < 2; ++kk) {
+                        unsigned wh[4], wl[4];
+#pragma unroll
+                        for (int j = 0; j < 4; ++j) {
+                            const float p0 = o[ot][8 * kk + 2 * j], p1 = o[ot][8 * kk + 2 * j + 1];
+                            wh[j] = T::pack2(p0, p1);
+                            if (NS == 2) wl[j] = T::lo2(p0, p1, wh[j], neg1);
+                        }
+                        {
+                            const auto xx = __builtin_amdgcn_permlane32_swap(wh[0], wh[2], false, false);
+                            const auto yy = __builtin_amdgcn_permlane32_swap(wh[1], wh[3], false, false);
+                            const u32x4 f = {xx[0], yy[0], xx[1], yy[1]};
+                            yf[0][2 * ot + kk] = __builtin_bit_cast(i16x8, f);
+                        }
+                        if (NS == 2) {
+                            const auto xx = __builtin_amdgcn_permlane32_swap(wl[0], wl[2], false, false);
+                            const auto yy = __builtin_amdgcn_permlane32_swap(wl[1], wl[3], false, false);
+                            const u32x4 f = {xx[0], yy[0], xx[1], yy[1]};
+                            yf[NS - 1][2 * ot + kk] = __builtin_bit_cast(i16x8, f);
+                        }
+                    }
+#pragma unroll
+                for (int pl = 0; pl < NS; ++pl)
+#pragma unroll
+                    for (int ks = 0; ks < 8; ++ks) *reinterpret_cast<i16x8*>(xch + (pl * 8 + ks) * 1024) = yf[pl][ks];
+            }
+            __syncthreads();
+            if (role == 1) {
+#pragma unroll
+                for (int pl = 0; pl < NS; ++pl)
+#pragma unroll
+                    for (int ks = 0; ks < 8; ++ks) yf[pl][ks] = *reinterpret_cast<const i16x8*>(xch + (pl * 8 + ks) * 1024);
+            }
+            kv4_project<T, NS, true>(lds, lds + 65536, a.kv, yf, m0, wave, lane, aoff, neg1, [&] {
+                if (has_next) dma_w1(0, 0);
+            });
 #ifdef UM_FFN_TRACE
-    if (tracing) trace_buf[24 * 8 + 2] = __builtin_amdgcn_s_memtime();
-#endif
-    if constexpr (KV4) {
-        i16x8 yf[NS][8];
-        unsigned char* xch = lds + 65536 + pair * 16384 + lane * 16;
-        if (role == 0) {
-#pragma unroll
-            for (int ot = 0; ot < 4; ++ot)
-#pragma unroll
-                for (int kk = 0; kk < 2; ++kk) {
-                    unsigned wh[4], wl[4];
-#pragma unroll
-                    for (int j = 0; j < 4; ++j) {
-                        const float p0 = o[ot][8 * kk + 2 * j], p1 = o[ot][8 * kk + 2 * j + 1];
-                        wh[j] = T::pack2(p0, p1);
-                        if (NS == 2) wl[j] = T::lo2(p0, p1, wh[j], neg1);
-                    }
-                    {
-                        const auto xx = __builtin_amdgcn_permlane32_swap(wh[0], wh[2], false, false);
-                        const auto yy = __builtin_amdgcn_permlane32_swap(wh[1], wh[3], false, false);
-                        const u32x4 f = {xx[0], yy[0], xx[1], yy[1]};
-                        yf[0][2 * ot + kk] = __builtin_bit_cast(i16x8, f);
-                    }
-                    if (NS == 2) {
-                        const auto xx = __builtin_amdgcn_permlane32_swap(wl[0], wl[2], false, false);
-                        const auto yy = __builtin_amdgcn_permlane32_swap(wl[1], wl[3], false, false);
-                        const u32x4 f = {xx[0], yy[0], xx[1], yy[1]};
-                        yf[NS - 1][2 * ot + kk] = __builtin_bit_cast(i16x8, f);
-                    }
-                }
-#pragma unroll
-            for (int pl = 0; pl < NS; ++pl)
-#pragma unroll
-                for (int ks = 0; ks < 8; ++ks) *reinterpret_cast<i16x8*>(xch + (pl * 8 + ks) * 1024) = yf[pl][ks];
-        }
-        __syncthreads();
-        if (role == 1) {
-#pragma unroll
-            for (int pl = 0; pl < NS; ++pl)
-#pragma unroll
-                for (int ks = 0; ks < 8; ++ks) yf[pl][ks] = *reinterpret_cast<const i16x8*>(xch + (pl * 8 + ks) * 1024);
-        }
-        kv4_project<T, NS, true>(lds, lds + 65536, a.kv, yf, m0, wave, lane, aoff, neg1);
-#ifdef UM_FFN_TRACE
-        if (tracing) trace_buf[24 * 8 + 3] = __builtin_amdgcn_s_memtime();
-#endif
+            if (tracing && trip == 0) trace_buf[24 * 8 + 3] = __builtin_amdgcn_s_memtime();
+#endif
+        }
+        if (!has_next) return;
     }
 }
 
@@ -1046,7 +1124,7 @@
 #endif
 
 template <typename T, int NS, bool HSPLIT, bool KV4 = false>
-static hipError_t launch_ffn_impl(const FfnArgs& a, hipStream_t stream) {
+static hipError_t launch_ffn_impl(const FfnArgs& a, int workgroups, hipStream_t stream) {
     constexpr int LDS = FfnLds<NS>::TOTAL > 131072 ? FfnLds<NS>::TOTAL : (KV4 ? 131072 : FfnLds<NS>::TOTAL);
     static bool configured = false;
     if (!configured) {
@@ -1057,14 +1135,15 @@
     }
     ScopedKernelTimer timer(UM_K_FFN, stream);
     um_census_hit(HSPLIT ? UM_V_FFN_HSPLIT : UM_V_FFN_TILE);
-    hipLaunchKernelGGL((ffn_kernel<T, NS, HSPLIT, KV4>), dim3(((a.M + 127) / 128) * a.split), dim3(512), LDS, stream, a);
+    const int tiles = (a.M + 127) / 128;
+    hipLaunchKernelGGL((ffn_kernel<T, NS, HSPLIT, KV4>), dim3(HSPLIT ? tiles * a.split : workgroups), dim3(512), LDS, stream, a);
     return hipGetLastError();
 }
 
 template <typename T, int NS>
-static hipError_t launch_ffn(const FfnArgs& a, hipStream_t stream) {
-    if (a.kv.w) return launch_ffn_impl<T, NS, false, true>(a, stream);
-    return a.split > 1 ? launch_ffn_impl<T, NS, true>(a, stream) : launch_ffn_impl<T, NS, false>(a, stream);
+static hipError_t launch_ffn(const FfnArgs& a, int workgroups, hipStream_t stream) {
+    if (a.kv.w) return launch_ffn_impl<T, NS, false, true>(a, workgroups, stream);
+    return a.split > 1 ? launch_ffn_impl<T, NS, true>(a, workgroups, stream) : launch_ffn_impl<T, NS, false>(a, workgroups, stream);
 }
 
 static int ffn_num_cus() { return um_num_cus(); }
@@ -1078,6 +1157,23 @@
     return split;
 }
 
+static int ffn_plan_workgroups(int tiles, int cus) {
+    if (tiles <= cus) return tiles;
+    const int per = (tiles + cus - 1) / cus;
+    return (tiles + per - 1) / per;
+}
+
+extern "C" int um_ffn_plan(int m, int* workgroups, int* tiles_per_wg_max) {
+    if (m <= 0) {
+        um_set_error("um_ffn_plan: bad argument (m=%d)", m);
+        return -1;
+    }
+    const int tiles = (m + 127) / 128, g = ffn_plan_workgroups(tiles, ffn_num_cus());
+    if (workgroups) *workgroups = g;
+    if (tiles_per_wg_max) *tiles_per_wg_max = (tiles + g - 1) / g;
+    return 0;
+}
+
 static size_t ffn_hs_bytes(int m, int split) {
     const size_t tiles = (size_t)((m + 127) / 128);
     return ((tiles * sizeof(unsigned) + 255) & ~(size_t)255) + tiles * split * (64 * 256 * sizeof(float));
@@ -1102,13 +1198,20 @@
 extern "C" int um_kv4_fwd(const float* x, const void* wc_planes, int m, int wshift, void* out_planes, int mode, void* stream_);
 static int ffn_impl(const float* x, const float* y, const void* w1_planes, const void* w2_planes, int m, int hidden,
                     int wshift, const float* gamma, const float* beta, float eps, float* out, int mode, void* workspace,
-                    size_t workspace_bytes, const void* wc_planes, void* kv_planes, void* stream_);
+                    size_t workspace_bytes, const void* wc_planes, void* kv_planes, int grid_limit, void* stream_);
 
 extern "C" int um_ffn_ws_fwd(const float* x, const float* y, const void* w1_planes, const void* w2_planes, int m, int hidden,
                              int wshift, const float* gamma, const float* beta, float eps, float* out, int mode, void* workspace,
                              size_t workspace_bytes, void* stream_) {
     return ffn_impl(x, y, w1_planes, w2_planes, m, hidden, wshift, gamma, beta, eps, out, mode, workspace, workspace_bytes, nullptr,
-                    nullptr, stream_);
+                    nullptr, 0, stream_);
+}
+
+extern "C" int um_ffn_ws_fwd_ex(const float* x, const float* y, const void* w1_planes, const void* w2_planes, int m, int hidden,
+                                int wshift, const float* gamma, const float* beta, float eps, float* out, int mode, void* workspace,
+                                size_t workspace_bytes, int grid_limit, void* stream_) {
+    return ffn_impl(x, y, w1_planes, w2_planes, m, hidden, wshift, gamma, beta, eps, out, mode, workspace, workspace_bytes, nullptr,
+                    nullptr, grid_limit, stream_);
 }
 
 extern "C" int um_ffn_kv_fwd(const float* x, const float* y, const void* w1_planes, const void* w2_planes, int m, int hidden,
@@ -1119,14 +1222,25 @@
         return -1;
     }
     return ffn_impl(x, y, w1_planes, w2_planes, m, hidden, wshift, gamma, beta, eps, out, mode, workspace, workspace_bytes, wc_planes,
-                    kv_planes, stream_);
+                    kv_planes, 0, stream_);
+}
+
+extern "C" int um_ffn_kv_fwd_ex(const float* x, const float* y, const void* w1_planes, const void* w2_planes, int m, int hidden,
+                                int wshift, const float* gamma, const float* beta, float eps, float* out, const void* wc_planes,
+                                void* kv_planes, int mode, void* workspace, size_t workspace_bytes, int grid_limit, void* stream_) {
+    if (!wc_planes || !kv_planes) {
+        um_set_error("um_ffn_kv_fwd: null k | v weight planes or output planes");
+        return -1;
+    }
+    return ffn_impl(x, y, w1_planes, w2_planes, m, hidden, wshift, gamma, beta, eps, out, mode, workspace, workspace_bytes, wc_planes,
+                    kv_planes, grid_limit, stream_);
 }
 
 static int ffn_impl(const float* x, const float* y, const void* w1_planes, const void* w2_planes, int m, int hidden,
                     int wshift, const float* gamma, const float* beta, float eps, float* out, int mode, void* workspace,
-                    size_t workspace_bytes, const void* wc_planes, void* kv_planes, void* stream_) {
+                    size_t workspace_bytes, const void* wc_planes, void* kv_planes, int grid_limit, void* stream_) {
     if (!x || !y || !w1_planes || !w2_planes || !gamma || !beta || !out || m <= 0 || hidden < 64 || hidden % 32 != 0 ||
-        (mode != 0 && mode != 1) || wshift < 0 || wshift > 14) {
+        (mode != 0 && mode != 1) || wshift < 0 || wshift > 14 || grid_limit < 0) {
         um_set_error("um_ffn_fwd: bad argument (m=%d hidden=%d wshift=%d mode=%d; hidden must be a multiple of 32, >= 64)",
                      m, hidden, wshift, mode);
         return -1;
@@ -1174,7 +1288,10 @@
         a.kv.M = m;
         a.kv.out_scale = a.out_scale;
     }
-    const hipError_t e = mode == 0 ? launch_ffn<Fp16, 2>(a, (hipStream_t)stream_) : launch_ffn<Bf16, 1>(a, (hipStream_t)stream_);
+    const int tiles = (m + 127) / 128;
+    const int workgroups = grid_limit > 0 ? (grid_limit < tiles ? grid_limit : tiles) : ffn_plan_workgroups(tiles, ffn_num_cus());
+    const hipError_t e = mode == 0 ? launch_ffn<Fp16, 2>(a, workgroups, (hipStream_t)stream_)
+                                   : launch_ffn<Bf16, 1>(a, workgroups, (hipStream_t)stream_);
     if (e != hipSuccess) {
         um_set_error("um_ffn_fwd: launch failed: %s", hipGetErrorString(e));
         return (int)e;
diff --git a/unimatch_amd/ops.py b/unimatch_amd/ops.py
--- a/unimatch_amd/ops.py
+++ b/unimatch_amd/ops.py
@@ -126,6 +126,8 @@
     block_kv = True
     refine_hoist = True
     fused_kv = True
+    ffn_tile_loop = True
+    ffn_grid_limit = 0
     fused_conv = True
     norm_on_load = True
     fused_entry = True
@@ -259,6 +261,11 @@
         _abi.check(code, 'um_linear_fwd')
         return out
 
+    def _ffn_grid_limit(self, m):
+        if not self.ffn_tile_loop:
+            return (m + 127) // 128
+        return int(self.ffn_grid_limit)
+
     def ffn_ln(self, x, y, w1, w2, norm):
         w1p, hid, k1 = self.weight_planes((w1,))
         w2p, n2, k2 = self.weight_planes((w2,))
@@ -271,11 +278,12 @@
             raise ValueError('ffn_ln: x and y must have the same number of rows')
         out = torch.empty((m, 128), dtype=torch.float32, device=x.device)
         ws = self._split_workspace('ffn_hsplit', (m, hid), x.device)
-        code = self._launch('ffn', lambda: self.lib.um_ffn_ws_fwd(
+        limit = self._ffn_grid_limit(m)
+        code = self._launch('ffn', lambda: self.lib.um_ffn_ws_fwd_ex(
             _ptr(x), _ptr(y), _ptr(w1p), _ptr(w2p), m, hid, self.WSHIFT, _ptr(norm.weight), _ptr(norm.bias),
             float(norm.eps), _ptr(out), self.mode, _ptr(ws) if ws is not None else None, ws.numel() if ws is not None else 0,
-            _stream()), {'flops': 2.0 * m * hid * (256 + 128)})
-        _abi.check(code, 'um_ffn_ws_fwd')
+            limit, _stream()), {'flops': 2.0 * m * hid * (256 + 128)})
+        _abi.check(code, 'um_ffn_ws_fwd_ex')
         return out
 
     def ffn_ln_kv(self, x, y, w1, w2, norm, kv_weights):
@@ -292,11 +300,12 @@
         out = torch.empty((m, 128), dtype=torch.float32, device=x.device)
         kv = torch.empty(self.lib.um_planes_bytes(4 * m, 128, self.mode), dtype=torch.uint8, device=x.device)
         ws = self._split_workspace('ffn_hsplit', (m, hid), x.device)
-        code = self._launch('ffn', lambda: self.lib.um_ffn_kv_fwd(
+        limit = self._ffn_grid_limit(m)
+        code = self._launch('ffn', lambda: self.lib.um_ffn_kv_fwd_ex(
             _ptr(x), _ptr(y), _ptr(w1p), _ptr(w2p), m, hid, self.WSHIFT, _ptr(norm.weight), _ptr(norm.bias),
             float(norm.eps), _ptr(out), _ptr(wc), _ptr(kv), self.mode, _ptr(ws) if ws is not None else None,
-            ws.numel() if ws is not None else 0, _stream()), {'flops': 2.0 * m * hid * (256 + 128) + 2.0 * m * 512 * 128})
-        _abi.check(code, 'um_ffn_kv_fwd')
+            ws.numel() if ws is not None else 0, limit, _stream()), {'flops': 2.0 * m * hid * (256 + 128) + 2.0 * m * 512 * 128})
+        _abi.check(code, 'um_ffn_kv_fwd_ex')
         return out, kv
 
     def window_attention_planes(self, q, k, v, streams, h, w, win_h, win_w, shift_h=0, shift_w=0, kv_rotate=0):
```

Result: no change. 963.8 (median of 6 runs) (+0.3%).
